# zzmuxi/simian-spacemonkey

Hardware: AMD Instinct MI355X
Metric: Msamples/s + fps, 512^3 VGH vol @1024^2 x 512 steps (higher is better)
Workload: dtype f32

## Files before the change

simian-spacemonkey_amd/csrc/smk_api.hip:

```cpp
#include <math.h>
#include <stdio.h>
#include <string.h>

#include <algorithm>

#include "smk_device.h"

static std::string g_create_err;

#include <condition_variable>
#include <mutex>
#include <thread>
namespace {
struct HostPool {
  std::vector<std::thread> workers;
  std::mutex m, use;
  std::condition_variable cv, done_cv;
  const std::function<void(int)> *job = nullptr;
  int njobs = 0, next = 0, pending = 0;
  unsigned long long gen = 0;
  bool quit = false;
  explicit HostPool(int n) {
    for (int i = 0; i < n; ++i)
      workers.emplace_back([this] {
        unsigned long long seen = 0;
        for (;;) {
          std::unique_lock<std::mutex> lk(m);
          cv.wait(lk, [&] { return quit || (gen != seen && next < njobs); });
          if (quit) return;
          while (next < njobs) {
            const int k = next++;
            lk.unlock();
            (*job)(k);
            lk.lock();
            if (--pending == 0) done_cv.notify_all();
          }
          seen = gen;
        }
      });
  }
  ~HostPool() {
    {
      std::lock_guard<std::mutex> lk(m);
      quit = true;
    }
    cv.notify_all();
    for (std::thread &t : workers) t.join();
  }
};
HostPool *host_pool() {
  static HostPool *pool = [] {
    const char *e = getenv("SMK_HOST_THREADS");
    int n = e ? atoi(e) : (int)std::min(16u, std::max(1u, std::thread::hardware_concurrency() / 2));
    n = std::max(1, std::min(n, 32));
    return new HostPool(n - 1);
  }();
  return pool;
}
}

int smk_host_pool_size() { return (int)host_pool()->workers.size() + 1; }

void smk_host_pool_run(int n, const std::function<void(int)> &f) {
  HostPool *p = host_pool();
  if (n <= 1 || p->workers.empty()) {
    for (int k = 0; k < n; ++k) f(k);
    return;
  }
  std::lock_guard<std::mutex> one(p->use);
  {
    std::lock_guard<std::mutex> lk(p->m);
    p->job = &f;
    p->njobs = n;
    p->next = 1;
    p->pending = n - 1;
    ++p->gen;
  }
  p->cv.notify_all();
  f(0);
  std::unique_lock<std::mutex> lk(p->m);
  while (p->next < p->njobs) {
    const int k = p->next++;
    lk.unlock();
    f(k);
    lk.lock();
    --p->pending;
  }
  p->done_cv.wait(lk, [&] { return p->pending == 0; });
  p->job = nullptr;
  p->njobs = 0;
}


extern "C" smk_ctx *smk_create(int device_ordinal, int *err) {
  int n = 0;
  hipError_t e = hipGetDeviceCount(&n);
  if (e != hipSuccess || n <= 0) {
    g_create_err = "smk_create: no HIP device available (this library has no CPU fallback)";
    if (err) *err = 1;
    return nullptr;
  }
  if (device_ordinal < 0 || device_ordinal >= n) {
    g_create_err = "smk_create: device ordinal out of range";
    if (err) *err = 2;
    return nullptr;
  }
  if (hipSetDevice(device_ordinal) != hipSuccess) {
    g_create_err = "smk_create: hipSetDevice failed";
    if (err) *err = 3;
    return nullptr;
  }
  smk_ctx *c = new smk_ctx();
  c->device = device_ordinal;
  if (hipStreamCreateWithFlags(&c->stream, hipStreamNonBlocking) != hipSuccess) {
    g_create_err = "smk_create: stream/event creation failed";
    delete c;
    if (err) *err = 4;
    return nullptr;
  }
  if (err) *err = 0;
  return c;
}

static void free_brick_set(BrickSet &B) {
  if (B.flags) (void)hipFree(B.flags);
  if (B.dil) (void)hipFree(B.dil);
  if (B.sat) (void)hipFree(B.sat);
  if (B.d_count) (void)hipFree(B.d_count);
  if (B.h_count) (void)hipHostFree(B.h_count);
  if (B.counted) (void)hipEventDestroy(B.counted);
  B = BrickSet();
}

static void free_volume(smk_ctx *c) {
  smk_free_steps(c);
  smk_cols_drop_layouts(&c->cols);
  c->d_brick_mm = nullptr;
  c->d_vox_x = nullptr;
  c->d_vox = nullptr;
  c->d_nrm = nullptr;
  c->have_volume = false;
}

extern "C" void smk_destroy(smk_ctx *c) {
  if (!c) return;
  (void)hipSetDevice(c->device);
  (void)hipDeviceSynchronize();
  free_volume(c);
  for (smk_ctx::TfVersion &T : c->tfv) {
    if (T.d) (void)hipFree(T.d);
    if (T.h) (void)hipHostFree(T.h);
    free_brick_set(T.br);
    if (T.copied) (void)hipEventDestroy(T.copied);
    if (T.used) (void)hipEventDestroy(T.used);
  }
  if (c->tf_raw_ev) (void)hipEventDestroy(c->tf_raw_ev);
  if (c->tf_ready) (void)hipEventDestroy(c->tf_ready);
  if (c->tf_stream) { (void)hipStreamSynchronize(c->tf_stream); (void)hipStreamDestroy(c->tf_stream); }
  free_brick_set(c->br3);
  smk_cols_free(&c->cols);
  void *ptrs[] = {c->d_light_hist, c->d_shadow_entries, c->d_shadow_exports, c->d_shadow_barrier, c->d_tf_raw, c->d_tlut, c->d_tf_h, c->d_tf3d, c->d_tf3d_occ, c->d_noise, c->d_out, c->d_depth, c->d_zscene, c->d_light[0], c->d_light[1]};
  for (void *p : ptrs)
    if (p) (void)hipFree(p);
  smk_slab_free(&c->slab);
  for (hipEvent_t e : c->tev0) (void)hipEventDestroy(e);
  for (hipEvent_t e : c->tev1) (void)hipEventDestroy(e);
  if (c->stream) (void)hipStreamDestroy(c->stream);
  delete c;
}

extern "C" const char *smk_last_error(smk_ctx *c) { return c ? c->err.c_str() : g_create_err.c_str(); }


template <int DT>
__global__ void smk_k_pack(const void *src, const unsigned char *grad, int bx, int by, int cz, int nelts,
                           int gx0, int gy0, int gz0,
                           int Ox, int Oy, int Oz, int Dx, int Dy, int Dz, void *dst, uint32_t *nrm, int n_in_w) {
  size_t t = (size_t)blockIdx.x * blockDim.x + threadIdx.x;
  size_t total = (size_t)bx * by * cz;
  if (t >= total) return;
  int x = (int)(t % bx);
  int y = (int)((t / bx) % by);
  int z = (int)(t / ((size_t)bx * by));
  int X = gx0 + x - Ox, Y = gy0 + y - Oy, Z = gz0 + z - Oz;
  if (X < 0 || X >= Dx || Y < 0 || Y >= Dy || Z < 0 || Z >= Dz) return;
  size_t o = ((size_t)Z * Dy + Y) * Dx + X;
  uint32_t nb = 0x00808080u;
  if (grad) nb = (uint32_t)grad[t * 3] | ((uint32_t)grad[t * 3 + 1] << 8) | ((uint32_t)grad[t * 3 + 2] << 16);
  if (DT == 0) {
    const unsigned char *s = (const unsigned char *)src + t * nelts;
    uint32_t d = 0;
    for (int e = 0; e < nelts; ++e) d |= (uint32_t)s[e] << (8 * e);
    ((uint2 *)dst)[o] = make_uint2(d, nb);
  } else {
    const float *s = (const float *)src + t * nelts;
    float4 v = make_float4(0.f, 0.f, 0.f, 0.f);
    v.x = s[0];
    if (nelts > 1) v.y = s[1];
    if (nelts > 2) v.z = s[2];
    if (n_in_w) v.w = __uint_as_float(nb);
    else {
      v.w = s[3];
      if (nrm) nrm[o] = nb;
    }
    ((float4 *)dst)[o] = v;
  }
}

static void shard_box(const int N[3], int rank, int nranks, int g0[3], int g1[3]) {
  for (int a = 0; a < 3; ++a) {
    g0[a] = 0;
    g1[a] = N[a];
  }
  int bit = 0;
  for (int n = nranks; n > 1; n >>= 1, ++bit) {
    int a = bit % 3, half = N[a] / 2;
    if ((rank >> bit) & 1) g0[a] = std::max(g0[a], half);
    else g1[a] = std::min(g1[a], half);
  }
}

void smk_shard_region(const smk_ctx *c, int rank, int g0[3], int g1[3]) { shard_box(c->N, rank, c->nranks, g0, g1); }

int smk_volume_geometry(smk_ctx *c, const char *who, const smk_volume_desc *b, int nb, int nelts, smk_dtype dtype,
                        smk_datamode dmode, SmkVolGeom &g) {
  if (!b || nb <= 0) FAIL(c, "%s: no bricks", who);
  if (nelts < 1 || nelts > 4) FAIL(c, "%s: nelts %d not in 1..4", who, nelts);
  if (dtype != SMK_U8 && dtype != SMK_F32) FAIL(c, "%s: bad dtype", who);
  g = SmkVolGeom();
  g.dtype = dtype;
  g.nelts = nelts;
  g.dmode = dmode;
  int *N = g.N;
  float *fs = g.fs;
  bool any_grad = false, all_grad = true;
  for (int i = 0; i < nb; ++i) {
    if (!b[i].data) FAIL(c, "%s: brick %d has no data", who, i);
    if (b[i].xiSize <= 0 || b[i].yiSize <= 0 || b[i].ziSize <= 0) FAIL(c, "%s: brick %d empty", who, i);
    if (b[i].xiPos < 0 || b[i].yiPos < 0 || b[i].ziPos < 0) FAIL(c, "%s: brick %d negative origin", who, i);
    N[0] = std::max(N[0], b[i].xiPos + b[i].xiSize);
    N[1] = std::max(N[1], b[i].yiPos + b[i].yiSize);
    N[2] = std::max(N[2], b[i].ziPos + b[i].ziSize);
    fs[0] = std::max(fs[0], b[i].xfPos + b[i].xfSize);
    fs[1] = std::max(fs[1], b[i].yfPos + b[i].yfSize);
    fs[2] = std::max(fs[2], b[i].zfPos + b[i].zfSize);
    any_grad |= b[i].grad != nullptr;
    all_grad &= b[i].grad != nullptr;
  }
  if (any_grad && !all_grad) FAIL(c, "%s: some bricks have normals and some do not", who);
  size_t vox = 0;
  for (int i = 0; i < nb; ++i) vox += (size_t)b[i].xiSize * b[i].yiSize * b[i].ziSize;
  if (vox != (size_t)N[0] * N[1] * N[2]) FAIL(c, "%s: bricks do not tile the %dx%dx%d volume", who, N[0], N[1], N[2]);
  if (!(fs[0] > 0 && fs[1] > 0 && fs[2] > 0)) FAIL(c, "%s: non-positive extent", who);
  if (c->nranks > 1)
    for (int a = 0; a < 3; ++a)
      if (N[a] < 2) FAIL(c, "%s: volume too thin to shard", who);
  g.grad = any_grad;
  shard_box(N, c->rank, c->nranks, g.g0, g.g1);
  for (int a = 0; a < 3; ++a) {
    int lo = std::max(g.g0[a] - c->halo, 0), hi = std::min(g.g1[a] + c->halo, N[a]);
    g.O[a] = lo;
    g.D[a] = hi - lo;
  }
  if (dtype == SMK_U8)
    for (int a = 0; a < 2; ++a)
      if (g.D[a] & 1) {
        if (g.O[a] + g.D[a] < N[a]) ++g.D[a];
        else if (g.O[a] > 0) { --g.O[a]; ++g.D[a]; }
        else { ++g.D[a]; g.padded = true; }
      }
  const size_t nst = (size_t)g.D[0] * g.D[1] * g.D[2];
  g.vox_bytes = nst * (dtype == SMK_U8 ? 8 : 16);
  g.nrm_bytes = dtype == SMK_F32 && nelts == 4 && any_grad ? nst * 4 : 0;
  for (int a = 0; a < 3; ++a) g.nbr[a] = (g.D[a] - 1) / (1 << SMK_BRICK_LOG2) + 1;
  g.mm_bytes = (size_t)g.nbr[0] * g.nbr[1] * g.nbr[2] * sizeof(float4);
  return 0;
}

void smk_set_geometry(smk_ctx *c, const SmkVolGeom &g) {
  c->dtype = g.dtype;
  c->nelts = g.nelts;
  c->dmode = g.dmode;
  for (int a = 0; a < 3; ++a) {
    c->N[a] = g.N[a];
    c->fsize[a] = g.fs[a];
    c->g0[a] = g.g0[a];
    c->g1[a] = g.g1[a];
    c->O[a] = g.O[a];
    c->D[a] = g.D[a];
    c->nbr[a] = g.nbr[a];
  }
  c->vox_bytes = g.vox_bytes;
  c->have_normals = g.grad;
}

int smk_alloc_step(smk_ctx *c, const SmkVolGeom &g, TimeStep &T) {
  if (!T.vox) {
    HIPCHK(c, hipMalloc(&T.vox, g.vox_bytes + 16));
    if (g.padded) HIPCHK(c, hipMemset(T.vox, 0, g.vox_bytes));
  }
  if (g.nrm_bytes && !T.nrm) HIPCHK(c, hipMalloc((void **)&T.nrm, g.nrm_bytes));
  if (!T.mm) HIPCHK(c, hipMalloc((void **)&T.mm, g.mm_bytes));
  return 0;
}

int smk_pack_step(smk_ctx *c, const char *who, const SmkVolGeom &g, const smk_volume_desc *b, int nb, bool on_device, TimeStep &T,
                  hipStream_t s) {
// ... 355 lines not shown
  if (!c || !out) return 1;
  if (!c->have_volume || !c->have_camera) FAIL(c, "smk_get_raycoef: volume and camera must be set");
  double inv[16];
  return compute_raycoef(c, out, inv);
}

static void normalize3(float v[3]) {
  float l = sqrtf(v[0] * v[0] + v[1] * v[1] + v[2] * v[2]);
  if (l > 0) {
    v[0] /= l;
    v[1] /= l;
    v[2] /= l;
  }
}

static void shading_vectors(const smk_ctx *c, RenderParams &P) {
  const float *r = c->xform;
  P.R[0] = r[0]; P.R[1] = r[4]; P.R[2] = r[8];
  P.R[3] = r[1]; P.R[4] = r[5]; P.R[5] = r[9];
  P.R[6] = r[2]; P.R[7] = r[6]; P.R[8] = r[10];
  P.intens = c->intens;
  P.use_spec = (c->shade == SMK_SHADE_R8K_DSPEC || c->shade == SMK_SHADE_NV20_DSPEC) ? 1 : 0;
  if (c->shade == SMK_SHADE_R8K_DIFF || c->shade == SMK_SHADE_R8K_DSPEC) {
    float l[3] = {-c->light_pos[0], -c->light_pos[1], -c->light_pos[2]};
    normalize3(l);
    float vd[3] = {-(c->eye[0] - c->at[0]), -(c->eye[1] - c->at[1]), -(c->eye[2] - c->at[2])};
    normalize3(vd);
    float h[3];
    for (int k = 0; k < 3; ++k) h[k] = l[k] + 0.5f * (vd[k] - l[k]);
    normalize3(h);
    memcpy(P.L, l, 12);
    memcpy(P.Hv, h, 12);
  } else {
    float vd[3] = {c->eye[0] - c->at[0], c->eye[1] - c->at[1], c->eye[2] - c->at[2]};
    normalize3(vd);
    float lt[3] = {c->light_pos[0] - c->at[0], c->light_pos[1] - c->at[1], c->light_pos[2] - c->at[2]};
    normalize3(lt);
    float h[3];
    for (int k = 0; k < 3; ++k) h[k] = lt[k] + 0.5f * (vd[k] - lt[k]);
    float hv[3] = {r[0] * h[0] + r[1] * h[1] + r[2] * h[2], r[4] * h[0] + r[5] * h[1] + r[6] * h[2],
                   r[8] * h[0] + r[9] * h[1] + r[10] * h[2]};
    float lv[3] = {r[0] * lt[0] + r[1] * lt[1] + r[2] * lt[2], r[4] * lt[0] + r[5] * lt[1] + r[6] * lt[2],
                   r[8] * lt[0] + r[9] * lt[1] + r[10] * lt[2]};
    for (int k = 0; k < 3; ++k) {
      hv[k] = -hv[k];
      lv[k] = -lv[k];
    }
    normalize3(hv);
    normalize3(lv);
    memcpy(P.L, lv, 12);
    memcpy(P.Hv, hv, 12);
  }
}

static int make_brick_set(smk_ctx *c, BrickSet &B, const uint32_t *occ, int roww, int sv, int sg, hipStream_t s) {
  const size_t nbricks = (size_t)c->nbr[0] * c->nbr[1] * c->nbr[2], sat_words = (size_t)(sv + 1) * (sg + 1);
  if (B.flags_cap < nbricks) {
    if (B.flags) (void)hipFree(B.flags);
    B.flags = nullptr;
    B.flags_cap = 0;
    HIPCHK(c, hipMalloc((void **)&B.flags, nbricks));
    B.flags_cap = nbricks;
  }
  if (B.sat_cap < sat_words) {
    if (B.sat) (void)hipFree(B.sat);
    B.sat = nullptr;
    B.sat_cap = 0;
    HIPCHK(c, hipMalloc((void **)&B.sat, sat_words * 4));
    B.sat_cap = sat_words;
  }
  if (!B.d_count) HIPCHK(c, hipMalloc((void **)&B.d_count, 4));
  if (!B.h_count) HIPCHK(c, hipHostMalloc((void **)&B.h_count, 4, hipHostMallocDefault));
  if (!B.counted) HIPCHK(c, hipEventCreateWithFlags(&B.counted, hipEventDisableTiming));
  else HIPCHK(c, hipEventSynchronize(B.counted));
  if (smk_step_wait_ready(c, s)) return 1;
  HIPCHK(c, smk_bricks_flags(c->d_brick_mm, c->nbr, occ, roww, sv, sg, B.sat, B.flags, B.d_count, s));
  HIPCHK(c, hipMemcpyAsync(B.h_count, B.d_count, 4, hipMemcpyDeviceToHost, s));
  HIPCHK(c, hipEventRecord(B.counted, s));
  B.valid = true;
  B.fill = -1.f;
  B.dil_r[0] = -1;
  return 0;
}

static const unsigned char *brick_flags_to_use(smk_ctx *c, BrickSet &B) {
  if (!B.valid) return nullptr;
  if (B.fill < 0.f && hipEventQuery(B.counted) == hipSuccess)
    B.fill = (float)((double)*B.h_count / ((double)c->nbr[0] * c->nbr[1] * c->nbr[2]));
  (void)hipGetLastError();
  return B.fill > 0.9f ? nullptr : B.flags;
}

__global__ __launch_bounds__(256) void smk_k_tf_effective(const uint32_t *raw, const unsigned char *map, int sv, int sg, int roww,
                                                           uint32_t *eff, uint32_t *occ) {
  const int wave = (int)((blockIdx.x * 256u + threadIdx.x) >> 6), lane = threadIdx.x & 63;
  const int wpr = (sv + 63) / 64;
  const int t = wave / wpr, s = (wave - t * wpr) * 64 + lane;
  if (t >= sg) return;
  bool any = false;
  if (s < sv) {
    const int s1 = min(s + 1, sv - 1), t1 = min(t + 1, sg - 1);
    const uint32_t a = raw[(size_t)t * sv + s];
    const unsigned ma = map[a >> 24];
    eff[(size_t)t * sv + s] = (a & 0x00ffffffu) | (ma << 24);
    any = (ma | map[raw[(size_t)t * sv + s1] >> 24] | map[raw[(size_t)t1 * sv + s] >> 24] | map[raw[(size_t)t1 * sv + s1] >> 24]) != 0;
  }
  const unsigned long long m = __ballot(any);
  const int w0 = (s - lane) >> 5;
  if (lane == 0 && w0 < roww) occ[(size_t)t * roww + w0] = (uint32_t)m;
  if (lane == 32 && w0 + 1 < roww) occ[(size_t)t * roww + w0 + 1] = (uint32_t)(m >> 32);
}

static float tf2d_rate(const smk_ctx *c, const smk_raycoef &rc) {
  if (c->scale_alphas) {
    float rate = c->steps > 0 ? (float)(c->fsize[0] / ((double)c->N[0] * (double)rc.dis)) : c->sample_rate;
    return rate * 1 / c->gamma;
  }
  return 1 / c->gamma;
}

static void tf2d_alpha_map(const smk_ctx *c, float sr, unsigned char map[256]) {
  if (c->opt_tf_raw) {
    for (int a = 0; a < 256; ++a) map[a] = (unsigned char)a;
    return;
  }
  const float alphaScale = (float)(1.0 / sr);
  for (int a = 0; a < 256; ++a) map[a] = (unsigned char)(int)((1.0 - pow((1.0 - (a / 255.0)), alphaScale)) * 255);
}

static int refresh_tf2d(smk_ctx *c, const smk_raycoef &rc, hipStream_t frame_stream) {
  if (c->tf_mode != 1) return 0;
  const float sr = tf2d_rate(c, rc);
  if (!c->tf_dirty && sr == c->tf_rate_applied && c->d_tf_vg) {
    if (c->tf_ready_pending) HIPCHK(c, hipStreamWaitEvent(frame_stream, c->tf_ready, 0));
    return 0;
  }
  unsigned char newmap[256];
  tf2d_alpha_map(c, sr, newmap);
  if (!c->tf_dirty && c->d_tf_vg && c->tf_map_valid && !memcmp(newmap, c->tf_map_applied, 256)) {
    c->tf_rate_applied = sr;
    if (c->tf_ready_pending) HIPCHK(c, hipStreamWaitEvent(frame_stream, c->tf_ready, 0));
    return 0;
  }
  if (!c->tf_stream) HIPCHK(c, hipStreamCreateWithFlags(&c->tf_stream, hipStreamNonBlocking));
  if (!c->tf_ready) HIPCHK(c, hipEventCreateWithFlags(&c->tf_ready, hipEventDisableTiming));
  const hipStream_t s = c->tf_stream;
  const size_t n = (size_t)c->sv * c->sg;
  const int sv = c->sv, sg = c->sg, roww = (sv + 31) / 32;
  const size_t occ_words = (size_t)roww * sg, bytes = n * 4 + occ_words * 4 + 256;
  const int v = (c->tf_cur + 1) & 3;
  smk_ctx::TfVersion &T = c->tfv[v];
  if (T.cap < bytes) {
    if (T.copied) (void)hipEventSynchronize(T.copied);
    if (T.used_valid) (void)hipEventSynchronize(T.used);
    if (T.d) (void)hipFree(T.d);
    if (T.h) (void)hipHostFree(T.h);
    T.d = nullptr;
    T.h = nullptr;
    T.cap = 0;
    HIPCHK(c, hipMalloc((void **)&T.d, bytes));
    HIPCHK(c, hipHostMalloc((void **)&T.h, bytes, hipHostMallocDefault));
    T.cap = bytes;
    if (!T.copied) HIPCHK(c, hipEventCreateWithFlags(&T.copied, hipEventDisableTiming));
    if (!T.used) HIPCHK(c, hipEventCreateWithFlags(&T.used, hipEventDisableTiming));
    T.used_valid = false;
  } else if (T.copied) {
    HIPCHK(c, hipEventSynchronize(T.copied));
  }
  if (c->tf_raw_cap < n * 4) {
    HIPCHK(c, hipDeviceSynchronize());
    if (c->d_tf_raw) (void)hipFree(c->d_tf_raw);
    c->d_tf_raw = nullptr;
    c->tf_raw_cap = 0;
    HIPCHK(c, hipMalloc((void **)&c->d_tf_raw, n * 4));
    c->tf_raw_cap = n * 4;
    c->tf_raw_stale = true;
  }
  if (!c->tf_raw_ev) HIPCHK(c, hipEventCreateWithFlags(&c->tf_raw_ev, hipEventDisableTiming));
  if (c->tf_raw_stale) {
    memcpy(T.h, c->h_tf_vg.data(), n * 4);
    if (c->tf_raw_ev_valid) HIPCHK(c, hipStreamWaitEvent(s, c->tf_raw_ev, 0));
    HIPCHK(c, hipMemcpyAsync(c->d_tf_raw, T.h, n * 4, hipMemcpyHostToDevice, s));
    c->tf_raw_stale = false;
  }
  unsigned char *map = T.h + n * 4 + occ_words * 4;
  memcpy(map, newmap, 256);
  memcpy(c->tf_map_applied, newmap, 256);
  c->tf_map_valid = true;
  if (T.used_valid) HIPCHK(c, hipStreamWaitEvent(s, T.used, 0));
  HIPCHK(c, hipMemcpyAsync(T.d + n * 4 + occ_words * 4, map, 256, hipMemcpyHostToDevice, s));
  HIPCHK(c, hipEventRecord(T.copied, s));
  {
    const int wpr = (sv + 63) / 64;
    const unsigned blocks = (unsigned)(((size_t)wpr * sg + 3) / 4);
    hipLaunchKernelGGL(smk_k_tf_effective, dim3(blocks), dim3(256), 0, s, (const uint32_t *)c->d_tf_raw, T.d + n * 4 + occ_words * 4, sv,
                       sg, roww, (uint32_t *)T.d, (uint32_t *)(T.d + n * 4));
    HIPCHK(c, hipGetLastError());
    HIPCHK(c, hipEventRecord(c->tf_raw_ev, s));
    c->tf_raw_ev_valid = true;
  }
  c->tf_cur = v;
  c->d_tf_vg = reinterpret_cast<uint32_t *>(T.d);
  c->d_tf_occ = reinterpret_cast<uint32_t *>(T.d + n * 4);
  T.br.valid = false;
  if (c->opt_bricks && c->d_brick_mm && make_brick_set(c, T.br, c->d_tf_occ, roww, sv, sg, s)) return 1;
  c->tf_occ_roww = roww;
  c->tf_rate_applied = sr;
  c->tf_dirty = false;
  HIPCHK(c, hipEventRecord(c->tf_ready, s));
  HIPCHK(c, hipStreamWaitEvent(frame_stream, c->tf_ready, 0));
  c->tf_ready_pending = true;
  return 0;
}

extern "C" int smk_get_tf2d_effective(smk_ctx *c, unsigned char *out, float *rate) {
  if (!c) return 1;
  if (c->tf_mode != 1 || !c->have_volume || !c->have_camera) FAIL(c, "smk_get_tf2d_effective: 2-D TF, volume and camera required");
  smk_raycoef rc;
  double inv[16];
  compute_raycoef(c, &rc, inv);
  if (refresh_tf2d(c, rc, c->stream)) return 1;
  if (out) {
    unsigned char map[256];
    tf2d_alpha_map(c, c->tf_rate_applied, map);
    memcpy(out, c->h_tf_vg.data(), c->h_tf_vg.size());
    for (size_t i = 0; i < (size_t)c->sv * c->sg; ++i) out[i * 4 + 3] = map[c->h_tf_vg[i * 4 + 3]];
  }
  if (rate) *rate = c->tf_rate_applied;
  return 0;
}

void smk_bsp_order(const smk_ctx *c, const double pos[3], int *order) {
  int nearbit[3];
  for (int a = 0; a < 3; ++a) nearbit[a] = pos[a] >= (double)(c->N[a] / 2) - 0.5 ? 1 : 0;
  int nbits = 0;
  for (int n = c->nranks; n > 1; n >>= 1) ++nbits;
  std::vector<std::pair<int, int>> keyed;
  for (int r = 0; r < c->nranks; ++r) {
    int key = 0;
    for (int bit = 0; bit < nbits; ++bit)
      if (((r >> bit) & 1) != nearbit[bit % 3]) key |= 1 << bit;
    keyed.push_back({key, r});
  }
  std::sort(keyed.begin(), keyed.end());
  for (int r = 0; r < c->nranks; ++r) order[r] = keyed[r].second;
}

extern "C" int smk_shard_order(smk_ctx *c, int *order) {
  if (!c || !order) return 1;
  if (!c->have_volume || !c->have_camera) FAIL(c, "smk_shard_order: volume and camera must be set");
  double inv[16];
  smk_inverse_affine(inv, c->mv);
  double e[3];
  for (int a = 0; a < 3; ++a) e[a] = inv[12 + a] * c->N[a] / c->fsize[a] - 0.5;
  smk_bsp_order(c, e, order);
  return 0;
}


extern "C" int smk_set_option(smk_ctx *c, const char *key, int value) {
  if (!c || !key) return 1;
  if (!strcmp(key, "kernel")) c->opt_kernel = value;
  else if (!strcmp(key, "slab_T")) c->slab.opt_T = value & 0xff;
  else if (!strcmp(key, "inject_slab_status")) c->opt_inject_status = value;
  else if (!strcmp(key, "slab_fly")) c->slab.opt_fly = value < 0 ? 0 : (value > 63 ? 63 : value);
  else if (!strcmp(key, "slab_ns")) c->slab.opt_ns = value < 0 ? 0 : (value > 63 ? 63 : value);
  else if (!strcmp(key, "tile")) c->slab.opt_tile = value;
  else if (!strcmp(key, "shadow_march")) c->opt_shadow_march = value ? 1 : 0;
  else if (!strcmp(key, "shadow_fused")) c->opt_lockstep = value ? (c->opt_lockstep | 256) : (c->opt_lockstep & ~256);
  else if (!strcmp(key, "slab_split")) c->slab.opt_split = value < 0 ? 0 : (value > 8 ? 8 : value);
  else if (!strcmp(key, "cols_shape")) c->cols.opt_shape = value & 0xff;
  else if (!strcmp(key, "cols_ns")) c->cols.opt_ns = value & 0xff;
  else if (!strcmp(key, "cols_chunk")) c->cols.opt_chunk = value & 0xfff;
  else if (!strcmp(key, "cols_wstep")) c->cols.opt_wstep = value & 7;
  else if (!strcmp(key, "cols_counts")) c->cols.want_counts = value ? 1 : 0;
  else if (!strcmp(key, "cols_fill")) { c->cols.opt_fill = value; smk_cols_drop_layouts(&c->cols); }
  else if (!strcmp(key, "cols_take_min")) c->cols.opt_take_min = value;
  else if (!strcmp(key, "cols_take_wait")) c->cols.opt_take_wait = value;
  else if (!strcmp(key, "cols_fly")) c->cols.opt_fly = value;
  else if (!strcmp(key, "bricks")) {
    c->opt_bricks = value ? 1 : 0;
    c->tf_dirty = true;
    c->bricks3_dirty = true;
  }
  else if (!strcmp(key, "wave_w")) {
    if (!(value == 1 || value == 2 || value == 4 || value == 8 || value == 16 || value == 32 || value == 64)) FAIL(c, "smk_set_option: wave_w must be a power of two <= 64");
    c->opt_wave_w = value;
  } else if (!strcmp(key, "blk_w")) {
    if (!(value == 1 || value == 2 || value == 4)) FAIL(c, "smk_set_option: blk_w must be 1, 2 or 4");
    c->opt_blk_w = value;
  } else if (!strcmp(key, "lockstep")) c->opt_lockstep = value;
  else if (!strcmp(key, "tf_raw")) {
    c->opt_tf_raw = value;
    c->tf_dirty = true;
  }
  else if (!strcmp(key, "halo")) {
    if (c->have_volume) FAIL(c, "smk_set_option: halo must be set before smk_upload_volume");
    if (value < 1) FAIL(c, "smk_set_option: halo must be >= 1");
    c->halo = value;
  } else
    FAIL(c, "smk_set_option: unknown key '%s'", key);
  return 0;
}

extern "C" int smk_get_brick_flags(smk_ctx *c, unsigned char *flags_out, int *nb_out, int *in_use_out) {
  if (!c || !nb_out) return 1;
  HIPCHK(c, hipSetDevice(c->device));
  RenderParams P;
  if (smk_build_params(c, P, c->stream)) return 1;
  HIPCHK(c, hipDeviceSynchronize());
  for (int a = 0; a < 3; ++a) nb_out[a] = c->nbr[a];
  const BrickSet *B = c->tf_mode == 1 && c->tf_cur >= 0 ? &c->tfv[c->tf_cur].br : c->tf_mode == 2 ? &c->br3 : nullptr;
  if (in_use_out) *in_use_out = P.bricks != nullptr ? 1 : 0;
  if (flags_out) {
    if (!B || !B->valid || !B->flags) FAIL(c, "smk_get_brick_flags: no flags for this table (1-D colour table, or option 'bricks' 0)");
    HIPCHK(c, hipMemcpy(flags_out, B->flags, (size_t)c->nbr[0] * c->nbr[1] * c->nbr[2], hipMemcpyDeviceToHost));
  }
  return 0;
}

template <class Launch>
static int count_on_device(smk_ctx *c, Launch launch, double *out) {
  unsigned long long *d = nullptr, h = 0;
  HIPCHK(c, hipMalloc((void **)&d, 8));
  hipError_t e = hipMemsetAsync(d, 0, 8, c->stream);
  if (e == hipSuccess) e = launch(d);
  if (e == hipSuccess) e = hipMemcpyAsync(&h, d, 8, hipMemcpyDeviceToHost, c->stream);
  if (e == hipSuccess) e = hipStreamSynchronize(c->stream);
  (void)hipFree(d);
  HIPCHK(c, e);
  *out = (double)h;
  return 0;
}

extern "C" int smk_get_stat(smk_ctx *c, const char *name, double *value) {
  if (!c || !name || !value) return 1;
  HIPCHK(c, hipSetDevice(c->device));
  static const char *diag_names[16] = {"slab_iters", "slab_active_lanes", "slab_inside_lanes", "slab_hit_lanes",
                                      "slab_loader_issue_kcyc", "slab_loader_wait_kcyc", "slab_loader_blocked_kcyc", "slab_loader_total_kcyc",
                                      "slab_iters_with_hit", "slab_lead_sum", "slab_waits", "slab_wstep_sum", "slab_dead_tail_sum", "slab_waves",
                                      "slab_iters_sampling", "slab_iters_own_brick"};
  for (int k = 0; k < 16; ++k)
    if (!strcmp(name, diag_names[k])) {
      float v = 0.f;
      if (c->slab.d_diag && read_back(c, &v, c->slab.d_diag + k, 1)) return 1;
      *value = v;
      return 0;
    }
  if (!strcmp(name, "light_samples")) {
    RenderParams P;
    smk_shadowcoef sc;
    float olo[3], ohi[3];
    if (smk_shadow_light_owned(c, P, sc, olo, ohi)) return 1;
    return count_on_device(c, [&](unsigned long long *d) { return smk_launch_shadow_count_light(P, sc, olo, ohi, d, c->stream); }, value);
  }
  if (!strcmp(name, "slab_status")) {
    HIPCHK(c, hipDeviceSynchronize());
    *value = c->slab.h_status ? (((volatile int *)c->slab.h_status)[c->slab.status_slot] & 0xff) : 0;
    return 0;
  }
  if (!strcmp(name, "slab_failures")) {
    long long n = c->slab_failures;
    if (c->slab.h_status)
      for (int k = 0; k < SMK_STATUS_RING; ++k) n += ((volatile int *)c->slab.h_status)[k] != 0;
    *value = (double)n;
    return 0;
  }
  if (!strcmp(name, "slab_streamed_fraction")) {
    *value = 1.0;
    const int nt = c->slab.ticks_n_last;
    if (c->last_kernel == 2 && c->slab.d_ticks && nt > 0) {
      std::vector<unsigned> h((size_t)2 * nt);
      if (read_back(c, h.data(), c->slab.d_ticks + nt, h.size())) return 1;
      double st = 0, pl = 0;
      for (int t = 0; t < nt; ++t) {
        st += h[t];
        pl += h[(size_t)nt + t];
      }
      if (pl > 0) *value = st / pl;
    }
    return 0;
  }
  if (!strcmp(name, "slab_tile_ms_max") || !strcmp(name, "slab_tile_ms_sum")) {
    *value = 0.0;
    const int nt = c->slab.ticks_n_last;
    if (c->last_kernel == 2 && c->slab.d_ticks && nt > 0) {
      std::vector<unsigned> h((size_t)nt);
      if (read_back(c, h.data(), c->slab.d_ticks, h.size())) return 1;
      double mx = 0, sum = 0;
      for (int t = 0; t < nt; ++t) {
        const double k = t < (int)c->slab.ksplit_last.size() ? std::max<int>(c->slab.ksplit_last[t], 1) : 1;
        mx = std::max(mx, (double)h[t] / k);
        sum += h[t];
      }
      *value = (name[13] == 'm' ? mx : sum) * 1e-5;
    }
    return 0;
  }
  if (!strncmp(name, "cols_", 5)) return smk_cols_stat(c, name, value);
  if (!strcmp(name, "slab_split_tiles")) { *value = c->slab.nsplit_last; return 0; }
  if (!strcmp(name, "slab_workgroups")) { *value = c->slab.nblocks_last; return 0; }
  if (!strcmp(name, "slab_retries")) { *value = (double)c->slab_retries; return 0; }
  if (!strcmp(name, "clip_slice_pass")) { *value = c->clip_slice_pass; return 0; }
  FAIL(c, "smk_get_stat: unknown name '%s'", name);
}

extern "C" int smk_get_trace(smk_ctx *c, unsigned *out, int cap_records, int *nrecords) {
  if (!c || !nrecords) return 1;
  HIPCHK(c, hipSetDevice(c->device));
  if (!(c->opt_lockstep & 32)) {
    const int nt = c->last_kernel == 2 && c->slab.d_ticks ? c->slab.ticks_n_last : 0;
    *nrecords = nt;
    if (out && nt > 0) {
      std::vector<unsigned> h((size_t)nt * 5);
      if (read_back(c, h.data(), c->slab.d_ticks, h.size())) return 1;
      for (int t = 0; t < std::min(cap_records, nt); ++t) {
        unsigned *r = out + (size_t)t * 8;
        r[0] = h[(size_t)3 * nt + t];
        r[1] = h[(size_t)3 * nt + t] ? r[0] + h[t] : 0u;
        r[2] = h[(size_t)4 * nt + t] & 0xff00u;
        r[3] = (h[(size_t)4 * nt + t] & 0xfu) | ((unsigned)t << 8) | (h[(size_t)2 * nt + t] << 20);
        r[4] = r[5] = r[6] = r[7] = 0;
      }
    }
    return 0;
  }
  *nrecords = c->slab.d_trace ? c->slab.trace_n : 0;
  if (out && *nrecords > 0 && read_back(c, out, c->slab.d_trace, (size_t)std::min(cap_records, *nrecords) * 8)) return 1;
  return 0;
}

extern "C" int smk_count_samples(smk_ctx *c, double *in_volume) {
  if (!c || !in_volume) return 1;
  HIPCHK(c, hipSetDevice(c->device));
  RenderParams P;
  if (smk_build_params(c, P, c->stream)) return 1;
  smk_shadowcoef sc;
  if (c->shadow_on && c->tf_mode != 0 && !P.pert_on && !c->region_on && smk_shadow_setup(c, P, sc, nullptr, nullptr)) return 1;
  return count_on_device(c, [&](unsigned long long *d) { return smk_launch_count_inside(P, d, c->stream); }, in_volume);
}

void smk_region_box(const smk_ctx *c, const int g0[3], const int g1[3], float lo[3], float hi[3], int top[3]) {
  for (int a = 0; a < 3; ++a) {
    lo[a] = (float)g0[a] - 0.5f;
    hi[a] = (float)g1[a] - 0.5f;
    top[a] = g1[a] == c->N[a];
  }
  if (c->clip_axis >= 1 && c->clip_axis <= 6) {
    const int a = (c->clip_axis - 1) / 2;
    const float fs = c->fsize[a];
    const float cp = c->clip_vpos[a] > 0.0f ? (c->clip_vpos[a] < fs ? c->clip_vpos[a] : fs) : 0.0f;
    const float face = (float)((double)cp / (double)fs * (double)c->N[a] - 0.5);
    if ((c->clip_axis - 1) % 2 == 0) {
      if (face < hi[a] || (face == hi[a] && !top[a])) { hi[a] = face; top[a] = 1; }
    } else if (face > lo[a]) {
      lo[a] = face;
    }
  }
  if (c->region_on)
    for (int a = 0; a < 3; ++a) {
      const double fs = c->fsize[a];
      const double l = c->region_lo[a] > 0 ? (c->region_lo[a] < fs ? c->region_lo[a] : fs) : 0.0;
      const double h = c->region_hi[a] > 0 ? (c->region_hi[a] < fs ? c->region_hi[a] : fs) : 0.0;
      const float flo = (float)(l / fs * (double)c->N[a] - 0.5), fhi = (float)(h / fs * (double)c->N[a] - 0.5);
      if (flo > lo[a]) lo[a] = flo;
      if (fhi < hi[a]) { hi[a] = fhi; top[a] = 0; }
    }
}

int smk_build_params(smk_ctx *c, RenderParams &P, hipStream_t s) {
  if (!c->have_volume) FAIL(c, "smk_render: no volume uploaded");
  if (!c->have_camera) FAIL(c, "smk_render: no camera set");
  if (c->tf_mode < 0) FAIL(c, "smk_render: no transfer function set");
  memset(&P, 0, sizeof P);
  double inv[16];
  compute_raycoef(c, &P.rc, inv);
  if (refresh_tf2d(c, P.rc, s)) return 1;
  if (smk_step_wait_ready(c, s)) return 1;
  P.vox = c->d_vox;
  P.nrm = c->d_nrm;
  for (int a = 0; a < 3; ++a) {
    P.N[a] = c->N[a];
    P.O[a] = c->O[a];
    P.D[a] = c->D[a];
    P.invN[a] = 1.0f / (float)c->N[a];
  }
  smk_region_box(c, c->g0, c->g1, P.lo, P.hi, P.top);
  for (int a = 0; a < 3; ++a) P.hin[a] = P.top[a] ? P.hi[a] : nextafterf(P.hi[a], -INFINITY);
  P.cplane_on = c->cplane_on;
  for (int k = 0; k < 4; ++k) P.cplane[k] = 0.0f;
  if (c->cplane_on) {
    double pm[4];
    for (int k = 0; k < 4; ++k)
      pm[k] = c->cplane_eye[0] * c->mv[4 * k + 0] + c->cplane_eye[1] * c->mv[4 * k + 1] + c->cplane_eye[2] * c->mv[4 * k + 2] +
              c->cplane_eye[3] * c->mv[4 * k + 3];
    double w = pm[3];
    for (int a = 0; a < 3; ++a) {
      const double sc = (double)c->fsize[a] / (double)c->N[a];
      P.cplane[a] = (float)(pm[a] * sc);
      w += pm[a] * sc * 0.5;
    }
    P.cplane[3] = (float)w;
  }
  P.nelts = c->nelts;
  P.n_in_w = (c->dtype == SMK_F32 && c->nelts <= 3) ? 1 : 0;
  P.tlut = c->d_tlut;
  P.tlut_size = c->tlut_size;
  P.tf_vg = c->d_tf_vg;
  P.tf_h = c->d_tf_h;
  P.tf_occ = c->tf_mode == 1 ? c->d_tf_occ : c->tf_mode == 2 ? c->d_tf3d_occ : nullptr;
  P.occ_roww = c->tf_mode == 2 ? c->tf3d_occ_roww : c->tf_occ_roww;
  P.sv = c->sv;
  P.sg = c->sg;
  bool third = c->dmode == SMK_GDM_VGH || c->dmode == SMK_GDM_V1GH || c->dmode == SMK_GDM_V2G ||
               c->dmode == SMK_GDM_V2GH || c->dmode == SMK_GDM_V3 || c->dmode == SMK_GDM_V3G || c->dmode == SMK_GDM_V4;
  P.third_axis = (third && c->d_tf_h && c->nelts >= 3) ? 1 : 0;
  P.tf3d = c->d_tf3d;
  P.s3v = c->s3v;
  P.s3g = c->s3g;
  P.s3h = c->s3h;
  P.bricks = nullptr;
  for (int a = 0; a < 3; ++a) P.nbr[a] = c->nbr[a];
  BrickSet *bset = nullptr;
  P.bricks_dil = nullptr;
  if (c->opt_bricks && c->d_brick_mm) {
    if (c->tf_mode == 1 && c->tf_cur >= 0) {
      P.bricks = brick_flags_to_use(c, c->tfv[c->tf_cur].br);
      bset = &c->tfv[c->tf_cur].br;
    }
    if (c->tf_mode == 2 && c->d_tf3d_occ) {
      if (c->bricks3_dirty || !c->br3.valid) {
        HIPCHK(c, hipDeviceSynchronize());
        if (make_brick_set(c, c->br3, c->d_tf3d_occ, c->tf3d_occ_roww, c->s3v, c->s3g, s)) return 1;
        c->bricks3_dirty = false;
      }
      P.bricks = brick_flags_to_use(c, c->br3);
      bset = &c->br3;
    }
  }
  P.W = c->W;
  P.H = c->H;
  P.znear = c->clip[0];
  shading_vectors(c, P);
  P.blend = c->blend;
  P.noise = c->d_noise;
  P.nn = c->nn;
  P.nn_log2 = -1;
  for (int l = 0; l < 12; ++l)
    if (c->nn == (1 << l)) P.nn_log2 = l;
  P.pw[0] = c->pw[0];
  P.pw[1] = c->pw[1];
  P.ps[0] = c->ps[0];
  P.ps[1] = c->ps[1];
  P.pert_on = (c->d_noise && (c->pw[0] != 0 || c->pw[1] != 0)) ? 1 : 0;
// ... 255 lines not shown
```

simian-spacemonkey_amd/csrc/smk_cols_plan.hip:

```cpp
#include <math.h>
#include <stdio.h>
#include <string.h>

#include <algorithm>
#include <vector>

#include "smk_cols.h"

struct ColPlan {
  int as, au, av;
  int perm;
  double dens;
  int shape;
  int vb;
  size_t fixed;
  int njobs;
};

static const char *cols_refusal(const RenderParams &P, int dtype, int tf_mode) {
  if (P.zscene) return "scene depth";
  if (tf_mode < 0 || tf_mode > 2) return "no classification mode";
  if (tf_mode == 0 && (!P.tlut || P.tlut_size < 1)) return "no colour table";
  if (tf_mode == 1 && (!P.tf_vg || P.sv < 2 || P.sg < 2)) return "transfer function smaller than 2x2";
  if (tf_mode == 2 && (!P.tf3d || P.s3v < 1 || P.s3g < 1 || P.s3h < 1)) return "no 3-D table";
// ... 98 lines not shown
    if (!project(u, v, sc, x0, y0) || !project(u + 1, v, sc, x1, y1) || !project(u, v + 1, sc, x2, y2) || !project(u, v, sc + 1, x3, y3))
      return "volume reaches behind the eye";
    dens = std::max(dens, fabs((x1 - x0) * (y2 - y0) - (x2 - x0) * (y1 - y0)));
  }
  if (!(dens > 1e-9)) return "degenerate projection";
  L.dens = dens;
  return nullptr;
}

static const char *cols_lds_budget(const RenderParams &P, int dtype, int tf_mode, const ColsAux *aux, ColParams &Q, ColPlan &L) {
  L.shape = aux->opt_shape ? aux->opt_shape - 1 : 0;
  if (L.shape < 0 || L.shape >= COL_NSHAPES) return "no such workgroup shape";
  L.vb = dtype == 0 ? 8 : 16;
  const bool three = P.third_axis && P.tf_h;
  Q.use_ah = (tf_mode == 1 && three && P.nelts <= 3 && P.sv >= 2 && P.sv <= 1024) ? 1 : 0;
  Q.fast_tf = (tf_mode == 1 && (!three || Q.use_ah)) ? 1 : 0;
  const size_t occ_bytes = tf_mode == 1 ? (size_t)P.occ_roww * P.sg * 4 : tf_mode == 2 ? (size_t)P.occ_roww * P.s3g * 4 : 0;
  Q.use_occ = (P.tf_occ && occ_bytes > 0 && occ_bytes <= 16384 && (Q.fast_tf || tf_mode == 2)) ? 1 : 0;
  L.fixed = (size_t)COL_MAX_RAYS * 9 + (size_t)3 * (COL_MAX_CL + 4) * 4 + 32 * 4 + (Q.use_ah ? (size_t)P.sv * 4 : 0) + (Q.use_occ ? occ_bytes : 0) + 64;
  return nullptr;
}

static size_t cols_slice_bytes(int cw, int ch, int vb) { return (((size_t)(cw + 1) * (ch + 1) * vb) + 15) & ~(size_t)15; }

static bool cols_fits(const ColPlan &L, double fill, int cw, int ch, int slots) {
  if ((double)cw * ch * L.dens > fill * (kColShapes[L.shape].nw * 64)) return false;
  const size_t sb = cols_slice_bytes(cw, ch, L.vb);
  if (sb * slots + L.fixed > COL_LDS_CAP) return false;
  if ((sb + 1023) / 1024 * 2 > 63) return false;
  return true;
}

static void cols_free_layout(ColLayout &L) {
  if (L.d) (void)hipFree(L.d);
  L = ColLayout();
}

static bool cols_column_size(const ColPlan &L, double fill, int cells_u, int cells_v, int slots, int *bw, int *bh) {
  *bw = *bh = 0;
  double best = 1e300;
  for (int ncu = 1; ncu <= cells_u; ++ncu) {
    const int cw = (cells_u + ncu - 1) / ncu;
    if (cw > 255) continue;
    if (ncu > 1 && (cells_u + ncu - 2) / (ncu - 1) == cw) continue;
    for (int ncv = 1; ncv <= cells_v; ++ncv) {
      const int ch = (cells_v + ncv - 1) / ncv;
      if (ch > 255) continue;
      if (ncv > 1 && (cells_v + ncv - 2) / (ncv - 1) == ch) continue;
      if (!cols_fits(L, fill, cw, ch, slots)) continue;
      const double over = (double)ncu * (cw + 1) * (double)ncv * (ch + 1) / ((double)cells_u * cells_v);
      if (over < best) { best = over; *bw = cw; *bh = ch; }
    }
  }
  return *bw != 0;
}

static hipError_t cols_layout(const RenderParams &P, ColParams &Q, const ColPlan &L, int dtype, const void *vox_native, ColsAux *aux,
                              const char **why, hipStream_t s) {
  ColLayout &LY = aux->lay[L.perm];
  const int lanes = kColShapes[L.shape].nw * 64;
  const int cells_u = Q.Du - 1, cells_v = Q.Dv - 1;
  const double fill = (aux->opt_fill > 0 ? aux->opt_fill : 92) * 0.01;
  bool reuse = LY.d && LY.Du == Q.Du && LY.Dv == Q.Dv && LY.Ds == Q.Ds && LY.src == vox_native && LY.vb == L.vb;
  if (reuse) {
    reuse = cols_fits(L, fill, LY.CW, LY.CH, 3) && ((double)LY.CW * LY.CH * L.dens > 0.45 * lanes || (LY.CW >= cells_u && LY.CH >= cells_v));
  }
  if (!reuse) {
    int bw, bh;
    if (!cols_column_size(L, fill, cells_u, cells_v, aux->opt_ns ? aux->opt_ns : 6, &bw, &bh)) {
      *why = "no column size fits the lanes (view too close)";
      return hipErrorNotSupported;
    }
    const int ncu = (cells_u + bw - 1) / bw, ncv = (cells_v + bh - 1) / bh;
    const size_t sb = cols_slice_bytes(bw, bh, L.vb);
    const size_t bytes = (size_t)ncu * ncv * Q.Ds * sb;
    size_t free_b = 0, total_b = 0;
    (void)hipMemGetInfo(&free_b, &total_b);
    if (LY.d) cols_free_layout(LY);
    if (bytes + ((size_t)2 << 30) > free_b + 0) {
      for (int k = 0; k < 3; ++k)
        if (k != L.perm) cols_free_layout(aux->lay[k]);
      (void)hipMemGetInfo(&free_b, &total_b);
      if (bytes + ((size_t)1 << 30) > free_b) { *why = "no memory for the column layout"; return hipErrorNotSupported; }
    }
    void *d = nullptr;
    if (hipMalloc(&d, bytes + 4096) != hipSuccess) { (void)hipGetLastError(); *why = "no memory for the column layout"; return hipErrorNotSupported; }
    LY.d = d; LY.bytes = bytes; LY.CW = bw; LY.CH = bh; LY.ncu = ncu; LY.ncv = ncv; LY.Du = Q.Du; LY.Dv = Q.Dv; LY.Ds = Q.Ds;
    LY.slice_bytes = (int)sb; LY.src = vox_native; LY.vb = L.vb;
    const size_t total = (size_t)ncu * ncv * Q.Ds * (size_t)(bw + 1) * (bh + 1);
    const unsigned blocks = (unsigned)((total + 255) / 256);
    if (total / 256 > 0x7fffffffull) { *why = "volume too large for the layout builder"; return hipErrorNotSupported; }
    hipError_t e = smk_cols_build(vox_native, dtype, L.perm, P.D, bw, bh, ncu, ncv, (int)sb, d, blocks, s);
    if (e != hipSuccess) return e;
    ++aux->builds;
  }
  Q.lay = (const char *)LY.d;
  Q.CW = LY.CW; Q.CH = LY.CH; Q.ncu = LY.ncu; Q.ncv = LY.ncv;
  Q.slice_bytes = LY.slice_bytes;
  return hipSuccess;
}

static const char *cols_ring(const ColsAux *aux, const ColPlan &L, ColParams &Q) {
  Q.n_ch = (Q.slice_bytes + 1023) / 1024;
  const int last_units = Q.slice_bytes / 16 - 64 * (Q.n_ch - 1);
  Q.last_mask = last_units >= 64 ? ~0ull : ((1ull << last_units) - 1ull);
  int nslots = (int)((COL_LDS_CAP - L.fixed) / (size_t)Q.slice_bytes);
  if (aux->opt_ns) nslots = std::min(nslots, aux->opt_ns);
  nslots = std::min(nslots, 12);
  if (nslots < 3) return "column slice does not fit LDS three times";
  Q.nslots = nslots;
  Q.maxfly = std::max(1, std::min(aux->opt_fly > 0 ? aux->opt_fly : 2, (nslots - 2) / kColShapes[L.shape].nl));
  while (Q.maxfly > 1 && Q.n_ch * Q.maxfly > 63) --Q.maxfly;
  if (Q.n_ch > 63) return "column slice needs more than 63 DMA instructions";
  Q.wstep = aux->opt_wstep ? aux->opt_wstep - 1 : (nslots >= 7 ? 2 : nslots >= 5 ? 1 : 0);
  Q.take_min = aux->opt_take_min > 0 ? aux->opt_take_min : 16;
  Q.take_wait = aux->opt_take_wait > 0 ? aux->opt_take_wait - 1 : 3;
  return nullptr;
}

static const char *cols_chunks(const ColsAux *aux, ColParams &Q, ColPlan &L) {
  const int npos_total = Q.Ds - 1;
  int clmax = aux->opt_chunk ? std::min(aux->opt_chunk, COL_MAX_CL) : 128;
  clmax = std::max(clmax, 4);
  Q.nck = (npos_total + clmax - 1) / clmax;
  Q.CL = (npos_total + Q.nck - 1) / Q.nck;
  Q.nck = (npos_total + Q.CL - 1) / Q.CL;
  Q.nkeys = Q.ncu + Q.ncv + Q.nck - 2;
  Q.mask_words = (Q.nkeys + 63) / 64;
  if (Q.mask_words > 8) return "more than 512 segment keys";
  L.njobs = Q.ncu * Q.ncv * Q.nck;
  return nullptr;
}

static hipError_t cols_side_buffers(const RenderParams &P, ColParams &Q, const ColPlan &L, ColsAux *aux, int *status_word, const char **why,
                                    hipStream_t s) {
  const size_t npix = (size_t)P.W * P.H;
  const size_t lay_bytes = (size_t)Q.nkeys * npix * 16;
  if (lay_bytes > aux->layers_cap) {
    if (aux->d_layers) (void)hipFree(aux->d_layers);
    aux->d_layers = nullptr; aux->layers_cap = 0;
    if (hipMalloc(&aux->d_layers, lay_bytes) != hipSuccess) { (void)hipGetLastError(); *why = "no memory for the segment layers"; return hipErrorNotSupported; }
    aux->layers_cap = lay_bytes;
  }
  const size_t mask_bytes = npix * Q.mask_words * 8;
  if (mask_bytes > aux->masks_cap || aux->masks_dirty) {
    if (mask_bytes > aux->masks_cap) {
      if (aux->d_masks) (void)hipFree(aux->d_masks);
      aux->d_masks = nullptr; aux->masks_cap = 0;
      if (hipMalloc(&aux->d_masks, mask_bytes) != hipSuccess) { (void)hipGetLastError(); *why = "no memory for the segment masks"; return hipErrorNotSupported; }
      aux->masks_cap = mask_bytes;
    }
    hipError_t e = hipMemsetAsync(aux->d_masks, 0, aux->masks_cap, s);
    if (e != hipSuccess) return e;
    aux->masks_dirty = false;
  }
  aux->mask_words_last = Q.mask_words;
  if (L.njobs > aux->ticks_cap) {
    if (aux->d_ticks) (void)hipFree(aux->d_ticks);
    aux->d_ticks = nullptr; aux->ticks_cap = 0;
    if (hipMalloc((void **)&aux->d_ticks, (size_t)L.njobs * 12) != hipSuccess) { (void)hipGetLastError(); *why = "no memory"; return hipErrorNotSupported; }
    aux->ticks_cap = L.njobs;
  }
  if (!aux->d_counts) {
    if (hipMalloc((void **)&aux->d_counts, 8 * 8) != hipSuccess) { (void)hipGetLastError(); *why = "no memory"; return hipErrorNotSupported; }
  }
  Q.layers = (float4 *)aux->d_layers;
  Q.masks = (unsigned long long *)aux->d_masks;
  Q.status = status_word;
  Q.status_tag = aux->status_tag;
  Q.job_ticks = aux->d_ticks;
  Q.counts = aux->want_counts ? aux->d_counts : nullptr;
  if (Q.counts) return hipMemsetAsync(aux->d_counts, 0, 64, s);
  return hipSuccess;
}

static hipError_t cols_run(const RenderParams &P, ColParams &Q, const ColPlan &L, ColsAux *aux, int dtype, int tf_mode, int shade_kind,
                           const char **why, hipStream_t s) {
  aux->njobs_last = L.njobs;
  aux->cw_last = Q.CW; aux->ch_last = Q.CH; aux->nslots_last = Q.nslots; aux->shape_last = L.shape;
  aux->last_stream_bytes = (double)L.njobs / Q.nck * ((double)(Q.Ds - 1) + Q.nck) * Q.slice_bytes;
  Q.ring_bytes = (int)std::max((size_t)Q.nslots * Q.slice_bytes, (size_t)COL_MAX_RAYS * 16);
  const size_t lds = (size_t)Q.ring_bytes + L.fixed;
  if (lds > COL_LDS_CAP) { *why = "column job does not fit LDS"; return hipErrorNotSupported; }
  if (aux->frame_ev0) {
    hipError_t e = hipEventRecord(aux->frame_ev0, s);
    if (e != hipSuccess) return e;
  }
  hipError_t e = smk_cols_march(P, Q, dtype, tf_mode, shade_kind, L.perm, L.shape, lds, L.njobs, s);
  if (e == hipErrorInvalidValue) { *why = "no column-stream instance for this mode"; return hipErrorNotSupported; }
  if (e != hipSuccess) return e;
  aux->masks_dirty = true;
  e = smk_cols_resolve((const float4 *)aux->d_layers, (unsigned long long *)aux->d_masks, Q.mask_words, (size_t)P.W * P.H, P.out,
                       P.blend == SMK_BLEND_MAX ? 1 : 0, s);
  if (e == hipSuccess) aux->masks_dirty = false;
  return e;
}

hipError_t smk_launch_cols(RenderParams P, int dtype, int tf_mode, int shade_kind, const void *vox_native, ColsAux *aux, int *status_word,
                           const char **why, hipStream_t s) {
  ColParams Q;
  memset(&Q, 0, sizeof Q);
  ColPlan L = {};
  if ((*why = cols_refusal(P, dtype, tf_mode))) return hipErrorNotSupported;
  if (tf_mode == 0) shade_kind = 0;
  if ((*why = cols_axes(P, Q, L)) || (*why = cols_projection(P, Q)) || (*why = cols_density(P, Q, L)) ||
      (*why = cols_lds_budget(P, dtype, tf_mode, aux, Q, L)))
    return hipErrorNotSupported;
  hipError_t e = cols_layout(P, Q, L, dtype, vox_native, aux, why, s);
  if (e != hipSuccess) return e;
  if ((*why = cols_ring(aux, L, Q)) || (*why = cols_chunks(aux, Q, L))) return hipErrorNotSupported;
  if ((e = cols_side_buffers(P, Q, L, aux, status_word, why, s)) != hipSuccess) return e;
  return cols_run(P, Q, L, aux, dtype, tf_mode, shade_kind, why, s);
}

void smk_cols_free(ColsAux *aux) {
  for (int k = 0; k < 3; ++k) cols_free_layout(aux->lay[k]);
  if (aux->d_layers) (void)hipFree(aux->d_layers);
  if (aux->d_masks) (void)hipFree(aux->d_masks);
  if (aux->d_ticks) (void)hipFree(aux->d_ticks);
  if (aux->d_counts) (void)hipFree(aux->d_counts);
  *aux = ColsAux();
}

void smk_cols_drop_layouts(ColsAux *aux) {
  for (int k = 0; k < 3; ++k) cols_free_layout(aux->lay[k]);
}

int smk_cols_stat(smk_ctx *c, const char *name, double *value) {
  const ColsAux &A = c->cols;
  *value = 0.0;
  if (!strcmp(name, "cols_builds")) { *value = A.builds; return 0; }
  if (!strcmp(name, "cols_config")) { *value = A.cw_last | (A.ch_last << 8) | (A.nslots_last << 16) | (A.shape_last << 24); return 0; }
  if (!strcmp(name, "cols_jobs")) { *value = A.njobs_last; return 0; }
  if (!strcmp(name, "cols_stream_bytes")) { *value = A.last_stream_bytes; return 0; }
  if (!strcmp(name, "cols_job_ms_max") || !strcmp(name, "cols_job_ms_sum") || !strcmp(name, "cols_setup_ms_sum") || !strcmp(name, "cols_rays")) {
    const int nj = A.njobs_last, part = name[5] == 'j' ? 0 : name[5] == 's' ? 1 : 2;
    if (c->last_kernel == 4 && A.d_ticks && nj > 0) {
      std::vector<unsigned> h((size_t)nj);
      if (read_back(c, h.data(), A.d_ticks + (size_t)nj * part, h.size())) return 1;
      double mx = 0, sum = 0;
      for (unsigned v : h) {
        mx = std::max(mx, (double)v);
        sum += v;
      }
      *value = part == 2 ? sum : (name[12] == 'm' ? mx : sum) * 1e-5;
    }
    return 0;
  }
  static const char *cn[8] = {"cols_samples", "cols_visible", "cols_slices", "cols_segments", "cols_iters", "cols_active_lanes", "cols_switch_iters", "cols_switch_lanes"};
  for (int k = 0; k < 8; ++k)
    if (!strcmp(name, cn[k])) {
      unsigned long long v = 0;
      if (A.d_counts && A.want_counts && read_back(c, &v, A.d_counts + k, 1)) return 1;
      *value = (double)v;
      return 0;
    }
  FAIL(c, "smk_get_stat: unknown name '%s'", name);
}
```

simian-spacemonkey_amd/csrc/smk_frame.hip:

```cpp
#include <math.h>
#include <stdio.h>
#include <stdlib.h>
#include <string.h>

#include <algorithm>

#include "smk_internal.h"

extern "C" int smk_timing_reset(smk_ctx *c) {
  if (!c) return 1;
  c->tcount = 0;
  return 0;
}

extern "C" int smk_timing_read(smk_ctx *c, float *avg_ms, int *nframes) {
  if (!c) return 1;
  HIPCHK(c, hipSetDevice(c->device));
  HIPCHK(c, hipDeviceSynchronize());
  int n = (int)std::min<long long>(c->tcount, SMK_TIMING_RING);
  double sum = 0;
  for (int i = 0; i < n; ++i) {
    float ms = 0;
    HIPCHK(c, hipEventElapsedTime(&ms, c->tev0[i], c->tev1[i]));
    sum += ms;
  }
  if (avg_ms) *avg_ms = n ? (float)(sum / n) : 0.f;
  if (nframes) *nframes = n;
  return 0;
}

extern "C" int smk_last_frame_info(smk_ctx *c, int *kernel, float *ms, double *alg_bytes) {
  if (!c) return 1;
  if (kernel) *kernel = c->last_kernel;
  if (ms) *ms = c->last_ms;
  if (alg_bytes) *alg_bytes = c->last_alg_bytes;
  return 0;
}

static int take_status(smk_ctx *c, long long id) {
  if (!c->slab.h_status || id <= 0) return 0;
  volatile int *w = (volatile int *)c->slab.h_status + (int)(id % SMK_STATUS_RING);
  const int st = *w;
  if (!st) return 0;
  const long long tag = (st >> 8) & 0x7fffff;
  if (tag != (id & 0x7fffff)) {
    if (((id - tag) & 0x7fffff) % SMK_STATUS_RING == 0 && tag != 0) {
      *w = 0;
      ++c->slab_failures;
      ++c->slab_lost;
    }
    return 0;
  }
  *w = 0;
  ++c->slab_failures;
  if (c->opt_kernel == 0 && c->last_slab_sig) c->tune_choice[c->last_slab_sig] = {1, c->frame_id + 256};
  return st & 0xff;
}

static const char *status_text(int st) {
  return st == 1 ? "a streaming kernel reported a producer/consumer time-out" : st == 2 ? "the slice-ring kernel reported a window outside its host bound"
         : st == 3 ? "the column-stream kernel reported a job whose rays do not fit its lanes or its list" : "the column-stream kernel reported a ray it cannot list";
}

static int check_frame_status(smk_ctx *c, long long id) {
  const int st = take_status(c, id);
  if (st) FAIL(c, "%s (status %d, frame %lld); frame invalid", status_text(st), st, id);
  return 0;
}

extern "C" long long smk_last_frame_id(smk_ctx *c) { return c ? c->frame_id : 0; }

extern "C" int smk_frame_failed(smk_ctx *c, long long frame_id) {
  if (!c) return 1;
  if (frame_id <= 0 || frame_id > c->frame_id || frame_id + SMK_STATUS_RING <= c->frame_id) return -1;
  return take_status(c, frame_id) ? 1 : 0;
}

static int status_ring_ready(smk_ctx *c) {
  if (c->slab.h_status) return 0;
  HIPCHK(c, hipHostMalloc((void **)&c->slab.h_status, SMK_STATUS_RING * sizeof(int), hipHostMallocMapped));
  for (int k = 0; k < SMK_STATUS_RING; ++k) c->slab.h_status[k] = 0;
  HIPCHK(c, hipMalloc((void **)&c->slab.d_diag, 16 * sizeof(float)));
  return 0;
}

static void inject_status(smk_ctx *c) {
  if (c->opt_inject_status && c->slab.h_status) {
    ((volatile int *)c->slab.h_status)[c->slab.status_slot] = c->slab.status_tag | c->opt_inject_status;
    c->opt_inject_status = 0;
  }
}


static int frame_open(smk_ctx *c, RenderParams &P, void *d_rgba, void *d_depth) {
  P.out = (float4 *)d_rgba;
  P.depth = (float *)d_depth;
  size_t nst = (size_t)c->D[0] * c->D[1] * c->D[2];
  double bv = c->dtype == SMK_U8 ? (double)c->nelts : 4.0 * c->nelts;
  if (smk_shade_kind(c)) bv += 3.0;
  double tfb = c->tf_mode == 0 ? 16.0 * c->tlut_size
               : c->tf_mode == 1 ? 4.0 * c->sv * c->sg * (P.third_axis ? 2 : 1)
                                 : 4.0 * c->s3v * c->s3g * c->s3h;
  c->last_alg_bytes = (double)nst * bv + tfb + 16.0 * c->W * c->H;
  if (P.zscene) c->last_alg_bytes += 4.0 * c->W * c->H;
  if (c->tev0.empty()) {
    c->tev0.resize(SMK_TIMING_RING);
    c->tev1.resize(SMK_TIMING_RING);
    for (int i = 0; i < SMK_TIMING_RING; ++i) {
      HIPCHK(c, hipEventCreate(&c->tev0[i]));
      HIPCHK(c, hipEventCreate(&c->tev1[i]));
    }
  }
  int slot = (int)(c->tcount % SMK_TIMING_RING);
  c->ev0 = c->tev0[slot];
  c->ev1 = c->tev1[slot];
  c->last_kernel = 1;
  c->slab_why.clear();
  if (check_frame_status(c, c->frame_id + 1 - SMK_STATUS_RING)) return 1;
  ++c->frame_id;
  c->slab.status_slot = (int)(c->frame_id % SMK_STATUS_RING);
  c->slab.status_tag = c->cols.status_tag = (int)((c->frame_id & 0x7fffff) << 8);
  if (c->slab.h_status) ((volatile int *)c->slab.h_status)[c->slab.status_slot] = 0;
  return 0;
}

struct KernelChoice {
  bool try_slab;
  unsigned long long sig;
  int trial;
};

static KernelChoice choose_kernel(smk_ctx *c, const RenderParams &P, bool with_depth, hipStream_t s) {
  KernelChoice k = {c->opt_kernel != 1 && c->opt_kernel != 3, 0, -1};
  if (c->opt_kernel != 0) return k;
  int as = 0;
  for (int a = 1; a < 3; ++a)
    if (fabsf(P.rc.Bc[a]) > fabsf(P.rc.Bc[as])) as = a;
  const unsigned long long f[] = {(unsigned long long)c->dtype, (unsigned long long)c->nelts, (unsigned long long)c->D[0],
                                  (unsigned long long)c->D[1], (unsigned long long)c->D[2], (unsigned long long)c->W,
                                  (unsigned long long)c->H, (unsigned long long)P.rc.nplanes, (unsigned long long)smk_shade_kind(c),
                                  (unsigned long long)P.third_axis, (unsigned long long)(as * 2 + (P.rc.Bc[as] > 0)),
                                  (unsigned long long)c->sv, (unsigned long long)c->sg, (unsigned long long)with_depth,
                                  (unsigned long long)P.pert_on, (unsigned long long)c->tf_mode, (unsigned long long)c->s3v,
                                  (unsigned long long)c->s3g, (unsigned long long)c->s3h, (unsigned long long)c->blend,
                                  (unsigned long long)P.sh.on, (unsigned long long)(P.zscene != nullptr)};
  k.sig = 1469598103934665603ull;
  for (unsigned long long v : f) k.sig = (k.sig ^ v) * 1099511628211ull;
  auto it = c->tune_choice.find(k.sig);
  if (it != c->tune_choice.end() && it->second.expires <= c->frame_id) {
    c->tune_choice.erase(it);
    it = c->tune_choice.end();
    c->tune_sig = 0;
  }
  if (it != c->tune_choice.end()) {
    k.try_slab = it->second.kernel == 2;
    return k;
  }
  if (c->tune_sig != k.sig) {
    c->tune_sig = k.sig;
    c->tune_state = 0;
  }
  if (c->tune_state == SMK_TUNE_SETTLE + 3) {
    float ms_s = 0, ms_g = 0;
    if (c->tcount - c->tune_tcount >= SMK_TIMING_RING - 8) (void)hipEventSynchronize(c->tev1[c->tune_slot[1]]);
    if (hipEventQuery(c->tev1[c->tune_slot[0]]) == hipSuccess && hipEventQuery(c->tev1[c->tune_slot[1]]) == hipSuccess &&
        hipEventElapsedTime(&ms_s, c->tev0[c->tune_slot[0]], c->tev1[c->tune_slot[0]]) == hipSuccess &&
        hipEventElapsedTime(&ms_g, c->tev0[c->tune_slot[1]], c->tev1[c->tune_slot[1]]) == hipSuccess) {
      c->tune_choice[k.sig] = {ms_s <= ms_g ? 2 : 1, c->frame_id + 1024};
      k.try_slab = ms_s <= ms_g;
      if (getenv("SMK_DEBUG")) fprintf(stderr, "[smk] auto mode: slice-ring %.3f ms, gather %.3f ms (frame %lld)\n", ms_s, ms_g, c->frame_id);
    }
    (void)hipGetLastError();
  } else {
    k.trial = c->tune_state;
    k.try_slab = k.trial != SMK_TUNE_SETTLE && k.trial != SMK_TUNE_SETTLE + 2;
    if (k.try_slab && k.trial > 0) (void)hipStreamSynchronize(s);
  }
  return k;
}

static int launch_cols(smk_ctx *c, const RenderParams &P, hipStream_t s) {
  if (status_ring_ready(c)) return 1;
  const char *why = nullptr;
  c->cols.frame_ev0 = c->ev0;
  hipError_t e = smk_launch_cols(P, c->dtype, c->tf_mode, smk_shade_kind(c), c->d_vox, &c->cols,
                                 c->slab.h_status + c->slab.status_slot, &why, s);
  if (e == hipErrorNotSupported) {
    c->slab_why = why ? why : "?";
    FAIL(c, "smk_render: column-stream kernel forced but not applicable: %s", c->slab_why.c_str());
  }
  HIPCHK(c, e);
  c->last_kernel = 4;
  inject_status(c);
  return 0;
}

static int launch_slab(smk_ctx *c, const RenderParams &P, KernelChoice &k, bool ev0_recorded, hipStream_t s) {
  if (status_ring_ready(c)) return 1;
  if (c->opt_lockstep & 16) HIPCHK(c, hipMemsetAsync(c->slab.d_diag, 0, 16 * sizeof(float), s));
  const char *why = nullptr;
  c->slab.frame_ev0 = ev0_recorded ? nullptr : c->ev0;
  hipError_t e = smk_launch_slab(P, c->dtype, c->tf_mode, smk_shade_kind(c), c->d_vox, c->d_vox_x, &c->slab, &why, s);
  if (e == hipErrorNotSupported && why && !strcmp(why, "x-major copy unavailable")) {
    if (smk_make_xmajor_copy(c)) return 1;
    e = smk_launch_slab(P, c->dtype, c->tf_mode, smk_shade_kind(c), c->d_vox, c->d_vox_x, &c->slab, &why, s);
  }
  if (e == hipSuccess) {
    c->last_kernel = 2;
    c->last_slab_sig = k.sig;
    inject_status(c);
  } else if (e == hipErrorNotSupported) {
    c->slab_why = why ? why : "?";
    if (c->opt_kernel == 2) FAIL(c, "smk_render: slab kernel forced but not applicable: %s", c->slab_why.c_str());
    if (c->opt_kernel == 0) k.trial = -1;
  } else
    HIPCHK(c, e);
  return 0;
}

static int launch_gather(smk_ctx *c, const RenderParams &P, bool ev0_recorded, hipStream_t s) {
  if (!ev0_recorded) HIPCHK(c, hipEventRecord(c->ev0, s));
  HIPCHK(c, smk_launch_gather(P, c->dtype, c->tf_mode, smk_shade_kind(c), s));
  return 0;
}

static int frame_close(smk_ctx *c, hipStream_t s, int trial) {
  HIPCHK(c, hipEventRecord(c->ev1, s));
  if (trial >= 0) {
    if (trial >= SMK_TUNE_SETTLE + 1) {
      c->tune_slot[trial - (SMK_TUNE_SETTLE + 1)] = (int)(c->tcount % SMK_TIMING_RING);
      c->tune_tcount = c->tcount;
    }
    c->tune_state = trial + 1;
  }
  if (c->tf_mode == 1 && c->tf_cur >= 0) {
    HIPCHK(c, hipEventRecord(c->tfv[c->tf_cur].used, s));
    c->tfv[c->tf_cur].used_valid = true;
  }
  if (smk_step_mark_used(c, s)) return 1;
  c->tcount++;
  return 0;
}

static int scene_depth_kind_check(smk_ctx *c, const char *who, int kind) {
  if (kind != SMK_SCENE_VIEW_DEPTH && kind != SMK_SCENE_WINDOW_DEPTH)
    FAIL(c, "%s: bad scene depth kind %d (SMK_SCENE_VIEW_DEPTH = 0 or SMK_SCENE_WINDOW_DEPTH = 1)", who, kind);
  return 0;
}

static int render_frame(smk_ctx *c, const char *who, void *d_rgba, void *d_depth, const float *d_zscene, int zkind, void *stream) {
  if (!c) return 1;
  HIPCHK(c, hipSetDevice(c->device));
  if (!d_rgba) FAIL(c, "%s: null output", who);
  RenderParams P;
  hipStream_t s = stream ? (hipStream_t)stream : c->stream;
  if (smk_build_params(c, P, s)) return 1;
  if (d_zscene) {
    P.zscene = d_zscene;
    P.zscene_kind = zkind;
    const double n = c->clip[0], f = c->clip[1];
    if (zkind == SMK_SCENE_WINDOW_DEPTH && !(f > n))
      FAIL(c, "%s: window depths need a far plane beyond the near plane (clip = %g, %g)", who, n, f);
    P.zs_fn = f * n;
    P.zs_f = f;
    P.zs_fmn = f - n;
  }
  if (frame_open(c, P, d_rgba, d_depth)) return 1;
  bool marched = false;
  if (c->shadow_on) {
    if (smk_shadow_frame(c, P, d_rgba, d_depth, s, &marched)) return 1;
    if (!marched) return smk_clip_slice_stage(c, P, s) ? 1 : frame_close(c, s, -1);
  }
  KernelChoice k = choose_kernel(c, P, d_depth != nullptr, s);
  if (c->opt_kernel == 3 && launch_cols(c, P, s)) return 1;
  if (k.try_slab) {
    if (launch_slab(c, P, k, marched, s)) return 1;
  } else if (c->opt_kernel == 2)
    FAIL(c, "smk_render: slab kernel forced but classification mode %d is gather-only", c->tf_mode);
  if (c->last_kernel == 1 && launch_gather(c, P, marched, s)) return 1;
  if (smk_clip_slice_stage(c, P, s)) return 1;
  return frame_close(c, s, k.trial);
}

extern "C" int smk_render_device(smk_ctx *c, void *d_rgba, void *d_depth, void *stream) {
  return render_frame(c, "smk_render_device", d_rgba, d_depth, nullptr, 0, stream);
}

extern "C" int smk_render_occluded_device(smk_ctx *c, const void *d_scene_depth, int kind, void *d_rgba, void *d_depth, void *stream) {
  if (!c) return 1;
  if (scene_depth_kind_check(c, "smk_render_occluded_device", kind)) return 1;
  return render_frame(c, "smk_render_occluded_device", d_rgba, d_depth, (const float *)d_scene_depth, kind, stream);
}

int smk_frame_buffers(smk_ctx *c) {
  const size_t npix = (size_t)c->W * c->H;
  if (npix > c->out_cap) {
    if (c->d_out) (void)hipFree(c->d_out);
    if (c->d_depth) (void)hipFree(c->d_depth);
    c->d_out = nullptr;
    c->d_depth = nullptr;
    HIPCHK(c, hipMalloc((void **)&c->d_out, npix * 16));
    HIPCHK(c, hipMalloc((void **)&c->d_depth, npix * 4));
    c->out_cap = npix;
  }
  return 0;
}

static int render_host(smk_ctx *c, const char *who, float *rgba, float *depth, const float *scene_depth, int zkind) {
  if (!c) return 1;
  HIPCHK(c, hipSetDevice(c->device));
  if (!rgba) FAIL(c, "%s: null output", who);
  if (!c->have_camera) FAIL(c, "%s: no camera set", who);
  size_t npix = (size_t)c->W * c->H;
  if (smk_frame_buffers(c)) return 1;
  const float *d_zscene = nullptr;
  if (scene_depth) {
    if (npix > c->zscene_cap) {
      if (c->d_zscene) (void)hipFree(c->d_zscene);
      c->d_zscene = nullptr;
      c->zscene_cap = 0;
      HIPCHK(c, hipMalloc((void **)&c->d_zscene, npix * 4));
      c->zscene_cap = npix;
    }
    HIPCHK(c, hipMemcpy(c->d_zscene, scene_depth, npix * 4, hipMemcpyHostToDevice));
    d_zscene = c->d_zscene;
  }
  if (render_frame(c, who, c->d_out, depth ? c->d_depth : nullptr, d_zscene, zkind, c->stream)) return 1;
  HIPCHK(c, hipStreamSynchronize(c->stream));
  HIPCHK(c, hipEventElapsedTime(&c->last_ms, c->ev0, c->ev1));
  if (check_frame_status(c, c->frame_id)) {
    if (c->opt_kernel != 0) return 1;
    const std::string first = c->err;
    ++c->slab_retries;
    if (render_frame(c, who, c->d_out, depth ? c->d_depth : nullptr, d_zscene, zkind, c->stream)) return 1;
    HIPCHK(c, hipStreamSynchronize(c->stream));
    if (c->last_kernel != 1 || check_frame_status(c, c->frame_id)) {
      c->err = first;
      return 1;
    }
    fprintf(stderr, "[smk] %s -- frame rendered again by the gather kernel\n", first.c_str());
  }
  HIPCHK(c, hipMemcpy(rgba, c->d_out, npix * 16, hipMemcpyDeviceToHost));
  if (depth) HIPCHK(c, hipMemcpy(depth, c->d_depth, npix * 4, hipMemcpyDeviceToHost));
  return 0;
}

extern "C" int smk_render(smk_ctx *c, float *rgba, float *depth) { return render_host(c, "smk_render", rgba, depth, nullptr, 0); }

extern "C" int smk_render_occluded(smk_ctx *c, const float *scene_depth, int kind, float *rgba, float *depth) {
  if (!c) return 1;
  if (scene_depth_kind_check(c, "smk_render_occluded", kind)) return 1;
  return render_host(c, "smk_render_occluded", rgba, depth, scene_depth, kind);
}
```

simian-spacemonkey_amd/csrc/smk_internal.h:

```cpp
#pragma once
#include <hip/hip_runtime.h>
#include <stdint.h>

#include <map>
#include <string>
#include <vector>

#include "../../include/smk.h"

#define SMK_MAX_RANKS 8
#define SMK_TIMING_RING 64
#define SMK_BRICK_LOG2 3
#define SMK_SHADOW_BOX_EPS 0.0009765625f
#define SMK_TUNE_SETTLE 6
#define SMK_STATUS_RING 8

#define HIPCHK(ctx, call)                                                              \
  do {                                                                                 \
    hipError_t e_ = (call);                                                            \
    if (e_ != hipSuccess) {                                                            \
      char b_[512];                                                                    \
      snprintf(b_, sizeof b_, "%s failed: %s (%s:%d)", #call, hipGetErrorString(e_), __FILE__, __LINE__); \
      (ctx)->err = b_;                                                                 \
      return 1;                                                                        \
    }                                                                                  \
  } while (0)

#define FAIL(ctx, ...)                     \
  do {                                     \
    char b_[512];                          \
    snprintf(b_, sizeof b_, __VA_ARGS__);  \
    (ctx)->err = b_;                       \
    return 1;                              \
  } while (0)

struct SmkShadowRays {
  int on;
  float Ec[3], Dc[3], Dx[3], Dy[3], nDc, nDx, nDy;
  float numA, dB;
  float llo[3], lhi[3];
  int k0, dk, LB;
  float Xm[4], Ym[4], Wm[4], lscale, lbias;
  const float4 *hist;
  long long hstride;
};

struct SmkShadowShard {
  int nranks, rank;
  float olo[3], ohi[3];
  float glo[SMK_MAX_RANKS][3], ghi[SMK_MAX_RANKS][3];
  float xlo[3], xhi[3];
  int order[SMK_MAX_RANKS];
  const float4 *entries;
  float4 *exports;
};

struct RenderParams {
  const void *vox;
  const uint32_t *nrm;
  int N[3];
  int O[3];
  int D[3];
  float lo[3], hi[3];
  int top[3];
  int cplane_on;
  float cplane[4];
  float hin[3];
  float invN[3];
  int nelts;
  int n_in_w;
  const float4 *tlut;
  int tlut_size;
  const uint32_t *tf_vg;
  const uint32_t *tf_h;
  const uint32_t *tf_occ;
  int occ_roww;
  int sv, sg, third_axis;
  const uint32_t *tf3d;
  int s3v, s3g, s3h;
  const unsigned char *bricks;
  int nbr[3];
  const unsigned char *bricks_dil;
  smk_raycoef rc;
  SmkShadowRays sh;
  int W, H;
  float znear;
  int use_spec;
  float L[3], Hv[3];
  float R[9];
  float intens;
  int blend;
  const uint32_t *noise;
  int nn, pert_on;
  int nn_log2;
  float pw[2], ps[2];
  float4 *out;
  float *depth;
  int ntx, nty, tiles_per_xcd;
  int wave_w, blk_w, lockstep;
  const float *zscene;
  int zscene_kind;
  double zs_fn, zs_f, zs_fmn;
};

struct SlabAux {
  int *h_status = nullptr;
  int status_slot = 0;
  int status_tag = 0;
  hipEvent_t frame_ev0 = nullptr;
  float *d_diag = nullptr;
  int2 *d_order = nullptr;
  int2 *h_order[4] = {nullptr, nullptr, nullptr, nullptr};
  hipEvent_t order_ev[4] = {nullptr, nullptr, nullptr, nullptr};
  int order_next = 0;
  int order_cap = 0;
  std::vector<int2> order_host;
  struct Scan {
    std::vector<unsigned char> key;
    double v[4] = {0, 0, 0, 0};
    std::vector<int> work;
  } scan[4];
  unsigned scan_next = 0;
  std::vector<unsigned char> shape_key;
  int shape_choice = -1, shape_age = 0, shape_chunks = 0;
  std::vector<int> plan_work;
  std::vector<unsigned char> plan_cuts;
  std::vector<int2> plan_order;
  int plan_slots = 0;
  unsigned *d_ticks = nullptr, *h_ticks = nullptr;
  int ticks_cap = 0, ticks_pending_n = 0, ticks_age = 0, ticks_adopted = 0;
  int ticks_n_last = 0;
  bool ticks_pending = false;
  long long ticks_pending_sig = 0, ticks_good_sig = -1;
  hipEvent_t ticks_ev = nullptr;
  std::vector<unsigned> ticks_good;
  void *d_seg = nullptr;
  size_t seg_cap = 0;
  int opt_split = 0;
  int opt_tile = 0, opt_T = 0, opt_fly = 0, opt_ns = 0;
  bool ticks_stale = false;
  int nsplit_last = 0, nblocks_last = 0;
  std::vector<unsigned char> ksplit_last;
  unsigned *d_pticks = nullptr, *h_pticks = nullptr;
  std::vector<unsigned> pticks_good;
  std::vector<unsigned char> cuts, cuts_pending, cuts_good;
  int cuts_split = -1;
  long long cuts_sig = -1;
  bool recut = true, cuts_engaged = false, merge_warm = false;
  unsigned *d_trace = nullptr;
  int trace_cap = 0, trace_n = 0;
};

struct ColLayout {
  void *d = nullptr;
  size_t bytes = 0;
  int CW = 0, CH = 0, ncu = 0, ncv = 0, Du = 0, Dv = 0, Ds = 0, slice_bytes = 0, vb = 0;
  const void *src = nullptr;
};
struct ColsAux {
  ColLayout lay[3];
  void *d_layers = nullptr;
  size_t layers_cap = 0;
  void *d_masks = nullptr;
  size_t masks_cap = 0;
  bool masks_dirty = true;
  int mask_words_last = 0;
  unsigned *d_ticks = nullptr;
  int ticks_cap = 0, njobs_last = 0;
  unsigned long long *d_counts = nullptr;
  int want_counts = 0;
  int opt_shape = 0, opt_ns = 0, opt_chunk = 0, opt_wstep = 0;
  int opt_fill = 0, opt_take_min = 0, opt_take_wait = 0, opt_fly = 0;
  int builds = 0;
  int cw_last = 0, ch_last = 0, nslots_last = 0, shape_last = 0;
  double last_stream_bytes = 0;
  hipEvent_t frame_ev0 = nullptr;
  int status_tag = 0;
};
void smk_cols_free(ColsAux *aux);
void smk_cols_drop_layouts(ColsAux *aux);

hipError_t smk_bricks_dilate(const unsigned char *flags, const int nb[3], const int r[3], unsigned char *out, hipStream_t s);
struct BrickSet {
  unsigned char *flags = nullptr;
  uint32_t *sat = nullptr;
  unsigned *d_count = nullptr, *h_count = nullptr;
  hipEvent_t counted = nullptr;
  size_t flags_cap = 0, sat_cap = 0;
  unsigned char *dil = nullptr;
  size_t dil_cap = 0;
  int dil_r[3] = {-1, -1, -1};
  bool valid = false;
  float fill = -1.f;
};

struct TimeStep {
  int id = -1;
  long long written = 0;
  void *vox = nullptr;
  uint32_t *nrm = nullptr;
  float4 *mm = nullptr;
  void *vox_x = nullptr;
  bool vox_x_valid = false;
  hipEvent_t ready = nullptr;
  bool ready_pending = false;
  hipEvent_t used = nullptr;
  bool used_valid = false;
};

struct smk_ctx {
  int device = 0;
  std::string err;
  hipStream_t stream = nullptr;
  hipEvent_t ev0 = nullptr, ev1 = nullptr;
  std::vector<hipEvent_t> tev0, tev1;
  long long tcount = 0;

  bool have_volume = false;
  int dtype = 0, nelts = 0, dmode = 0;
  int N[3] = {0, 0, 0};
  float fsize[3] = {1, 1, 1};
  int g0[3] = {0, 0, 0}, g1[3] = {0, 0, 0};
  int O[3] = {0, 0, 0}, D[3] = {0, 0, 0};
  int halo = 1;
  int region_on = 0;
  float region_lo[3] = {0, 0, 0}, region_hi[3] = {0, 0, 0};
  int clip_axis = 0;
  float clip_vpos[3] = {0, 0, 0};
  int cplane_on = 0;
  double cplane_eye[4] = {0, 0, 0, 0};
  int clip_slice_on = 0, clip_slice_look = 0;
  float clip_slice_corners[4][3] = {{0, 0, 0}, {0, 0, 0}, {0, 0, 0}, {0, 0, 0}};
  float clip_slice_alpha = 0, clip_slice_dv = 0;
  int clip_slice_pass = 0;
  void *d_vox = nullptr;
  void *d_vox_x = nullptr;
  float4 *d_brick_mm = nullptr;
  int nbr[3] = {0, 0, 0};
  BrickSet br3;
  bool bricks3_dirty = true;
  std::string slab_why;
  uint32_t *d_nrm = nullptr;
  bool have_normals = false;
  size_t vox_bytes = 0;
  std::vector<TimeStep> ts;
  int ts_cap = 1, ts_cur = -1, ts_cur_id = 0;
  long long ts_written = 0;
  bool ts_series = false;

  int rank = 0, nranks = 1;

  int tf_mode = -1;
  float4 *d_tlut = nullptr;
  int tlut_size = 0;
  std::vector<unsigned char> h_tf_vg, h_tf_h;
  unsigned char *d_tf_raw = nullptr;
  size_t tf_raw_cap = 0;
  bool tf_raw_stale = true, tf_raw_ev_valid = false;
  hipEvent_t tf_raw_ev = nullptr;
  hipStream_t tf_stream = nullptr;
  hipEvent_t tf_ready = nullptr;
  bool tf_ready_pending = false;
  uint32_t *d_tf_vg = nullptr, *d_tf_h = nullptr, *d_tf3d = nullptr;
  uint32_t *d_tf3d_occ = nullptr;
  int tf3d_occ_roww = 0;
  uint32_t *d_tf_occ = nullptr;
  int tf_occ_roww = 0;
  struct TfVersion {
    unsigned char *d = nullptr, *h = nullptr;
    BrickSet br;
    size_t cap = 0;
    hipEvent_t copied = nullptr, used = nullptr;
    bool used_valid = false;
  } tfv[4];
  int tf_cur = -1;
  int sv = 0, sg = 0, s3v = 0, s3g = 0, s3h = 0;
  bool tf_dirty = true;
  float tf_rate_applied = -1.f;
  unsigned char tf_map_applied[256] = {0};
  bool tf_map_valid = false;

  bool have_camera = false;
  double mv[16];
  float frustum[4], clip[2];
  int W = 0, H = 0;

  float sample_rate = 2.5f, gamma = 1.f;
  int steps = 0, scale_alphas = 1;

  int blend = 0;
  int shade = 0;
  float light_pos[3] = {0, 0, -5}, eye[3] = {0, 0, -7}, at[3] = {0, 0, 0};
  float xform[16] = {1, 0, 0, 0, 0, 1, 0, 0, 0, 0, 1, 0, 0, 0, 0, 1};
  float intens = .75f, amb = .05f;

  int shadow_on = 0, shadow_px = 1024;
  float shadow_q = .5f;
  float4 *d_light[2] = {nullptr, nullptr};
  size_t light_cap = 0;
  int light_lb = 0;
  float4 *d_light_hist = nullptr;
  size_t light_hist_cap = 0;
  const float4 *d_light_last = nullptr;
  int opt_shadow_march = 1;
  unsigned *d_shadow_barrier = nullptr;
  int light_hist_n = 0;
  long long light_hist_stride = 0;
  float4 *d_shadow_entries = nullptr;
  size_t shadow_entries_cap = 0;
  bool shadow_entries_fresh = false;
  smk_shadowcoef shadow_entries_sc;
  float4 *d_shadow_exports = nullptr;
  size_t shadow_exports_cap = 0;

  uint32_t *d_noise = nullptr;
  std::vector<unsigned char> h_noise;
  int nn = 0;
  float pw[4] = {0, 0, 0, 0}, ps[4] = {0, 0, 0, 0};

  float4 *d_out = nullptr;
  float *d_depth = nullptr;
  size_t out_cap = 0;
  float *d_zscene = nullptr;
  size_t zscene_cap = 0;

  int opt_kernel = 0, opt_tf_raw = 0;
  int opt_bricks = 1;
  int opt_inject_status = 0;
  int opt_wave_w = 8, opt_blk_w = 2, opt_lockstep = 1;
  SlabAux slab;
  ColsAux cols;
  long long frame_id = 0;
  long long slab_failures = 0, slab_retries = 0;
  long long slab_lost = 0;
  struct TuneEntry { int kernel; long long expires; };
  std::map<unsigned long long, TuneEntry> tune_choice;
  unsigned long long last_slab_sig = 0;
  unsigned long long tune_sig = 0;
  int tune_state = 0, tune_slot[2] = {0, 0};
  long long tune_tcount = 0;
  int last_kernel = 0;
  float last_ms = 0;
  double last_alg_bytes = 0;
};

hipError_t smk_bricks_minmax(const void *vox, int dtype, const int D[3], const int nb[3], float4 *mm, hipStream_t s);
hipError_t smk_bricks_flags(const float4 *mm, const int nb[3], const uint32_t *occ, int roww, int sv, int sg, uint32_t *sat,
                            unsigned char *flags, unsigned *count, hipStream_t s);

hipError_t smk_launch_gather(const RenderParams &P, int dtype, int tf_mode, int shade_kind,
                             hipStream_t s);
hipError_t smk_launch_count_inside(const RenderParams &P, unsigned long long *d_count, hipStream_t s);
hipError_t smk_launch_shadow(const RenderParams &P, const smk_shadowcoef &sc, int dtype, int tf_mode, int shade_kind,
                             float4 *L0, float4 *L1, unsigned *barrier , hipStream_t s);
hipError_t smk_launch_shadow_march(const RenderParams &P, const smk_shadowcoef &sc, int dtype, int tf_mode, float4 *hist, long long hstride,
                                   hipStream_t s);
hipError_t smk_launch_shadow_exports(const RenderParams &P, const smk_shadowcoef &sc, int dtype, int tf_mode, const SmkShadowShard &S,
                                     hipStream_t s);
hipError_t smk_launch_shadow_march_shard(const RenderParams &P, const smk_shadowcoef &sc, int dtype, int tf_mode, float4 *hist,
                                         long long hstride, const SmkShadowShard &S, hipStream_t s);
hipError_t smk_launch_shadow_count_light(const RenderParams &P, const smk_shadowcoef &sc, const float olo[3], const float ohi[3],
                                         unsigned long long *d_count, hipStream_t s);
int smk_shadow_shard_setup(smk_ctx *c, RenderParams &P, smk_shadowcoef &sc, SmkShadowShard &S, hipStream_t s);
float4 *smk_shadow_entries_reserve(smk_ctx *c, int LB);
void smk_shadow_entries_commit(smk_ctx *c, const smk_shadowcoef &sc);
hipError_t smk_launch_slab(RenderParams P, int dtype, int tf_mode, int shade_kind, const void *vox_native, const void *vox_xmajor, SlabAux *aux,
                           const char **why, hipStream_t s);
void smk_slab_forget_measurements(SlabAux *aux);
hipError_t smk_launch_cols(RenderParams P, int dtype, int tf_mode, int shade_kind, const void *vox_native, ColsAux *aux, int *status_word,
                           const char **why, hipStream_t s);

#include <functional>
int smk_host_pool_size();
void smk_host_pool_run(int n, const std::function<void(int)> &f);

struct SmkVolGeom {
  int dtype = 0, nelts = 0, dmode = 0;
  int N[3] = {0, 0, 0};
  float fs[3] = {0, 0, 0};
  int g0[3] = {0, 0, 0}, g1[3] = {0, 0, 0}, O[3] = {0, 0, 0}, D[3] = {0, 0, 0}, nbr[3] = {0, 0, 0};
  bool grad = false, padded = false;
  size_t vox_bytes = 0, nrm_bytes = 0, mm_bytes = 0;
};
int smk_volume_geometry(smk_ctx *c, const char *who, const smk_volume_desc *b, int nb, int nelts, smk_dtype dtype,
                        smk_datamode dmode, SmkVolGeom &g);
void smk_set_geometry(smk_ctx *c, const SmkVolGeom &g);
int smk_alloc_step(smk_ctx *c, const SmkVolGeom &g, TimeStep &T);
int smk_pack_step(smk_ctx *c, const char *who, const SmkVolGeom &g, const smk_volume_desc *b, int nb, bool on_device, TimeStep &T,
                  hipStream_t s);
void smk_use_step(smk_ctx *c, int k);

template <class T>
static int read_back(smk_ctx *c, T *h, const T *d, size_t n) {
  HIPCHK(c, hipDeviceSynchronize());
  HIPCHK(c, hipMemcpy(h, d, n * sizeof(T), hipMemcpyDeviceToHost));
  return 0;
}

#pragma GCC visibility push(hidden)
int smk_build_params(smk_ctx *c, RenderParams &P, hipStream_t s);
int smk_shade_kind(const smk_ctx *c);
void smk_region_box(const smk_ctx *c, const int g0[3], const int g1[3], float lo[3], float hi[3], int top[3]);
void smk_shard_region(const smk_ctx *c, int rank, int g0[3], int g1[3]);
void smk_bsp_order(const smk_ctx *c, const double pos[3], int *order);
void smk_inverse_affine(double inv[16], const double m[16]);
int smk_make_xmajor_copy(smk_ctx *c);
int smk_frame_buffers(smk_ctx *c);
void smk_slab_free(SlabAux *aux);
void host_ray_at(const RenderParams &P, double px, double py, double A[3], double B[3]);
int smk_cols_stat(smk_ctx *c, const char *name, double *value);
int smk_shadow_setup(smk_ctx *c, RenderParams &P, smk_shadowcoef &sc, SmkShadowShard *S, int *halo_need);
int smk_shadow_light_owned(smk_ctx *c, RenderParams &P, smk_shadowcoef &sc, float olo[3], float ohi[3]);
int smk_shadow_frame(smk_ctx *c, RenderParams &P, void *d_rgba, void *d_depth, hipStream_t s, bool *marched);
bool smk_shadow_light_along_view(const smk_ctx *c);
int smk_clip_slice_stage(smk_ctx *c, const RenderParams &P, hipStream_t s);
#pragma GCC visibility pop

int smk_step_wait_ready(smk_ctx *c, hipStream_t s);
int smk_step_mark_used(smk_ctx *c, hipStream_t s);
void smk_free_steps(smk_ctx *c);
```

simian-spacemonkey_amd/csrc/smk_shadow_plan.hip:

```cpp
#include <math.h>
#include <stdio.h>
#include <string.h>

#include <algorithm>

#include "smk_internal.h"

static double dot3d(const double a[3], const double b[3]) { return a[0] * b[0] + a[1] * b[1] + a[2] * b[2]; }

static bool view_and_light(const smk_ctx *c, double vd[3], double ld[3], double *light_dist, double *vdl) {
  for (int k = 0; k < 3; ++k) {
    vd[k] = (double)c->at[k] - c->eye[k];
    ld[k] = -(double)c->light_pos[k];
  }
  const double vl = sqrt(dot3d(vd, vd)), d0 = sqrt(dot3d(ld, ld));
  if (!(vl > 0) || !(d0 > 0)) return false;
  for (int k = 0; k < 3; ++k) {
    vd[k] /= vl;
    ld[k] /= d0;
  }
  *light_dist = d0;
  *vdl = dot3d(vd, ld);
  return true;
}
// ... 159 lines not shown
    HIPCHK(c, hipDeviceSynchronize());
    HIPCHK(c, hipMemcpy(rgba_out, c->d_light_last, (size_t)c->light_lb * c->light_lb * 16, hipMemcpyDeviceToHost));
  }
  return 0;
}

extern "C" int smk_shard_light_order(smk_ctx *c, int *order) {
  if (!c || !order) return 1;
  if (!c->have_volume || !c->have_camera) FAIL(c, "smk_shard_light_order: volume and camera must be set");
  smk_shadowcoef sc;
  if (compute_shadowcoef(c, &sc)) return 1;
  const double l[3] = {sc.Lc[0], sc.Lc[1], sc.Lc[2]};
  smk_bsp_order(c, l, order);
  return 0;
}

static int shadow_margin(const smk_shadowcoef &sc, const int g0[3], const int g1[3]) {
  double worst = 0.0;
  const int n = 8;
  for (int iz = 0; iz <= n; ++iz)
    for (int iy = 0; iy <= n; ++iy)
      for (int ix = 0; ix <= n; ++ix) {
        const int ii[3] = {ix, iy, iz};
        double p[3];
        for (int a = 0; a < 3; ++a) p[a] = (double)g0[a] - 0.5 + (double)(g1[a] - g0[a]) * ii[a] / n;
        const double lw = sc.Wm[0] * p[0] + sc.Wm[1] * p[1] + sc.Wm[2] * p[2] + sc.Wm[3];
        if (!(fabs(lw) > 1e-30)) return 1 << 20;
        const double lx = (sc.Xm[0] * p[0] + sc.Xm[1] * p[1] + sc.Xm[2] * p[2] + sc.Xm[3]) / lw * sc.lscale + sc.lbias;
        const double ly = (sc.Ym[0] * p[0] + sc.Ym[1] * p[1] + sc.Ym[2] * p[2] + sc.Ym[3]) / lw * sc.lscale + sc.lbias;
        const double a = lx * sc.las + sc.lal, b = ly * sc.las + sc.lal;
        double G[3], d[3], gg = 0.0, dg = 0.0;
        for (int q = 0; q < 3; ++q) {
          G[q] = a * sc.Gx[q] + b * sc.Gy[q] + sc.Gc[q];
          d[q] = p[q] - sc.Lc[q];
          gg += G[q] * G[q];
          dg += d[q] * G[q];
        }
        const double nG = a * sc.nGx + b * sc.nGy + sc.nGc;
        if (!(gg > 0.0) || !(fabs(nG) > 1e-30)) return 1 << 20;
        const double w = dg / gg;
        for (int q = 0; q < 3; ++q) {
          const double ja = w * (sc.Gx[q] - G[q] * sc.nGx / nG), jb = w * (sc.Gy[q] - G[q] * sc.nGy / nG);
          worst = std::max(worst, (double)sc.las * (fabs(ja) + fabs(jb)));
        }
      }
  const double m = ceil(1.5 * worst + 0.5);
  return m > (double)(1 << 20) || m != m ? 1 << 20 : std::max(1, (int)m);
}

int smk_shadow_setup(smk_ctx *c, RenderParams &P, smk_shadowcoef &sc, SmkShadowShard *S, int *halo_need) {
  if (compute_shadowcoef(c, &sc)) return 1;
  SmkShadowRays &h = P.sh;
  memset(&h, 0, sizeof h);
  h.on = 1;
  for (int a = 0; a < 3; ++a) { h.Ec[a] = sc.Ec[a]; h.Dc[a] = sc.Dc[a]; h.Dx[a] = sc.Dx[a]; h.Dy[a] = sc.Dy[a]; }
  h.nDc = sc.nDc; h.nDx = sc.nDx; h.nDy = sc.nDy;
  if (sc.front_to_back) { h.numA = fmaf(1.0f, sc.dnum, sc.num0); h.dB = sc.dnum; h.k0 = 1; h.dk = 1; }
  else { h.numA = fmaf((float)sc.nslices, sc.dnum, sc.num0); h.dB = -sc.dnum; h.k0 = sc.nslices; h.dk = -1; }
  h.LB = sc.LB;
  for (int q = 0; q < 4; ++q) { h.Xm[q] = sc.Xm[q]; h.Ym[q] = sc.Ym[q]; h.Wm[q] = sc.Wm[q]; }
  h.lscale = sc.lscale; h.lbias = sc.lbias;
  {
    smk_raycoef &rc = P.rc;
    memset(&rc, 0, sizeof rc);
    rc.pxs = sc.pxs; rc.pxl = sc.pxl; rc.pys = sc.pys; rc.pyl = sc.pyl;
    rc.nplanes = sc.nslices;
    const double nDc = (double)sc.nDc != 0.0 ? (double)sc.nDc : 1.0;
    for (int a = 0; a < 3; ++a) rc.Bc[a] = (float)((double)h.dB / nDc * (double)sc.Dc[a]);
  }
  float wlo[3], whi[3];
  int wtop[3];
  const int z0[3] = {0, 0, 0};
  smk_region_box(c, z0, c->N, wlo, whi, wtop);
  float olo[3], ohi[3];
  for (int a = 0; a < 3; ++a) {
    const bool inner_lo = c->g0[a] > 0 && P.lo[a] == (float)c->g0[a] - 0.5f, inner_hi = !P.top[a];
    h.llo[a] = wlo[a] - SMK_SHADOW_BOX_EPS;
    h.lhi[a] = whi[a] + SMK_SHADOW_BOX_EPS;
    olo[a] = inner_lo ? P.lo[a] : P.lo[a] - SMK_SHADOW_BOX_EPS;
    ohi[a] = inner_hi ? nextafterf(P.hi[a], -INFINITY) : P.hi[a] + SMK_SHADOW_BOX_EPS;
    if (!inner_lo) P.lo[a] -= SMK_SHADOW_BOX_EPS;
    if (inner_hi) P.hin[a] = nextafterf(P.hi[a], -INFINITY);
    else {
      P.hi[a] += SMK_SHADOW_BOX_EPS;
      P.hin[a] = P.hi[a];
      P.top[a] = 1;
    }
  }
  if (!S) return 0;
  memset(S, 0, sizeof *S);
  S->nranks = c->nranks;
  S->rank = c->rank;
  for (int a = 0; a < 3; ++a) { S->olo[a] = olo[a]; S->ohi[a] = ohi[a]; }
  int m_own = 0;
  for (int j = 0; j < c->nranks; ++j) {
    int g0[3], g1[3];
    smk_shard_region(c, j, g0, g1);
    const int m = shadow_margin(sc, g0, g1);
    if (j == c->rank) m_own = m;
    for (int a = 0; a < 3; ++a) {
      S->glo[j][a] = (float)((double)g0[a] - 0.5 - m);
      S->ghi[j][a] = (float)((double)g1[a] - 0.5 + m);
    }
  }
  for (int a = 0; a < 3; ++a) {
    S->xlo[a] = S->glo[c->rank][a] - 0.25f;
    S->xhi[a] = S->ghi[c->rank][a] + 0.25f;
  }
  const double l[3] = {sc.Lc[0], sc.Lc[1], sc.Lc[2]};
  smk_bsp_order(c, l, S->order);
  if (halo_need) *halo_need = m_own + 1;
  return 0;
}

static int shadow_refusals(smk_ctx *c, const RenderParams &P) {
  const int sk = smk_shade_kind(c);
  if (c->tf_mode == 0) FAIL(c, "smk_render: shadows need a 2-D or 3-D transfer function (the 1-D table renderer has no shadow mode)");
  if (sk == 2) FAIL(c, "smk_render: shadows are implemented for R8k shading or none (NV20 combiners: no shadow mode in NV20VolRen3D)");
  if (c->nranks > 1 && (!c->opt_shadow_march || (c->opt_lockstep & 256)))
    FAIL(c, "smk_render: shadows need the whole volume on one GPU with option shadow_march 0 or shadow_fused (the light buffer couples every "
            "slice of every brick); a shard renders shadows with the two marches only");
  if (P.pert_on || c->region_on) FAIL(c, "smk_render: shadows cannot be combined with perturbation or a sub-box");
  if (c->opt_kernel == 3) FAIL(c, "smk_render: the column-stream kernel has no shadow mode");
  return 0;
}

static int shadow_halo_check(smk_ctx *c, int need) {
  for (int a = 0; a < 3; ++a)
    if (c->halo < need && c->D[a] < c->N[a])
      FAIL(c, "smk_render: shadows on a shard need halo >= %d voxels (have %d; margin %d, smk_get_shadow_margin); set option 'halo' before upload",
           need, c->halo, need - 1);
  return 0;
}

static bool light_history_fits(smk_ctx *c, size_t nhist) {
  if (nhist <= c->light_hist_cap) return true;
  size_t fr = 0, tot = 0;
  if (c->d_light_hist) (void)hipFree(c->d_light_hist);
  c->d_light_hist = nullptr;
  c->light_hist_cap = 0;
  c->d_light_last = nullptr;
  if (hipMemGetInfo(&fr, &tot) != hipSuccess || nhist * 16 > fr / 4 || nhist * 16 > ((size_t)32 << 30) ||
      hipMalloc((void **)&c->d_light_hist, nhist * 16) != hipSuccess) {
    (void)hipGetLastError();
    c->d_light_hist = nullptr;
    return false;
  }
  c->light_hist_cap = nhist;
  return true;
}

static int light_march(smk_ctx *c, RenderParams &P, const smk_shadowcoef &sc, const SmkShadowShard &S, size_t hstride, hipStream_t s) {
  HIPCHK(c, hipEventRecord(c->ev0, s));
  hipError_t e = c->nranks > 1 ? smk_launch_shadow_march_shard(P, sc, c->dtype, c->tf_mode, c->d_light_hist, (long long)hstride, S, s)
                               : smk_launch_shadow_march(P, sc, c->dtype, c->tf_mode, c->d_light_hist, (long long)hstride, s);
  if (e == hipErrorNotSupported) FAIL(c, "smk_render: no shadow kernel instance for this configuration");
  HIPCHK(c, e);
  P.sh.hist = c->d_light_hist;
  P.sh.hstride = (long long)hstride;
  c->light_hist_n = sc.nslices + 1;
  c->light_hist_stride = (long long)hstride;
  c->d_light_last = c->d_light_hist + (size_t)sc.nslices * hstride;
  c->last_alg_bytes += (double)sc.nslices * (16.0 * (double)((size_t)sc.LB * sc.LB));
  return 0;
}

static int launch_per_slice(smk_ctx *c, const RenderParams &P, const smk_shadowcoef &sc, void *d_rgba, void *d_depth, hipStream_t s) {
  const size_t nl = (size_t)sc.LB * sc.LB;
  if (nl > c->light_cap) {
    for (int k = 0; k < 2; ++k) {
      if (c->d_light[k]) (void)hipFree(c->d_light[k]);
      c->d_light[k] = nullptr;
      HIPCHK(c, hipMalloc((void **)&c->d_light[k], nl * 16));
    }
    c->light_cap = nl;
    c->d_light_last = nullptr;
  }
  HIPCHK(c, hipEventRecord(c->ev0, s));
  HIPCHK(c, hipMemsetAsync(c->d_light[0], 0, nl * 16, s));
  HIPCHK(c, hipMemsetAsync(d_rgba, 0, (size_t)c->W * c->H * 16, s));
  if (d_depth) HIPCHK(c, hipMemsetD32Async((hipDeviceptr_t)d_depth, 0x7f800000, (size_t)c->W * c->H, s));
  if (!c->d_shadow_barrier) HIPCHK(c, hipMalloc((void **)&c->d_shadow_barrier, 16 * 9 * 4));
  hipError_t e = smk_launch_shadow(P, sc, c->dtype, c->tf_mode, smk_shade_kind(c), c->d_light[0], c->d_light[1], c->d_shadow_barrier, s);
  if (e == hipErrorNotSupported) FAIL(c, "smk_render: no shadow kernel instance for this configuration");
  HIPCHK(c, e);
  c->d_light_last = c->d_light[sc.nslices & 1];
  c->last_alg_bytes += (double)sc.nslices * (32.0 * (double)nl);
  c->last_kernel = 3;
  return 0;
}

int smk_shadow_frame(smk_ctx *c, RenderParams &P, void *d_rgba, void *d_depth, hipStream_t s, bool *marched) {
  const int sk = smk_shade_kind(c);
  if (c->nranks > 1 && !c->shadow_entries_fresh && c->tf_mode != 0 && sk != 2)
    FAIL(c, "smk_render: shadows need the whole volume on one GPU (the light buffer couples every slice of every brick) -- "
            "or, on a shard, this frame's light entries: smk_shadow_exports_device on every rank, then smk_shadow_entries_device "
            "(smk_shadow_exchange_local in one process)");
  const bool entries = c->shadow_entries_fresh;
  c->shadow_entries_fresh = false;
  if (shadow_refusals(c, P)) return 1;
  smk_shadowcoef sc;
  SmkShadowShard S;
  int halo_need = 0;
  if (smk_shadow_setup(c, P, sc, c->nranks > 1 ? &S : nullptr, &halo_need)) return 1;
  if (c->nranks > 1) {
    if (shadow_halo_check(c, halo_need)) return 1;
    if (!entries || memcmp(&sc, &c->shadow_entries_sc, sizeof sc))
      FAIL(c, "smk_render: shadows on a shard: the light entries were made for another slice set (camera, light or buffer changed since)");
    S.entries = c->d_shadow_entries;
  }
  P.blend = SMK_BLEND_FRONT_TO_BACK;
  const size_t hstride = (size_t)sc.LB * sc.LB + 272;
  const size_t nhist = hstride * ((size_t)sc.nslices + 1);
  *marched = c->opt_shadow_march && !(c->opt_lockstep & 256) && sc.nslices > 0 && light_history_fits(c, nhist);
  c->light_lb = sc.LB;
  c->light_hist_n = 0;
  if (c->nranks > 1 && !*marched)
    FAIL(c, "smk_render: shadows on a shard: the light history (%.1f GB) does not fit a quarter of the free device memory",
         (double)nhist * 16.0 / 1e9);
  return *marched ? light_march(c, P, sc, S, hstride, s) : launch_per_slice(c, P, sc, d_rgba, d_depth, s);
}

float4 *smk_shadow_entries_reserve(smk_ctx *c, int LB) {
  const size_t n = (size_t)c->nranks * LB * LB;
  if (n > c->shadow_entries_cap) {
    if (c->d_shadow_entries) (void)hipFree(c->d_shadow_entries);
    c->d_shadow_entries = nullptr;
    c->shadow_entries_cap = 0;
    if (hipMalloc((void **)&c->d_shadow_entries, n * 16) != hipSuccess) {
      (void)hipGetLastError();
      c->d_shadow_entries = nullptr;
      return nullptr;
    }
    c->shadow_entries_cap = n;
  }
  c->shadow_entries_fresh = false;
  return c->d_shadow_entries;
}

void smk_shadow_entries_commit(smk_ctx *c, const smk_shadowcoef &sc) {
  c->shadow_entries_sc = sc;
  c->shadow_entries_fresh = true;
}

int smk_shadow_shard_setup(smk_ctx *c, RenderParams &P, smk_shadowcoef &sc, SmkShadowShard &S, hipStream_t s) {
  if (!c->shadow_on) FAIL(c, "smk_shadow_exports_device: shadows are off (smk_set_shadow)");
  if (smk_build_params(c, P, s)) return 1;
  if (shadow_refusals(c, P)) return 1;
  int need = 0;
  if (smk_shadow_setup(c, P, sc, &S, &need)) return 1;
  if (shadow_halo_check(c, need)) return 1;
  return 0;
}

extern "C" int smk_shadow_exports_device(smk_ctx *c, void *d_exports, void *stream) {
  if (!c) return 1;
  HIPCHK(c, hipSetDevice(c->device));
  if (!d_exports) FAIL(c, "smk_shadow_exports_device: null output");
  hipStream_t s = stream ? (hipStream_t)stream : c->stream;
  RenderParams P;
  smk_shadowcoef sc;
  SmkShadowShard S;
  if (smk_shadow_shard_setup(c, P, sc, S, s)) return 1;
  S.exports = (float4 *)d_exports;
  hipError_t e = smk_launch_shadow_exports(P, sc, c->dtype, c->tf_mode, S, s);
  if (e == hipErrorNotSupported) FAIL(c, "smk_shadow_exports_device: no shadow kernel instance for this configuration");
  HIPCHK(c, e);
  return smk_step_mark_used(c, s);
}

extern "C" int smk_shadow_entries_device(smk_ctx *c, const void *d_entries, void *stream) {
  if (!c) return 1;
  HIPCHK(c, hipSetDevice(c->device));
  if (!d_entries) FAIL(c, "smk_shadow_entries_device: null input");
  if (!c->have_volume || !c->have_camera) FAIL(c, "smk_shadow_entries_device: volume and camera must be set");
  hipStream_t s = stream ? (hipStream_t)stream : c->stream;
  smk_shadowcoef sc;
  if (compute_shadowcoef(c, &sc)) return 1;
  float4 *d = smk_shadow_entries_reserve(c, sc.LB);
  if (!d) FAIL(c, "smk_shadow_entries_device: device allocation failed");
  HIPCHK(c, hipMemcpyAsync(d, d_entries, (size_t)c->nranks * sc.LB * sc.LB * 16, hipMemcpyDeviceToDevice, s));
  smk_shadow_entries_commit(c, sc);
  return 0;
}

extern "C" int smk_get_shadow_margin(smk_ctx *c, int *m, int *halo_needed) {
  if (!c) return 1;
  if (!c->have_volume || !c->have_camera) FAIL(c, "smk_get_shadow_margin: volume and camera must be set");
  smk_shadowcoef sc;
  if (compute_shadowcoef(c, &sc)) return 1;
  const int mm = shadow_margin(sc, c->g0, c->g1);
  if (m) *m = mm;
  if (halo_needed) *halo_needed = mm + 1;
  return 0;
}

int smk_shadow_light_owned(smk_ctx *c, RenderParams &P, smk_shadowcoef &sc, float olo[3], float ohi[3]) {
  if (!c->shadow_on) FAIL(c, "smk_get_stat: light_samples needs shadows on (smk_set_shadow)");
  if (smk_build_params(c, P, c->stream)) return 1;
  SmkShadowShard S;
  if (smk_shadow_setup(c, P, sc, &S, nullptr)) return 1;
  for (int a = 0; a < 3; ++a) { olo[a] = S.olo[a]; ohi[a] = S.ohi[a]; }
  return 0;
}

extern "C" int smk_shadow_exchange_local(smk_ctx *const *all, int nranks) {
  if (!all || nranks < 1 || nranks > SMK_MAX_RANKS) return 1;
  for (int r = 0; r < nranks; ++r) {
    if (!all[r]) return 1;
    if (all[r]->nranks != nranks || all[r]->rank != r) FAIL(all[r], "smk_shadow_exchange_local: context %d is not shard %d of %d", r, r, nranks);
  }
  std::vector<smk_shadowcoef> scs(nranks);
  for (int r = 0; r < nranks; ++r) {
    smk_ctx *c = all[r];
    HIPCHK(c, hipSetDevice(c->device));
    HIPCHK(c, hipStreamSynchronize(c->stream));
    RenderParams P;
    SmkShadowShard S;
    if (smk_shadow_shard_setup(c, P, scs[r], S, c->stream)) return 1;
    if (r > 0 && memcmp(&scs[r], &scs[0], sizeof scs[0])) FAIL(c, "smk_shadow_exchange_local: the ranks' slice sets differ (camera, light, buffer or volume)");
    const size_t n = (size_t)nranks * scs[r].LB * scs[r].LB;
    if (n > c->shadow_exports_cap) {
      if (c->d_shadow_exports) (void)hipFree(c->d_shadow_exports);
      c->d_shadow_exports = nullptr;
      c->shadow_exports_cap = 0;
      HIPCHK(c, hipMalloc((void **)&c->d_shadow_exports, n * 16));
      c->shadow_exports_cap = n;
    }
    S.exports = c->d_shadow_exports;
    hipError_t e = smk_launch_shadow_exports(P, scs[r], c->dtype, c->tf_mode, S, c->stream);
    if (e == hipErrorNotSupported) FAIL(c, "smk_shadow_exchange_local: no shadow kernel instance for this configuration");
    HIPCHK(c, e);
  }
  const size_t nl = (size_t)scs[0].LB * scs[0].LB;
// ... 35 lines not shown
```

simian-spacemonkey_amd/csrc/smk_slab.h:

```cpp
#pragma once

#include "smk_internal.h"

struct SlabParams {
  int perm;
  int au, av, as;
  long long strideV, strideS;
  int Ou, Ov, Os;
  int Du, Dv, Ds;
  int wu;
  int wv;
  int wp;
  int per, rpg;
  int groups;
  int mask_need;
  int chunks;
  int slot_bytes;
  int nslots;
  int maxfly;
  int wstep;
  int pmask;
  int dir;
  int tw, th;
  const void *vox;
  int use_ah;
  int use_occ;
  int fast_tf;
  const unsigned char *bricks;
  int bsu, bsv, bss;
  const int2 *order;
  unsigned *tile_ticks;
  int ntiles;
  int *status;
  int status_tag;
  float *diag;
  unsigned *trace;
  float4 *seg_out;
  unsigned *piece_ticks;
};

struct SlabEnt {
  int base;
  unsigned pack;
};

#define SLAB_EPS 0.02f

constexpr int SLAB_BIG_WAVES = 12;
constexpr bool slab_big(int nw, int nl) { return nw + nl > SLAB_BIG_WAVES; }
constexpr int SLAB_BIG_NLG = 2;
constexpr int slab_loader_groups(int nw, int nl) { return slab_big(nw, nl) ? ((nl % SLAB_BIG_NLG) == 0 ? SLAB_BIG_NLG : 1) : nl; }

hipError_t smk_slab_dispatch_u8(const RenderParams &P, const SlabParams &Q, int tf_mode, int shade_kind, int nw, int nl, bool diag, size_t lds,
                                int nblocks, const char **why, hipStream_t s);
hipError_t smk_slab_dispatch_f32(const RenderParams &P, const SlabParams &Q, int tf_mode, int shade_kind, int nw, int nl, bool diag, size_t lds,
                                 int nblocks, const char **why, hipStream_t s);
hipError_t smk_slab_dispatch_shadow(const RenderParams &P, const SlabParams &Q, int dtype, int tf_mode, int shade_kind, int nw, int nl, size_t lds,
                                    int nblocks, const char **why, hipStream_t s);
hipError_t smk_slab_dispatch_occluded(const RenderParams &P, const SlabParams &Q, int dtype, int tf_mode, int shade_kind, int nw, int nl, size_t lds,
                                      int nblocks, const char **why, hipStream_t s);
hipError_t smk_slab_dispatch_occluded_shadow(const RenderParams &P, const SlabParams &Q, int dtype, int tf_mode, int shade_kind, int nw, int nl,
                                             size_t lds, int nblocks, const char **why, hipStream_t s);
hipError_t smk_slab_merge(const int2 *list, int n, int tw, int th, int ntx, int W, int H, const float4 *seg_out, float4 *out, int use_max,
                          hipStream_t s);
```

simian-spacemonkey_amd/csrc/smk_slab.hip:

```cpp
#include <math.h>
#include <stdio.h>
#include <stdlib.h>
#include <string.h>

#include <algorithm>
#include <functional>
#include <type_traits>

#include "smk_device.h"
#include "smk_slab.h"

#define SLAB_DONE 0x3fffffff
constexpr int SLAB_POLL_SLEEP = 2;

template <int DT>
struct VoxT;
template <>
struct VoxT<0> {
  typedef uint2 type;
};
template <>
struct VoxT<1> {
  typedef float4 type;
};
// ... 965 lines not shown
            }
            hit = col.w != 0.0f;
          } else if (TF == 2 && Q.use_occ) {
            int s0, s1, t0, t1;
            float fs, ft;
            smk_lin_clamp(__fmaf_rn(ch0, (float)P.s3v, -0.5f), P.s3v, s0, s1, fs);
            smk_lin_clamp(__fmaf_rn(ch1, (float)P.s3g, -0.5f), P.s3g, t0, t1, ft);
            col.w = 0.0f;
            hit = false;
            if ((occ[__mul24(t0, P.occ_roww) + (s0 >> 5)] >> (s0 & 31)) & 1u) {
              ch2 = tri_h_early();
              hit = smk_classify<DT, TF>(P, ch0, ch1, ch2, ch3, col);
            }
          } else {
            hit = smk_classify<DT, TF>(P, ch0, ch1, ch2, ch3, col);
          }
          d_hit = hit;
          if (hit) {
            if (TF == 1 && Q.fast_tf) {
              col.x = slab_tex_chan(tx4, 0);
              col.y = slab_tex_chan(tx4, 1);
              col.z = slab_tex_chan(tx4, 2);
            }
            float4 src;
            float shadow[3];
            const float *shp = nullptr;
            if (TF != 0 && SHD) {
              const float mf = (float)m;
              smk_shadow_term(P, m, __fmaf_rn(mf, B[0], A[0]), __fmaf_rn(mf, B[1], A[1]), __fmaf_rn(mf, B[2], A[2]), shadow);
              shp = shadow;
            }
            if (TF == 0) {
              src = col;
            } else if (SH == 0) {
              src = smk_shade_sample<0>(P, col, 0.f, 0.f, 0.f, 0.f, shp);
            } else {
              uint32_t nb[8];
              if constexpr (EARLY) {
#pragma unroll
                for (int k = 0; k < 8; ++k) {
                  if constexpr (DT == 1) nb[k] = __float_as_uint(rq[k].w);
                  else nb[k] = rq[k].y;
                }
              } else if (DT == 1) slab_read8_nb16(a0, a0 + pitch_b, b0, b0 + pitch_b, nb);
              else slab_read8_nb8(a0, a0 + pitch_b, b0, b0 + pitch_b, nb);
#define NB(dx, dy, dz) nb[QI(dx, dy, dz)]
              float n0 = smk_nrm(NB(0, 0, 0), NB(1, 0, 0), NB(0, 1, 0), NB(1, 1, 0), NB(0, 0, 1), NB(1, 0, 1), NB(0, 1, 1), NB(1, 1, 1), 0, fx, fy, fz);
              float n1 = smk_nrm(NB(0, 0, 0), NB(1, 0, 0), NB(0, 1, 0), NB(1, 1, 0), NB(0, 0, 1), NB(1, 0, 1), NB(0, 1, 1), NB(1, 1, 1), 1, fx, fy, fz);
              float n2 = smk_nrm(NB(0, 0, 0), NB(1, 0, 0), NB(0, 1, 0), NB(1, 1, 0), NB(0, 0, 1), NB(1, 0, 1), NB(0, 1, 1), NB(1, 1, 1), 2, fx, fy, fz);
#undef NB
              src = smk_shade_sample<SH>(P, col, n0, n1, n2, ch1, shp);
            }
            if (P.depth != nullptr && C3 == 0.0f) P.depth[(size_t)j * P.W + i] = smk_plane_depth_px<SHD>(P, m, px, py);
            if (P.blend == SMK_BLEND_MAX) {
              C0 = fmaxf(C0, src.x);
              C1 = fmaxf(C1, src.y);
              C2 = fmaxf(C2, src.z);
              C3 = fmaxf(C3, src.w);
            } else {
              float w = 1.0f - C3;
              C0 = __fmaf_rn(w, src.x, C0);
              C1 = __fmaf_rn(w, src.y, C1);
              C2 = __fmaf_rn(w, src.z, C2);
              C3 = __fmaf_rn(w, src.w, C3);
              if (C3 == 1.0f) m1 = m;
            }
          }
#undef QI
        }
        if (act) {
          m = m_next;
          if constexpr (EARLY) {
            if (m <= m1) {
              car_sc = early_nsc;
              car_i = early_ni;
              pb = __mul24(psgn, car_i) + poff;
            } else pb = SLAB_DONE;
          } else if (m <= m1) {
            car_i = base_slice_c(m, car_sc);
            pb = __mul24(psgn, car_i) + poff;
          } else pb = SLAB_DONE;
        }
        if (count) {
          n_it += 1.f;
          n_act += (float)__popcll(__ballot(act));
          n_in += (float)__popcll(__ballot(work));
          n_hit += (float)__popcll(__ballot(d_hit));
          n_anyhit += __any(d_hit) ? 1.f : 0.f;
          n_work += __any(work) ? 1.f : 0.f;
          n_own += __any(work && d_own) ? 1.f : 0.f;
        }
        }
      }
      if (lane == 0) lds_st(&ctl[8 + wave], SLAB_DONE);
      if (tracing && lane == 0) atomicAdd(Q.trace + 8 * (size_t)blockIdx.x + 7, (unsigned)n_it);
      if (count && lane == 0) {
        atomicAdd(&Q.diag[0], n_it);
        atomicAdd(&Q.diag[1], n_act);
        atomicAdd(&Q.diag[2], n_in);
        atomicAdd(&Q.diag[3], n_hit);
        atomicAdd(&Q.diag[8], n_anyhit);
        atomicAdd(&Q.diag[14], n_work);
        atomicAdd(&Q.diag[15], n_own);
        atomicAdd(&Q.diag[9], n_lead);
        atomicAdd(&Q.diag[10], n_waits);
        atomicAdd(&Q.diag[11], n_wstep);
        atomicAdd(&Q.diag[12], (float)max(npos - min(pos, npos), 0) / (float)max(npos, 1));
        atomicAdd(&Q.diag[13], 1.0f);
      }
    }
  }
  if (live) {
    size_t o = (size_t)j * P.W + i;
    float4 *outp = seg == 0 ? P.out : Q.seg_out + (size_t)(seg - 1) * ((size_t)P.W * P.H);
    outp[o] = make_float4(C0, C1, C2, C3);
    if (P.depth != nullptr && C3 == 0.0f) P.depth[o] = __int_as_float(0x7f800000);
  }
  if (npos > 0) {
    __syncthreads();
    if (tid == 0 && ctl[3]) *(volatile int *)Q.status = Q.status_tag | ctl[3];
  }
  if (tid == 0 && Q.tile_ticks && nseg > 1) {
    const unsigned dur = max((unsigned)__builtin_amdgcn_s_memrealtime() - trace_t0, 1u);
    if (Q.piece_ticks) Q.piece_ticks[(size_t)tile * 8 + seg] = dur;
    atomicAdd(&Q.tile_ticks[tile], dur);
    atomicAdd(&Q.tile_ticks[Q.ntiles + tile], npos > 0 ? (unsigned)max(min(max(min(min(ctl[4], ctl[5]), min(ctl[6], ctl[7])), 0), npos + 1) - ctl[2], 0) : 0u);
    atomicAdd(&Q.tile_ticks[2 * Q.ntiles + tile], npos > 0 ? (unsigned)(npos + 1) : 0u);
  } else if (tid == 0 && Q.tile_ticks) {
    Q.tile_ticks[tile] = max((unsigned)__builtin_amdgcn_s_memrealtime() - trace_t0, 1u);
    Q.tile_ticks[Q.ntiles + tile] = npos > 0 ? (unsigned)max(min(max(min(min(ctl[4], ctl[5]), min(ctl[6], ctl[7])), 0), npos + 1) - ctl[2], 0) : 0u;
    Q.tile_ticks[2 * Q.ntiles + tile] = npos > 0 ? (unsigned)(npos + 1) : 0u;
    Q.tile_ticks[3 * Q.ntiles + tile] = trace_t0;
    Q.tile_ticks[4 * Q.ntiles + tile] = (__builtin_amdgcn_s_getreg((31 << 11) | 4) & 0xff00u) | (__builtin_amdgcn_s_getreg((31 << 11) | 20) & 0xfu);
  }
  if (tracing && tid == 0) {
    unsigned *t = Q.trace + 8 * (size_t)blockIdx.x;
    if (phases) {
      t[4] = ph1;
      t[5] = ph2;
      t[6] = ph3;
    }
    t[0] = trace_t0;
    t[1] = (unsigned)__builtin_amdgcn_s_memrealtime();
    t[2] = __builtin_amdgcn_s_getreg((31 << 11) | 4);
    t[3] = (__builtin_amdgcn_s_getreg((31 << 11) | 20) & 0xf) | ((unsigned)tile << 8) | ((unsigned)max(npos, 0) << 20);
  }
}


#ifndef SLAB_PART
#define SLAB_PART 0
#endif
#if SLAB_PART == 0
__global__ __launch_bounds__(256) void smk_k_slab_merge(const int2 *list, int tw, int th, int ntx, int W, int H, const float4 *seg_out, float4 *out, int use_max) {
  const int code = list[blockIdx.x].x;
  const int tile = code & 0xfffff, nseg = code >> 20;
  const int ty = tile / ntx, tx = tile - ty * ntx;
  const size_t npix = (size_t)W * H;
  for (int p = threadIdx.x; p < tw * th; p += blockDim.x) {
    const int i = tx * tw + p % tw, j = ty * th + p / tw;
    if (i >= W || j >= H) continue;
    const size_t o = (size_t)j * W + i;
    float4 C = out[o];
    for (int k = 1; k < nseg; ++k) {
      const float4 sgm = seg_out[(size_t)(k - 1) * npix + o];
      if (use_max) {
        C = make_float4(fmaxf(C.x, sgm.x), fmaxf(C.y, sgm.y), fmaxf(C.z, sgm.z), fmaxf(C.w, sgm.w));
      } else {
        const float w = 1.0f - C.w;
        C.x = __fmaf_rn(w, sgm.x, C.x);
        C.y = __fmaf_rn(w, sgm.y, C.y);
        C.z = __fmaf_rn(w, sgm.z, C.z);
        C.w = __fmaf_rn(w, sgm.w, C.w);
      }
    }
    out[o] = C;
  }
}
hipError_t smk_slab_merge(const int2 *list, int n, int tw, int th, int ntx, int W, int H, const float4 *seg_out, float4 *out, int use_max,
                          hipStream_t s) {
  hipLaunchKernelGGL(smk_k_slab_merge, dim3(n), dim3(256), 0, s, list, tw, th, ntx, W, H, seg_out, out, use_max);
  return hipGetLastError();
}
#endif

template <int DT, int SH, int PERM, int NW, int NL, bool DIAG, int TF = 1, bool BR = true, bool SHD = false, bool OCC = false>
static hipError_t launch_slab(const RenderParams &P, const SlabParams &Q, size_t lds, int nblocks, hipStream_t s) {
  auto k = smk_k_slab<DT, SH, PERM, NW, NL, DIAG, TF, BR, SHD, OCC>;
  static bool attr_set[64] = {};
  int dev = 0;
  (void)hipGetDevice(&dev);
  if (dev < 0 || dev >= 64 || !attr_set[dev]) {
    hipError_t e = hipFuncSetAttribute((const void *)k, hipFuncAttributeMaxDynamicSharedMemorySize, 160 * 1024);
    if (e != hipSuccess) return e;
    if (dev >= 0 && dev < 64) attr_set[dev] = true;
  }
  hipLaunchKernelGGL(k, dim3(nblocks), dim3((NW + NL) * 64), lds, s, P, Q);
  return hipGetLastError();
}

#if SLAB_PART == 3 || SLAB_PART == 4
#if SLAB_PART == 3
hipError_t smk_slab_dispatch_occluded(const RenderParams &P, const SlabParams &Q, int dtype, int tf_mode, int shade_kind, int nw, int nl, size_t lds,
                                      int nblocks, const char **why, hipStream_t s) {
#define GO(D, S, R, N, L)                                                                              \
  if (dtype == D && shade_kind == S && Q.perm == R && nw == N && nl == L) {                          \
    if (tf_mode == 2) return (launch_slab<D, S, R, N, L, false, 2, true, false, true>(P, Q, lds, nblocks, s)); \
    if (tf_mode == 1) return (launch_slab<D, S, R, N, L, false, 1, true, false, true>(P, Q, lds, nblocks, s)); \
    if constexpr (S == 0) return (launch_slab<D, S, R, N, L, false, 0, false, false, true>(P, Q, lds, nblocks, s)); \
    *why = "no colour-table instance with this shading";                                               \
    return hipErrorNotSupported;                                                                     \
  }
#define GO_R(D, S) GO_NW(D, S, 0) GO_NW(D, S, 1) GO_NW(D, S, 2)
#define GO_NW(D, S, R) GO(D, S, R, 8, 2) GO(D, S, R, 10, 2) GO(D, S, R, 12, 4)
  GO_R(0, 0) GO_R(0, 1) GO_R(0, 2) GO_R(1, 0) GO_R(1, 1) GO_R(1, 2)
#else
hipError_t smk_slab_dispatch_occluded_shadow(const RenderParams &P, const SlabParams &Q, int dtype, int tf_mode, int shade_kind, int nw, int nl,
                                             size_t lds, int nblocks, const char **why, hipStream_t s) {
#define GO(D, S, R, N, L)                                                                              \
  if (dtype == D && shade_kind == S && Q.perm == R && nw == N && nl == L) {                          \
    if (tf_mode == 2) return (launch_slab<D, S, R, N, L, false, 2, true, true, true>(P, Q, lds, nblocks, s)); \
    if (tf_mode == 1) return (launch_slab<D, S, R, N, L, false, 1, true, true, true>(P, Q, lds, nblocks, s)); \
    *why = "shadows need a 2-D or 3-D table";                                                        \
    return hipErrorNotSupported;                                                                     \
  }
#define GO_R(D, S) GO_NW(D, S, 0) GO_NW(D, S, 1) GO_NW(D, S, 2)
#define GO_NW(D, S, R) GO(D, S, R, 8, 2) GO(D, S, R, 10, 2) GO(D, S, R, 12, 4)
  GO_R(0, 0) GO_R(0, 1) GO_R(1, 0) GO_R(1, 1)
#endif
#undef GO_R
#undef GO_NW
#undef GO
  *why = "no scene-depth instance for this configuration";
  return hipErrorNotSupported;
}
#elif SLAB_PART == 2
hipError_t smk_slab_dispatch_shadow(const RenderParams &P, const SlabParams &Q, int dtype, int tf_mode, int shade_kind, int nw, int nl, size_t lds,
                                    int nblocks, const char **why, hipStream_t s) {
#define GO(D, S, R, N, L)                                                                                  \
  if (dtype == D && shade_kind == S && Q.perm == R && nw == N && nl == L) {                              \
    if (tf_mode == 2) {                                                                                  \
      if (Q.bricks) return (launch_slab<D, S, R, N, L, false, 2, true, true>(P, Q, lds, nblocks, s));    \
      return (launch_slab<D, S, R, N, L, false, 2, false, true>(P, Q, lds, nblocks, s));                 \
    }                                                                                                    \
    if (tf_mode == 1) {                                                                                  \
      if (Q.bricks) return (launch_slab<D, S, R, N, L, false, 1, true, true>(P, Q, lds, nblocks, s));    \
      return (launch_slab<D, S, R, N, L, false, 1, false, true>(P, Q, lds, nblocks, s));                 \
    }                                                                                                    \
    *why = "shadows need a 2-D or 3-D table";                                                            \
    return hipErrorNotSupported;                                                                         \
  }
#define GO_NW(D, S, R) GO(D, S, R, 8, 2) GO(D, S, R, 10, 2) GO(D, S, R, 12, 4)
#define GO_R(D, S) GO_NW(D, S, 0) GO_NW(D, S, 1) GO_NW(D, S, 2)
  GO_R(0, 0) GO_R(0, 1) GO_R(1, 0) GO_R(1, 1)
#undef GO_R
#undef GO_NW
#undef GO
  *why = "no shadow instance for this configuration";
  return hipErrorNotSupported;
}
#else
#if SLAB_PART == 0
hipError_t smk_slab_dispatch_u8(const RenderParams &P, const SlabParams &Q, int tf_mode, int shade_kind, int nw, int nl, bool diag, size_t lds,
                                int nblocks, const char **why, hipStream_t s) {
  const int dtype = 0;
#else
hipError_t smk_slab_dispatch_f32(const RenderParams &P, const SlabParams &Q, int tf_mode, int shade_kind, int nw, int nl, bool diag, size_t lds,
                                 int nblocks, const char **why, hipStream_t s) {
  const int dtype = 1;
#endif
  (void)diag;
#define GO(D, S, R, N, L)                                                                              \
  if (dtype == D && shade_kind == S && Q.perm == R && nw == N && nl == L) {                          \
    if (tf_mode == 2) {                                                                              \
      if constexpr ((N == 8 && L == 2) || (N == 10 && L == 2) || (N == 12 && L == 4)) {              \
        if (Q.bricks) return (launch_slab<D, S, R, N, L, false, 2, true>(P, Q, lds, nblocks, s));  \
        return (launch_slab<D, S, R, N, L, false, 2, false>(P, Q, lds, nblocks, s));     \
      }                                                                                              \
      *why = "no dense-3-D-table instance for this tile size";                                       \
      return hipErrorNotSupported;                                                                   \
    }                                                                                                \
    if (tf_mode == 0) {                                                                              \
      if constexpr (S == 0 && ((N == 8 && L == 2) || (N == 10 && L == 2) || (N == 12 && L == 4)))    \
        return (launch_slab<D, S, R, N, L, false, 0, false>(P, Q, lds, nblocks, s));     \
      *why = "no colour-table instance for this tile size";                                          \
      return hipErrorNotSupported;                                                                   \
    }                                                                                                \
    if constexpr (D == 1 && S == 1) {                                                                \
      if (diag) return (launch_slab<D, S, R, N, L, true>(P, Q, lds, nblocks, s));        \
    }                                                                                                \
    if (Q.bricks) return (launch_slab<D, S, R, N, L, false, 1, true>(P, Q, lds, nblocks, s));  \
    return (launch_slab<D, S, R, N, L, false, 1, false>(P, Q, lds, nblocks, s));         \
  }
#define GO_NW(D, S, R) GO(D, S, R, 8, 2) GO(D, S, R, 10, 2) GO(D, S, R, 12, 4)
#define GO_R(D, S) GO_NW(D, S, 0) GO_NW(D, S, 1) GO_NW(D, S, 2)
#if SLAB_PART == 0
  GO_R(0, 0) GO_R(0, 1) GO_R(0, 2)
#else
  GO_R(1, 0) GO_R(1, 1) GO_R(1, 2)
#endif
#undef GO_R
#undef GO_NW
#undef GO
  *why = "no kernel instance for this tile size";
  return hipErrorNotSupported;
}
#endif
```

simian-spacemonkey_amd/csrc/smk_slab_plan.hip:

```cpp
#include <math.h>
#include <stdio.h>
#include <stdlib.h>
#include <string.h>
#include <time.h>

#include <algorithm>
#include <vector>

#include "smk_slab.h"

void host_ray_at(const RenderParams &P, double px, double py, double A[3], double B[3]) {
  const smk_raycoef &rc = P.rc;
  if (!P.sh.on) {
    for (int a = 0; a < 3; ++a) {
      A[a] = px * rc.Ax[a] + py * rc.Ay[a] + rc.Ac[a];
      B[a] = px * rc.Bx[a] + py * rc.By[a] + rc.Bc[a];
    }
    return;
  }
  const SmkShadowRays &sh = P.sh;
  const double nD = px * sh.nDx + py * sh.nDy + sh.nDc, tauA = sh.numA / nD, dtau = sh.dB / nD;
  for (int a = 0; a < 3; ++a) {
    const double D = px * sh.Dx[a] + py * sh.Dy[a] + sh.Dc[a];
    A[a] = sh.Ec[a] + tauA * D;
// ... 336 lines not shown
    int g = 64, r = wp;
    while (r) { int t = g % r; g = r; r = t; }
    per = wp / g;
    rpg = 64 / g;
    groups = (Q.wv + rpg - 1) / rpg;
  };
  int wp8 = (Q.wu + 7) & ~7, per8, rpg8, gr8;
  shape(wp8, per8, rpg8, gr8);
  Q.wp = wp8; Q.per = per8; Q.rpg = rpg8;
  const int wp4 = (Q.wu + 3) & ~3;
  if (wp4 != wp8) {
    int per4, rpg4, gr4;
    shape(wp4, per4, rpg4, gr4);
    if (per4 <= 7 && gr4 * per4 < gr8 * per8) { Q.wp = wp4; Q.per = per4; Q.rpg = rpg4; }
  }
  Q.groups = (Q.wv + Q.rpg - 1) / Q.rpg;
  if (!big && Q.groups * Q.rpg <= Q.Dv) Q.wv = Q.groups * Q.rpg;
  Q.chunks = Q.groups * Q.per;
  return nullptr;
}

static const char *slab_size_shape(RenderParams &P, SlabParams &Q, SlabShape sh, int dtype, bool sparse, bool last, SlabAux *aux,
                                   std::vector<int> &work) {
  Q.tw = sh.tw;
  Q.th = sh.th;
  P.ntx = (P.W + sh.tw - 1) / sh.tw;
  P.nty = (P.H + sh.th - 1) / sh.th;
  P.tiles_per_xcd = (P.ntx * P.nty + 7) / 8;
  double m[4];
  const char *why = slab_scan(P, Q, sparse, aux, m, work);
  return why ? why : slab_window(P, Q, dtype, slab_big(slab_waves(sh), sh.nl), m, last);
}

static const char *slab_probe(RenderParams P, SlabParams Q, int dtype, SlabAux *aux, int *best) {
  double best_score = 1e300;
  int best_wu = 0;
  std::vector<int> work;
  *best = -1;
  for (int ci = 0; ci < 3; ++ci) {
    const SlabShape sh = SLAB_CAND[ci];
    const char *why = slab_size_shape(P, Q, sh, dtype, true, false, aux, work);
    if (why == SLAB_NEXT) continue;
    if (why) return why;
    const int nw = slab_waves(sh);
    const double score = (double)Q.chunks / (nw * 64) * (nw + sh.nl < 12 ? 1.4 : 1.0);
    if (score < best_score || (score == best_score && Q.wu > best_wu)) { best_score = score; *best = ci; best_wu = Q.wu; }
  }
  return nullptr;
}

static const char *slab_ring(const RenderParams &P, SlabParams &Q, SlabShape sh, int tf_mode, double ds, const SlabAux *aux, bool last,
                             size_t *lds) {
  const int nw = slab_waves(sh), nl = sh.nl;
  const bool big = slab_big(nw, nl);
  Q.slot_bytes = Q.chunks * 1024;
  Q.mask_need = Q.chunks >= 4 ? 1 : 0;
  const int nlg = slab_loader_groups(nw, nl), lpg = nl / nlg;
  const int mych = (Q.groups + lpg - 1) / lpg * Q.per;
  if (mych > 63) return last ? "window needs more than 63 DMA chunks per loader" : SLAB_NEXT;
  if (!last && (double)Q.chunks * 1024.0 / (nw * 64) > 16.0 * nl) return SLAB_NEXT_BIG;
  Q.use_ah = (tf_mode == 1 && P.third_axis && P.nelts <= 3 && P.sv >= 2 && P.sv <= 2048) ? 1 : 0;
  if (tf_mode == 1 && (P.sv < 2 || P.sg < 2)) return "transfer function smaller than 2x2";
  const size_t occ_bytes = tf_mode == 1 ? (size_t)P.occ_roww * P.sg * 4 : tf_mode == 2 ? (size_t)P.occ_roww * P.s3g * 4 : 0;
  Q.fast_tf = (tf_mode == 1 && (!P.third_axis || Q.use_ah)) ? 1 : 0;
  Q.use_occ = ((Q.fast_tf || tf_mode == 2) && Q.mask_need && P.tf_occ && occ_bytes > 0 && occ_bytes <= 8192) ? 1 : 0;
  {
    Q.bricks = (tf_mode == 1 || tf_mode == 2) ? P.bricks : nullptr;
    const int bst[3] = {1, P.nbr[0], P.nbr[0] * P.nbr[1]};
    Q.bsu = bst[Q.au];
    Q.bsv = bst[Q.av];
    Q.bss = bst[Q.as];
  }
  const size_t fixed = (size_t)Q.Ds * sizeof(SlabEnt) + (8 + 32) * 4 + 64 + (Q.use_ah ? (size_t)P.sv * 4 : 0) + (Q.use_occ ? occ_bytes : 0);
  const size_t budget = big ? 158 * 1024 : 78 * 1024;
  if (budget <= fixed) return "slice table does not fit LDS";
  int ns = (int)((budget - fixed) / (size_t)Q.slot_bytes);
  if (ns > 24) ns = 24;
  const int band = (int)ceil(ds) + 2;
  if (ns < band + 2 && 158 * 1024 > fixed) {
    if (!last && budget < 158 * 1024) return SLAB_NEXT;
    ns = (int)((158 * 1024 - fixed) / (size_t)Q.slot_bytes);
    if (ns > band + 4) ns = band + 4;
  }
  if (aux->opt_ns >= 3 && ns > aux->opt_ns) ns = aux->opt_ns;
  if (ns < 3) return last ? "window does not fit LDS" : SLAB_NEXT;
  Q.nslots = ns;
  if (Q.bricks && (size_t)ns * Q.slot_bytes < ((size_t)((Q.Ds - 1) >> SMK_BRICK_LOG2) + 1) * 16) Q.bricks = nullptr;
  Q.maxfly = std::max(1, std::min(std::min(ns, 63 / mych + 1), aux->opt_fly > 0 ? aux->opt_fly : (nlg > 1 && !big ? 1 : 2)));
  Q.wstep = std::max(0, std::min((int)ceil(ds), ns - 4));
  if (aux->opt_T > 0) Q.wstep = std::max(0, std::min(aux->opt_T - 1, ns - 3));
  Q.pmask = ns >= 2 * band ? 1 : 0;
  *lds = (size_t)ns * Q.slot_bytes + fixed;
  if (getenv("SMK_DEBUG"))
    fprintf(stderr, "[smk] slice-ring plan: tile %dx%d, %d+%d waves, window %d units x %d rows (pitch %d units), %d chunks/slice, %d slots of %d B, table+ctl %zu B, LDS %zu B, band %d, wstep %d, pmask %d, maxfly %d\n",
            sh.tw, sh.th, nw, nl, Q.wu, Q.wv, Q.wp, Q.chunks, ns, Q.slot_bytes, fixed, *lds, band, Q.wstep, Q.pmask, Q.maxfly);
  return nullptr;
}

static const char *slab_choose_shape(RenderParams &P, SlabParams &Q, int dtype, int tf_mode, double ds, SlabAux *aux, SlabShape &shape,
                                     size_t *lds, std::vector<int> &work) {
  SlabShape list[3] = {{32, 16, 2}, SLAB_BIG_SHAPE, SLAB_BIG_SHAPE};
  int n = 2;
  const bool choose = aux->opt_tile == 0;
  if (!choose) {
    const auto *t = std::find_if(std::begin(SLAB_TILE_OPTION), std::end(SLAB_TILE_OPTION), [&](const auto &o) { return o.id == aux->opt_tile; });
    if (t == std::end(SLAB_TILE_OPTION)) return "no kernel instance for this tile size";
    list[0] = t->sh;
    n = 1;
  }
  struct ShapeKey { int as, dir, W, H, dtype, N[3]; float lo[3], hi[3]; } skey;
  memset(&skey, 0, sizeof skey);
  skey.as = Q.as; skey.dir = Q.dir; skey.W = P.W; skey.H = P.H; skey.dtype = dtype;
  for (int a = 0; a < 3; ++a) { skey.N[a] = P.N[a]; skey.lo[a] = P.lo[a]; skey.hi[a] = P.hi[a]; }
  const bool shape_known = choose && aux->shape_key.size() == sizeof skey && !memcmp(aux->shape_key.data(), &skey, sizeof skey) &&
                           aux->shape_choice >= 0 && ++aux->shape_age < 64;
  int best = shape_known ? aux->shape_choice : -1;
  const char *why = choose && !shape_known ? slab_probe(P, Q, dtype, aux, &best) : nullptr;
  if (why) return why;
  int alt = -1;
  if (best >= 0) {
    alt = best == 0 ? 1 : 0;
    list[0] = SLAB_CAND[best];
    list[1] = SLAB_CAND[alt];
    list[2] = SLAB_BIG_SHAPE;
    n = 3;
    if (!shape_known) {
      aux->shape_key.assign(reinterpret_cast<const unsigned char *>(&skey), reinterpret_cast<const unsigned char *>(&skey) + sizeof skey);
      aux->shape_choice = best;
      aux->shape_age = 0;
    }
  }
  for (int ci = 0; ci < n; ++ci) {
    shape = list[ci];
    const bool last = ci + 1 == n;
    why = slab_size_shape(P, Q, shape, dtype, false, last, aux, work);
    if (!why && choose && best >= 0 && ci == 0) {
      if (shape_known && aux->shape_chunks != Q.chunks) aux->shape_age = 64;
      if (!shape_known) aux->shape_chunks = Q.chunks;
    }
    if (!why) why = slab_ring(P, Q, shape, tf_mode, ds, aux, last, lds);
    if (why == SLAB_NEXT_BIG && alt >= 0 && ci == 0) ci = 1;
    if (why == SLAB_NEXT || why == SLAB_NEXT_BIG) continue;
    if (why) return why;
    if (choose && alt >= 0 && ci == 1) {
      aux->shape_choice = alt;
      aux->shape_chunks = Q.chunks;
      aux->shape_age = 0;
    }
    return nullptr;
  }
  return "no configuration fits";
}

static hipError_t slab_measured_weights(SlabAux *aux, long long tsig, int nt, std::vector<int> &work, SlabParams &Q) {
  ++aux->ticks_age;
  if (aux->ticks_pending && aux->ticks_stale && hipEventQuery(aux->ticks_ev) == hipSuccess) {
    aux->ticks_pending = aux->ticks_stale = false;
  }
  if (aux->ticks_pending && hipEventQuery(aux->ticks_ev) == hipSuccess) {
    const bool fresh = aux->ticks_good_sig != aux->ticks_pending_sig;
    const int due = aux->ticks_adopted < 3 ? (4 << aux->ticks_adopted) : 32;
    if (fresh || aux->ticks_age >= due) {
      if (fresh || (int)aux->ticks_good.size() != aux->ticks_pending_n) {
        aux->ticks_good.assign(aux->h_ticks, aux->h_ticks + aux->ticks_pending_n);
        aux->ticks_adopted = 0;
      } else {
        unsigned longest_new = 0;
        for (int t = 0; t < aux->ticks_pending_n; ++t) longest_new = std::max(longest_new, aux->h_ticks[t]);
        for (int t = 0; t < aux->ticks_pending_n; ++t)
          aux->ticks_good[t] = longest_new < 10000u ? (aux->h_ticks[t] ? std::min(std::max(aux->ticks_good[t], 1u), aux->h_ticks[t]) : aux->ticks_good[t])
                                                    : (aux->ticks_good[t] + aux->h_ticks[t] + 1) / 2;
        ++aux->ticks_adopted;
      }
      aux->ticks_good_sig = aux->ticks_pending_sig;
      aux->ticks_age = 0;
      if (aux->h_pticks && (int)aux->cuts_pending.size() == aux->ticks_pending_n * 10) {
        aux->pticks_good.assign(aux->h_pticks, aux->h_pticks + (size_t)aux->ticks_pending_n * 8);
        aux->cuts_good = aux->cuts_pending;
      }
      aux->recut = true;
    }
    aux->ticks_pending = false;
  }
  (void)hipGetLastError();
  if (aux->ticks_good_sig == tsig && (int)aux->ticks_good.size() == nt) {
    for (int t = 0; t < nt; ++t)
      if (aux->ticks_good[t] > 0) work[t] = (int)std::min<unsigned>(aux->ticks_good[t], 1u << 30);
  }
  if (nt > aux->ticks_cap) {
    if (aux->ticks_pending) (void)hipEventSynchronize(aux->ticks_ev);
    aux->ticks_pending = aux->ticks_stale = false;
    if (aux->d_ticks) (void)hipFree(aux->d_ticks);
    if (aux->h_ticks) (void)hipHostFree(aux->h_ticks);
    if (aux->d_pticks) (void)hipFree(aux->d_pticks);
    if (aux->h_pticks) (void)hipHostFree(aux->h_pticks);
    aux->d_ticks = aux->h_ticks = aux->d_pticks = aux->h_pticks = nullptr;
    aux->ticks_cap = 0;
    hipError_t e = hipMalloc((void **)&aux->d_ticks, (size_t)nt * 20);
    if (e == hipSuccess) e = hipMemset(aux->d_ticks, 0, (size_t)nt * 20);
    if (e == hipSuccess) e = hipHostMalloc((void **)&aux->h_ticks, (size_t)nt * 4, hipHostMallocDefault);
    if (e == hipSuccess) e = hipMalloc((void **)&aux->d_pticks, (size_t)nt * 32);
    if (e == hipSuccess) e = hipMemset(aux->d_pticks, 0, (size_t)nt * 32);
    if (e == hipSuccess) e = hipHostMalloc((void **)&aux->h_pticks, (size_t)nt * 32, hipHostMallocDefault);
    if (e != hipSuccess) return e;
    aux->ticks_cap = nt;
  }
  if (!aux->ticks_ev) {
    hipError_t e = hipEventCreateWithFlags(&aux->ticks_ev, hipEventDisableTiming);
    if (e != hipSuccess) return e;
  }
  Q.tile_ticks = aux->d_ticks;
  Q.piece_ticks = aux->d_pticks;
  Q.ntiles = nt;
  aux->ticks_n_last = nt;
  return hipSuccess;
}

void smk_slab_forget_measurements(SlabAux *aux) {
  aux->ticks_good.clear();
  aux->ticks_good_sig = -1;
  aux->ticks_adopted = 0;
  aux->ticks_stale = aux->ticks_pending;
  aux->pticks_good.clear();
  aux->cuts_good.clear();
  aux->cuts.clear();
  aux->cuts_sig = -1;
  aux->cuts_engaged = false;
  aux->recut = true;
}

void smk_slab_free(SlabAux *aux) {
  for (void *p : {(void *)aux->d_diag, (void *)aux->d_order, (void *)aux->d_pticks, aux->d_seg, (void *)aux->d_trace, (void *)aux->d_ticks})
    if (p) (void)hipFree(p);
  for (void *p : {(void *)aux->h_status, (void *)aux->h_pticks, (void *)aux->h_ticks, (void *)aux->h_order[0], (void *)aux->h_order[1],
                  (void *)aux->h_order[2], (void *)aux->h_order[3]})
    if (p) (void)hipHostFree(p);
  for (hipEvent_t e : {aux->order_ev[0], aux->order_ev[1], aux->order_ev[2], aux->order_ev[3], aux->ticks_ev})
    if (e) (void)hipEventDestroy(e);
}

static void slab_cut_segments(SlabAux *aux, const std::vector<int> &work, int nt, long long tsig, int opt_split, bool big) {
  const bool measured = aux->ticks_good_sig == tsig && (int)aux->ticks_good.size() == nt;
  if ((int)aux->cuts.size() != nt * 10 || aux->cuts_split != opt_split || aux->cuts_sig != tsig) {
    aux->cuts.assign((size_t)nt * 10, 0);
    for (int t = 0; t < nt; ++t) { aux->cuts[(size_t)t * 10] = 1; aux->cuts[(size_t)t * 10 + 2] = 255; }
    aux->cuts_split = opt_split;
    aux->cuts_sig = tsig;
    aux->recut = true;
  }
  if (aux->recut) {
    aux->recut = false;
    auto equal_cuts = [&](int t, int K) {
      unsigned char *c = &aux->cuts[(size_t)t * 10];
      c[0] = (unsigned char)K;
      for (int k = 0; k <= K; ++k) c[1 + k] = (unsigned char)(255 * k / K);
    };
    if (opt_split >= 2) {
      for (int t = 0; t < nt; ++t) equal_cuts(t, std::min(opt_split, 8));
    } else if (opt_split == 0 && measured) {
      long long total = 0;
      for (int t = 0; t < nt; ++t) total += work[t];
      const double wg_slots = 256.0 * (big ? 1 : 2);
      const double mean_load = (double)total / wg_slots;
      double longest_tile = 0;
      for (int t = 0; t < nt; ++t) longest_tile = std::max(longest_tile, (double)work[t]);
      const double piece = std::max(0.75 * mean_load, 6000.0);
      bool big_frame = mean_load >= 5000.0 && longest_tile > 1.5 * mean_load;
      if (aux->cuts_engaged && mean_load >= 5000.0 && longest_tile > 1.2 * mean_load) big_frame = true;
      aux->cuts_engaged = big_frame;
      const bool have_pieces = (int)aux->pticks_good.size() == nt * 8 && (int)aux->cuts_good.size() == nt * 10;
      for (int t = 0; t < nt; ++t) {
        unsigned char *c = &aux->cuts[(size_t)t * 10];
        int Kw = (big_frame && (double)work[t] > 1.25 * piece) ? (int)std::min(8.0, ceil((double)work[t] / piece)) : 1;
        if (big_frame && c[0] >= 2 && Kw >= 1 && abs(Kw - (int)c[0]) <= 1 && (double)work[t] > piece) Kw = c[0];
        if (Kw == 1) { equal_cuts(t, 1); continue; }
        const unsigned char *g = have_pieces ? &aux->cuts_good[(size_t)t * 10] : nullptr;
        const int Kg = g ? g[0] : 1;
        if (!g || Kg < 2) {
          if (c[0] != Kw) equal_cuts(t, Kw);
          continue;
        }
        double d[8], tot = 0, longest = 0;
        for (int k = 0; k < Kg; ++k) {
          d[k] = std::max(1.0, (double)aux->pticks_good[(size_t)t * 8 + k] - 1300.0);
          tot += d[k];
          longest = std::max(longest, d[k]);
        }
        const bool same = !memcmp(g, c, 10);
        if (same && Kg == Kw && longest <= 1.3 * tot / Kg) continue;
        unsigned char nc[10] = {(unsigned char)Kw, 0};
        int k = 0;
        double acc = 0;
        for (int j = 1; j < Kw; ++j) {
          const double want = tot * j / Kw;
          while (k < Kg - 1 && acc + d[k] < want) acc += d[k++];
          const double f = d[k] > 0 ? (want - acc) / d[k] : 0.5;
          int x = (int)lround(g[1 + k] + f * (g[2 + k] - g[1 + k]));
          x = std::max(x, (int)nc[j] + 1);
          x = std::min(x, 255 - (Kw - j));
          nc[1 + j] = (unsigned char)x;
        }
        nc[1 + Kw] = 255;
        memcpy(c, nc, 10);
      }
    } else {
      for (int t = 0; t < nt; ++t) equal_cuts(t, 1);
    }
  }
}

static void slab_schedule(const RenderParams &P, SlabAux *aux, const std::vector<int> &work, int slots, std::vector<int2> &order) {
  const int nt = P.ntx * P.nty;
  if (aux->plan_slots == slots && aux->plan_work == work && aux->plan_cuts == aux->cuts && !aux->plan_order.empty()) {
    order = aux->plan_order;
    return;
  }
  std::vector<unsigned char> ksplit((size_t)nt, 1);
  for (int t = 0; t < nt; ++t) ksplit[t] = aux->cuts[(size_t)t * 10];
  auto piece_weight = [&](int t, int k) -> int {
    const unsigned char *c = &aux->cuts[(size_t)t * 10];
    if ((int)aux->pticks_good.size() == nt * 8 && (int)aux->cuts_good.size() == nt * 10 && !memcmp(&aux->cuts_good[(size_t)t * 10], c, 10) &&
        aux->pticks_good[(size_t)t * 8 + k] > 0)
      return (int)std::min<unsigned>(aux->pticks_good[(size_t)t * 8 + k], 1u << 30);
    return work[t] / std::max<int>(c[0], 1);
  };
  std::vector<std::vector<int>> run(8);
  std::vector<int> ws;
  ws.reserve((size_t)nt);
  for (int t = 0; t < nt; ++t)
    if (work[t] > 0) ws.push_back(work[t]);
  std::sort(ws.begin(), ws.end());
  const bool even = ws.size() >= 16 && (long long)ws[ws.size() * 95 / 100] * 4 <= (long long)ws[ws.size() / 2] * 5;
  const int SLAB_DEAL_W = even ? 4 : 2, SLAB_DEAL_H = even ? 4 : 2;
  const int gbx = (P.ntx + SLAB_DEAL_W - 1) / SLAB_DEAL_W, gby = (P.nty + SLAB_DEAL_H - 1) / SLAB_DEAL_H;
  std::vector<long long> gw((size_t)gbx * gby, 0);
  for (int t = 0; t < nt; ++t) gw[(size_t)((t / P.ntx) / SLAB_DEAL_H) * gbx + (t % P.ntx) / SLAB_DEAL_W] += work[t];
  std::vector<int> idx((size_t)gbx * gby);
  for (int g = 0; g < gbx * gby; ++g) idx[g] = g;
  std::stable_sort(idx.begin(), idx.end(), [&](int a, int b) { return gw[a] > gw[b]; });
  long long load[8] = {0, 0, 0, 0, 0, 0, 0, 0};
  for (int g : idx) {
    int x = 0;
    for (int k = 1; k < 8; ++k)
      if (load[k] < load[x]) x = k;
    const int gy = g / gbx, gx = g - gy * gbx;
    for (int dy = 0; dy < SLAB_DEAL_H; ++dy)
      for (int dx = 0; dx < SLAB_DEAL_W; ++dx) {
        const int ty = gy * SLAB_DEAL_H + dy, tx = gx * SLAB_DEAL_W + dx;
        if (ty < P.nty && tx < P.ntx) run[x].push_back(ty * P.ntx + tx);
      }
    load[x] += gw[g];
  }
  for (int x = 0; x < 8; ++x)
    std::stable_sort(run[x].begin(), run[x].end(), [&](int a, int b) { return work[a] / ksplit[a] > work[b] / ksplit[b]; });
  size_t longest = 0;
  std::vector<std::vector<std::pair<int, int2>>> items(8);
  for (int x = 0; x < 8; ++x) {
    for (int t : run[x]) {
      const unsigned char *c = &aux->cuts[(size_t)t * 10];
      for (int k = 0; k < c[0]; ++k)
        items[x].push_back({piece_weight(t, k), make_int2(t | (k << 20) | ((int)c[0] << 26), (int)c[1 + k] | ((int)c[2 + k] << 8))});
    }
    std::stable_sort(items[x].begin(), items[x].end(), [](const std::pair<int, int2> &a, const std::pair<int, int2> &b) { return a.first > b.first; });
    longest = std::max(longest, items[x].size());
  }
  order.assign(longest * 8, make_int2(-1, 0));
  for (int x = 0; x < 8; ++x)
    for (size_t k = 0; k < items[x].size(); ++k) order[k * 8 + x] = items[x][k].second;
  int nsplit = 0;
  for (int t = 0; t < nt; ++t)
    if (ksplit[t] > 1) { order.push_back(make_int2(t | ((int)ksplit[t] << 20), 0)); ++nsplit; }
  order.push_back(make_int2(nsplit, 0));
  aux->plan_work = work;
  aux->plan_cuts = aux->cuts;
  aux->plan_order = order;
  aux->plan_slots = slots;
}

static hipError_t slab_segments(const RenderParams &P, SlabParams &Q, SlabAux *aux, const std::vector<int2> &order, int *nblocks) {
  const int nt = P.ntx * P.nty;
  const int nsplit = order.back().x;
  *nblocks = (int)order.size() - 1 - nsplit;
  aux->ksplit_last.assign((size_t)nt, 1);
  int maxseg = 1;
  for (int k = 0; k < nsplit; ++k) {
    const int code = order[(size_t)*nblocks + k].x;
    aux->ksplit_last[code & 0xfffff] = (unsigned char)(code >> 20);
    maxseg = std::max(maxseg, code >> 20);
  }
  aux->nsplit_last = nsplit;
  aux->nblocks_last = *nblocks;
  if (maxseg > 1) {
    const size_t need = (size_t)(8 - 1) * P.W * P.H * 16;
    if (need > aux->seg_cap) {
      if (aux->d_seg) (void)hipFree(aux->d_seg);
      aux->d_seg = nullptr;
      aux->seg_cap = 0;
      hipError_t e = hipMalloc(&aux->d_seg, need);
      if (e != hipSuccess) return e;
      aux->seg_cap = need;
    }
  }
  Q.seg_out = (float4 *)aux->d_seg;
  return hipSuccess;
}

static hipError_t slab_upload_order(SlabAux *aux, std::vector<int2> &order, hipStream_t s) {
  if (aux->frame_ev0) {
    hipError_t e = hipEventRecord(aux->frame_ev0, s);
    if (e != hipSuccess) return e;
  }
  auto same_order = [&]() { return aux->order_host.size() == order.size() && (order.empty() || !memcmp(aux->order_host.data(), order.data(), order.size() * sizeof(int2))); };
  if (!same_order()) {
    if ((int)order.size() > aux->order_cap) {
      if (aux->d_order) (void)hipFree(aux->d_order);
      aux->d_order = nullptr;
      for (int k = 0; k < 4; ++k) {
        if (aux->order_ev[k]) (void)hipEventSynchronize(aux->order_ev[k]);
        if (aux->h_order[k]) (void)hipHostFree(aux->h_order[k]);
        aux->h_order[k] = nullptr;
      }
      aux->order_cap = 0;
      const size_t cap = order.size() * 2 + 1024;
      hipError_t e = hipMalloc((void **)&aux->d_order, cap * sizeof(int2));
      for (int k = 0; k < 4 && e == hipSuccess; ++k) e = hipHostMalloc((void **)&aux->h_order[k], cap * sizeof(int2), hipHostMallocDefault);
      if (e != hipSuccess) return e;
      aux->order_cap = (int)cap;
    }
    const int k = aux->order_next;
    aux->order_next = (k + 1) & 3;
    hipError_t e = aux->order_ev[k] ? hipEventSynchronize(aux->order_ev[k]) : hipEventCreateWithFlags(&aux->order_ev[k], hipEventDisableTiming);
    if (e != hipSuccess) return e;
    memcpy(aux->h_order[k], order.data(), order.size() * sizeof(int2));
    e = hipMemcpyAsync(aux->d_order, aux->h_order[k], order.size() * sizeof(int2), hipMemcpyHostToDevice, s);
    if (e != hipSuccess) return e;
    e = hipEventRecord(aux->order_ev[k], s);
    if (e != hipSuccess) return e;
    aux->order_host.swap(order);
  }
  return hipSuccess;
}

static hipError_t slab_trace(const RenderParams &P, SlabParams &Q, SlabAux *aux, int nblocks, hipStream_t s) {
  Q.trace = nullptr;
  if (!(P.lockstep & 32)) return hipSuccess;
  if (nblocks > aux->trace_cap) {
    if (aux->d_trace) (void)hipFree(aux->d_trace);
    aux->d_trace = nullptr;
    aux->trace_cap = 0;
    hipError_t e = hipMalloc((void **)&aux->d_trace, (size_t)nblocks * 32);
    if (e != hipSuccess) return e;
    aux->trace_cap = nblocks;
  }
  hipError_t e = hipMemsetAsync(aux->d_trace, 0, (size_t)nblocks * 32, s);
  if (e != hipSuccess) return e;
  aux->trace_n = nblocks;
  Q.trace = aux->d_trace;
  return hipSuccess;
}

static hipError_t slab_run(const RenderParams &P, const SlabParams &Q, SlabAux *aux, int dtype, int tf_mode, int shade_kind, SlabShape sh,
                           size_t lds, int nblocks, long long tsig, const char **why, hipStream_t s) {
  const int nw = slab_waves(sh), nt = Q.ntiles, nsplit = aux->nsplit_last;
  const bool diag = (P.lockstep & ~1) != 0 && dtype == 1 && shade_kind == 1;
  hipError_t e = nsplit > 0 ? hipMemsetAsync(aux->d_ticks, 0, (size_t)nt * 20, s) : hipSuccess;
  if (e != hipSuccess) return e;
  if (!aux->merge_warm && nblocks >= 1) {
    aux->merge_warm = true;
    static const int2 one = make_int2(0 | (1 << 20), 0);
    int2 *d_one = nullptr;
    if (hipMalloc((void **)&d_one, sizeof one) == hipSuccess) {
      if (hipMemcpyAsync(d_one, &one, sizeof one, hipMemcpyHostToDevice, s) == hipSuccess)
        (void)smk_slab_merge(d_one, 1, sh.tw, sh.th, P.ntx, P.W, P.H, (const float4 *)P.out, P.out, 0, s);
      (void)hipStreamSynchronize(s);
      (void)hipFree(d_one);
    }
    (void)hipGetLastError();
  }
  e = P.zscene   ? (P.sh.on ? smk_slab_dispatch_occluded_shadow(P, Q, dtype, tf_mode, shade_kind, nw, sh.nl, lds, nblocks, why, s)
                             : smk_slab_dispatch_occluded(P, Q, dtype, tf_mode, shade_kind, nw, sh.nl, lds, nblocks, why, s))
      : P.sh.on    ? smk_slab_dispatch_shadow(P, Q, dtype, tf_mode, shade_kind, nw, sh.nl, lds, nblocks, why, s)
      : dtype == 0 ? smk_slab_dispatch_u8(P, Q, tf_mode, shade_kind, nw, sh.nl, diag, lds, nblocks, why, s)
                   : smk_slab_dispatch_f32(P, Q, tf_mode, shade_kind, nw, sh.nl, diag, lds, nblocks, why, s);
  if (e == hipSuccess && nsplit > 0)
    e = smk_slab_merge(aux->d_order + nblocks, nsplit, sh.tw, sh.th, P.ntx, P.W, P.H, (const float4 *)aux->d_seg, P.out,
                       P.blend == SMK_BLEND_MAX ? 1 : 0, s);
  if (e != hipSuccess || aux->ticks_pending) return e;
  e = hipMemcpyAsync(aux->h_ticks, aux->d_ticks, (size_t)nt * 4, hipMemcpyDeviceToHost, s);
  if (e == hipSuccess && nsplit > 0) e = hipMemcpyAsync(aux->h_pticks, aux->d_pticks, (size_t)nt * 32, hipMemcpyDeviceToHost, s);
  if (nsplit > 0) aux->cuts_pending = aux->cuts; else aux->cuts_pending.clear();
  if (e == hipSuccess) e = hipEventRecord(aux->ticks_ev, s);
  if (e != hipSuccess) return e;
  aux->ticks_pending = true;
  aux->ticks_pending_sig = tsig;
  aux->ticks_pending_n = nt;
  return hipSuccess;
}

static hipError_t slab_plan_and_launch(RenderParams &P, int dtype, int tf_mode, int shade_kind, const void *vox_native, const void *vox_xmajor,
                                       SlabAux *aux, const char **why, hipStream_t s) {
  const double t0 = slab_clock.on ? slab_now() : 0;
  slab_clock.frame_scan = 0;
  SlabParams Q;
  memset(&Q, 0, sizeof Q);
  Q.status = aux->h_status + aux->status_slot;
  Q.status_tag = aux->status_tag;
  Q.diag = aux->d_diag;
  const double ds = slab_axes(P, vox_native, vox_xmajor, Q);
  if ((*why = slab_refusal(P, dtype, tf_mode, Q))) return hipErrorNotSupported;
  if (tf_mode == 0) shade_kind = 0;
  SlabShape shape;
  size_t lds = 0;
  std::vector<int> work;
  if ((*why = slab_choose_shape(P, Q, dtype, tf_mode, ds, aux, shape, &lds, work))) return hipErrorNotSupported;

  const int nw = slab_waves(shape), nt = P.ntx * P.nty;
  const long long tsig = (((long long)P.ntx * 4096 + P.nty) * 64 + shape.tw) * 64 + shape.th + ((long long)(Q.perm * 2 + (Q.dir > 0)) << 48) +
                         ((long long)nw << 52) + ((long long)dtype << 56);
  hipError_t e = slab_measured_weights(aux, tsig, nt, work, Q);
  if (e != hipSuccess) return e;
  const int opt_split = P.depth ? 1 : aux->opt_split;
  slab_cut_segments(aux, work, nt, tsig, opt_split, slab_big(nw, shape.nl));
  std::vector<int2> order;
  slab_schedule(P, aux, work, (nw + shape.nl) | (opt_split << 12), order);
  int nblocks = 0;
  if ((e = slab_segments(P, Q, aux, order, &nblocks)) != hipSuccess) return e;
  if (slab_clock.on) {
    slab_clock.scan += slab_clock.frame_scan;
    slab_clock.planned += slab_now() - t0;
    if (++slab_clock.n % 60 == 0) {
      fprintf(stderr, "[smk] planning per frame: scans %.3f ms, all of it up to the launch %.3f ms, whole launcher (previous 60) %.3f ms\n",
              slab_clock.scan / 60, slab_clock.planned / 60, slab_clock.whole / 60);
      slab_clock.scan = slab_clock.planned = slab_clock.whole = 0;
    }
  }
  if ((e = slab_upload_order(aux, order, s)) != hipSuccess) return e;
  Q.order = aux->d_order;
  if ((e = slab_trace(P, Q, aux, nblocks, s)) != hipSuccess) return e;
  return slab_run(P, Q, aux, dtype, tf_mode, shade_kind, shape, lds, nblocks, tsig, why, s);
}

hipError_t smk_launch_slab(RenderParams P, int dtype, int tf_mode, int shade_kind, const void *vox_native, const void *vox_xmajor, SlabAux *aux,
                           const char **why, hipStream_t s) {
  const double t0 = slab_clock.on ? slab_now() : 0;
  const hipError_t e = slab_plan_and_launch(P, dtype, tf_mode, shade_kind, vox_native, vox_xmajor, aux, why, s);
  if (slab_clock.on) slab_clock.whole += slab_now() - t0;
  return e;
}
```

simian-spacemonkey_amd/csrc/smk_timesteps.hip:

```cpp
#include <string.h>

#include <algorithm>

#include "smk_internal.h"

int smk_step_wait_ready(smk_ctx *c, hipStream_t s) {
  if (c->ts_cur < 0) return 0;
  TimeStep &T = c->ts[c->ts_cur];
  if (!T.ready_pending) return 0;
  if (hipEventQuery(T.ready) == hipSuccess) {
    T.ready_pending = false;
    return 0;
  }
  (void)hipGetLastError();
  HIPCHK(c, hipStreamWaitEvent(s, T.ready, 0));
  return 0;
}

int smk_step_mark_used(smk_ctx *c, hipStream_t s) {
  if (!c->ts_series || c->ts_cur < 0) return 0;
  TimeStep &T = c->ts[c->ts_cur];
  if (!T.used) HIPCHK(c, hipEventCreateWithFlags(&T.used, hipEventDisableTiming));
  HIPCHK(c, hipEventRecord(T.used, s));
  T.used_valid = true;
  return 0;
}

static void free_step(TimeStep &T) {
  if (T.used_valid) (void)hipEventSynchronize(T.used);
  if (T.ready_pending) (void)hipEventSynchronize(T.ready);
  if (T.vox) (void)hipFree(T.vox);
  if (T.nrm) (void)hipFree(T.nrm);
  if (T.mm) (void)hipFree(T.mm);
  if (T.vox_x) (void)hipFree(T.vox_x);
  if (T.ready) (void)hipEventDestroy(T.ready);
  if (T.used) (void)hipEventDestroy(T.used);
  T = TimeStep();
}

void smk_free_steps(smk_ctx *c) {
  for (TimeStep &T : c->ts) free_step(T);
  c->ts.clear();
  c->ts_cur = -1;
}

void smk_use_step(smk_ctx *c, int k) {
  TimeStep &T = c->ts[(size_t)k];
  c->ts_cur = k;
  c->ts_cur_id = T.id;
  c->d_vox = T.vox;
  c->d_nrm = T.nrm;
  c->d_brick_mm = T.mm;
  c->d_vox_x = T.vox_x_valid ? T.vox_x : nullptr;
  c->bricks3_dirty = true;
  c->tf_dirty = true;
  c->have_volume = true;
}

static void switch_step(smk_ctx *c, int k) {
  smk_use_step(c, k);
  smk_slab_forget_measurements(&c->slab);
  bool layouts = false;
  for (const ColLayout &L : c->cols.lay) layouts |= L.d != nullptr;
  if (layouts) smk_cols_drop_layouts(&c->cols);
}

static int find_step(const smk_ctx *c, int id) {
  for (size_t k = 0; k < c->ts.size(); ++k)
    if (c->ts[k].id == id) return (int)k;
  return -1;
}

static size_t bytes_per_step(const smk_ctx *c) {
  const size_t nst = (size_t)c->D[0] * c->D[1] * c->D[2];
  const size_t nrm = c->dtype == SMK_F32 && c->nelts == 4 && c->have_normals ? nst * 4 : 0;
  return c->vox_bytes + 16 + nrm + (size_t)c->nbr[0] * c->nbr[1] * c->nbr[2] * sizeof(float4);
}

extern "C" int smk_set_timestep_cache(smk_ctx *c, int nsteps) {
  if (!c) return 1;
  if (nsteps < 1) FAIL(c, "smk_set_timestep_cache: capacity %d: the cache holds at least the current step", nsteps);
  HIPCHK(c, hipSetDevice(c->device));
  c->ts_series = true;
  if (!c->have_volume) {
    c->ts_cap = nsteps;
    return 0;
  }
  int held = 0;
  for (const TimeStep &T : c->ts) held += T.vox != nullptr;
  if (nsteps > held) {
    const size_t per = bytes_per_step(c), need = per * (size_t)(nsteps - held);
    size_t fr = 0, tot = 0;
    HIPCHK(c, hipMemGetInfo(&fr, &tot));
    if (need > fr)
      FAIL(c, "smk_set_timestep_cache: %d steps do not fit: %zu bytes per step, %zu bytes more needed, %zu free", nsteps, per, need, fr);
  }
  std::vector<int> order;
  for (size_t k = 0; k < c->ts.size(); ++k)
    if (c->ts[k].id >= 0) order.push_back((int)k);
  std::sort(order.begin(), order.end(), [&](int a, int b) { return c->ts[(size_t)a].written < c->ts[(size_t)b].written; });
  std::vector<int> keep;
  if (c->ts_cur >= 0) keep.push_back(c->ts_cur);
  for (int i = (int)order.size() - 1; i >= 0 && (int)keep.size() < nsteps; --i)
    if (order[(size_t)i] != c->ts_cur) keep.push_back(order[(size_t)i]);
  std::sort(keep.begin(), keep.end(), [&](int a, int b) { return c->ts[(size_t)a].written < c->ts[(size_t)b].written; });
  std::vector<TimeStep> ring((size_t)nsteps);
  int cur = -1;
  for (size_t i = 0; i < keep.size(); ++i) {
    if (keep[i] == c->ts_cur) cur = (int)i;
    ring[i] = c->ts[(size_t)keep[i]];
    c->ts[(size_t)keep[i]] = TimeStep();
  }
  for (TimeStep &T : c->ts) free_step(T);
  c->ts.swap(ring);
  c->ts_cap = nsteps;
  c->ts_cur = cur;
  return 0;
}

static int next_slot(const smk_ctx *c) {
  for (size_t k = 0; k < c->ts.size(); ++k)
    if (c->ts[k].id < 0) return (int)k;
  int last = 0;
  for (size_t k = 0; k < c->ts.size(); ++k)
    if (c->ts[k].written > c->ts[(size_t)last].written) last = (int)k;
  int k = (last + 1) % (int)c->ts.size();
  if (k == c->ts_cur) k = (k + 1) % (int)c->ts.size();
  return k;
}

static int upload_step(smk_ctx *c, const char *who, int id, const smk_volume_desc *b, int nb, int nelts, smk_dtype dtype,
                       smk_datamode dmode, bool on_device, void *stream) {
  if (!c) return 1;
  HIPCHK(c, hipSetDevice(c->device));
  if (id < 0) FAIL(c, "%s: time step %d: ids are >= 0", who, id);
  SmkVolGeom g;
  if (smk_volume_geometry(c, who, b, nb, nelts, dtype, dmode, g)) return 1;
  c->ts_series = true;
  if (c->have_volume) {
    if (g.N[0] != c->N[0] || g.N[1] != c->N[1] || g.N[2] != c->N[2])
      FAIL(c, "%s: time step %d: sizes %dx%dx%d differ from the series' %dx%dx%d", who, id, g.N[0], g.N[1], g.N[2], c->N[0], c->N[1], c->N[2]);
    if (g.fs[0] != c->fsize[0] || g.fs[1] != c->fsize[1] || g.fs[2] != c->fsize[2])
      FAIL(c, "%s: time step %d: extents %g x %g x %g differ from the series' %g x %g x %g", who, id, g.fs[0], g.fs[1], g.fs[2],
           c->fsize[0], c->fsize[1], c->fsize[2]);
    if (g.nelts != c->nelts) FAIL(c, "%s: time step %d: nelts %d differs from the series' %d", who, id, g.nelts, c->nelts);
    if (g.dtype != c->dtype) FAIL(c, "%s: time step %d: dtype %d differs from the series' %d", who, id, g.dtype, c->dtype);
    if (g.dmode != c->dmode) FAIL(c, "%s: time step %d: datamode %d differs from the series' %d", who, id, g.dmode, c->dmode);
    if (g.grad != c->have_normals)
      FAIL(c, "%s: time step %d: normals %s, the series' %s", who, id, g.grad ? "present" : "absent", c->have_normals ? "present" : "absent");
  }
  int k = c->have_volume ? find_step(c, id) : -1;
  if (k < 0) {
    if (!c->have_volume) {
      smk_set_geometry(c, g);
      c->ts.assign((size_t)c->ts_cap, TimeStep());
      c->ts_cur = -1;
      c->tune_choice.clear();
      c->tune_sig = 0;
    } else if (c->ts.size() == 1)
      FAIL(c, "%s: time step %d: the cache holds one step, the current one (%d); smk_set_timestep_cache sets more", who, id, c->ts_cur_id);
    k = next_slot(c);
  }
  TimeStep &T = c->ts[(size_t)k];
  const hipStream_t s = on_device ? (stream ? (hipStream_t)stream : c->stream) : nullptr;
  if (T.used_valid) {
    if (s) HIPCHK(c, hipStreamWaitEvent(s, T.used, 0));
    else HIPCHK(c, hipEventSynchronize(T.used));
  }
  if (T.ready_pending) {
    if (s) HIPCHK(c, hipStreamWaitEvent(s, T.ready, 0));
    else HIPCHK(c, hipEventSynchronize(T.ready));
    T.ready_pending = false;
  }
  T.id = -1;
  if (smk_alloc_step(c, g, T)) return 1;
  if (smk_pack_step(c, who, g, b, nb, on_device, T, s)) return 1;
  T.id = id;
  T.written = ++c->ts_written;
  if (s) {
    if (!T.ready) HIPCHK(c, hipEventCreateWithFlags(&T.ready, hipEventDisableTiming));
    HIPCHK(c, hipEventRecord(T.ready, s));
    T.ready_pending = true;
  }
  if (c->ts_cur < 0) smk_use_step(c, k);
  else if (k == c->ts_cur) switch_step(c, k);
  return 0;
}

extern "C" int smk_upload_timestep(smk_ctx *c, int timestep, const smk_volume_desc *bricks, int n_bricks, int nelts, smk_dtype dtype,
                                   smk_datamode dmode) {
  return upload_step(c, "smk_upload_timestep", timestep, bricks, n_bricks, nelts, dtype, dmode, false, nullptr);
}

extern "C" int smk_upload_timestep_device(smk_ctx *c, int timestep, const smk_volume_desc *bricks, int n_bricks, int nelts,
                                          smk_dtype dtype, smk_datamode dmode, void *stream) {
  return upload_step(c, "smk_upload_timestep_device", timestep, bricks, n_bricks, nelts, dtype, dmode, true, stream);
}

extern "C" int smk_select_timestep(smk_ctx *c, int timestep) {
  if (!c) return 1;
  HIPCHK(c, hipSetDevice(c->device));
  c->ts_series = true;
  if (!c->have_volume) FAIL(c, "smk_select_timestep: no volume uploaded");
  const int k = find_step(c, timestep);
  if (k < 0) FAIL(c, "smk_select_timestep: time step %d is not cached (upload it with smk_upload_timestep)", timestep);
  if (k != c->ts_cur) switch_step(c, k);
  return 0;
}

extern "C" int smk_get_timesteps(smk_ctx *c, int *current, int *ids_out, int cap, int *n) {
  if (!c) return 1;
  std::vector<const TimeStep *> held;
  for (const TimeStep &T : c->ts)
    if (T.id >= 0) held.push_back(&T);
  std::sort(held.begin(), held.end(), [](const TimeStep *a, const TimeStep *b) { return a->written < b->written; });
  if (current) *current = c->have_volume ? c->ts_cur_id : -1;
  if (n) *n = (int)held.size();
  if (ids_out)
    for (int i = 0; i < cap && i < (int)held.size(); ++i) ids_out[i] = held[(size_t)i]->id;
  return 0;
}
```

Before: 938,300.

## Cut per-frame stream ops: reuse timing events, double-buffer tick zeroing, throttle readbacks

Replaces the per-frame 'used' event records for transfer-function versions and time steps with a frame index that refers to the existing timing-ring end event. Double-buffers the slab tick array so the merge kernel zeroes the idle half, which removes a per-frame memset. Tick readbacks now happen only when the adaptive-weights logic will actually adopt them. Together these reduce per-frame enqueued stream operations and API overhead, and add frame-op counters for inspection. The trade-off is more complex lifetime tracking tied to the timing ring, plus extra zeroing work inside the merge kernel.

```diff
diff --git a/simian-spacemonkey_amd/csrc/smk_api.hip b/simian-spacemonkey_amd/csrc/smk_api.hip
--- a/simian-spacemonkey_amd/csrc/smk_api.hip
+++ b/simian-spacemonkey_amd/csrc/smk_api.hip
@@ -152,7 +152,6 @@
     if (T.h) (void)hipHostFree(T.h);
     free_brick_set(T.br);
     if (T.copied) (void)hipEventDestroy(T.copied);
-    if (T.used) (void)hipEventDestroy(T.used);
   }
   if (c->tf_raw_ev) (void)hipEventDestroy(c->tf_raw_ev);
   if (c->tf_ready) (void)hipEventDestroy(c->tf_ready);
@@ -814,7 +813,7 @@
   smk_ctx::TfVersion &T = c->tfv[v];
   if (T.cap < bytes) {
     if (T.copied) (void)hipEventSynchronize(T.copied);
-    if (T.used_valid) (void)hipEventSynchronize(T.used);
+    if (smk_frame_ref_wait(c, T.used_frame, nullptr)) return 1;
     if (T.d) (void)hipFree(T.d);
     if (T.h) (void)hipHostFree(T.h);
     T.d = nullptr;
@@ -824,8 +823,6 @@
     HIPCHK(c, hipHostMalloc((void **)&T.h, bytes, hipHostMallocDefault));
     T.cap = bytes;
     if (!T.copied) HIPCHK(c, hipEventCreateWithFlags(&T.copied, hipEventDisableTiming));
-    if (!T.used) HIPCHK(c, hipEventCreateWithFlags(&T.used, hipEventDisableTiming));
-    T.used_valid = false;
   } else if (T.copied) {
     HIPCHK(c, hipEventSynchronize(T.copied));
   }
@@ -849,7 +846,7 @@
   memcpy(map, newmap, 256);
   memcpy(c->tf_map_applied, newmap, 256);
   c->tf_map_valid = true;
-  if (T.used_valid) HIPCHK(c, hipStreamWaitEvent(s, T.used, 0));
+  if (smk_frame_ref_wait(c, T.used_frame, s)) return 1;
   HIPCHK(c, hipMemcpyAsync(T.d + n * 4 + occ_words * 4, map, 256, hipMemcpyHostToDevice, s));
   HIPCHK(c, hipEventRecord(T.copied, s));
   {
@@ -1062,6 +1059,9 @@
   if (!strncmp(name, "cols_", 5)) return smk_cols_stat(c, name, value);
   if (!strcmp(name, "slab_split_tiles")) { *value = c->slab.nsplit_last; return 0; }
   if (!strcmp(name, "slab_workgroups")) { *value = c->slab.nblocks_last; return 0; }
+  if (!strcmp(name, "frame_stream_ops")) { *value = c->frame_ops + c->slab.frame_ops + c->cols.frame_ops; return 0; }
+  if (!strcmp(name, "slab_tick_readbacks")) { *value = (double)c->slab.tick_readbacks; return 0; }
+  if (!strcmp(name, "slab_tick_adoptions")) { *value = (double)c->slab.tick_adoptions; return 0; }
   if (!strcmp(name, "slab_retries")) { *value = (double)c->slab_retries; return 0; }
   if (!strcmp(name, "clip_slice_pass")) { *value = c->clip_slice_pass; return 0; }
   FAIL(c, "smk_get_stat: unknown name '%s'", name);
diff --git a/simian-spacemonkey_amd/csrc/smk_cols_plan.hip b/simian-spacemonkey_amd/csrc/smk_cols_plan.hip
--- a/simian-spacemonkey_amd/csrc/smk_cols_plan.hip
+++ b/simian-spacemonkey_amd/csrc/smk_cols_plan.hip
@@ -274,6 +274,7 @@
     }
     hipError_t e = hipMemsetAsync(aux->d_masks, 0, aux->masks_cap, s);
     if (e != hipSuccess) return e;
+    ++aux->frame_ops;
     aux->masks_dirty = false;
   }
   aux->mask_words_last = Q.mask_words;
@@ -292,7 +293,10 @@
   Q.status_tag = aux->status_tag;
   Q.job_ticks = aux->d_ticks;
   Q.counts = aux->want_counts ? aux->d_counts : nullptr;
-  if (Q.counts) return hipMemsetAsync(aux->d_counts, 0, 64, s);
+  if (Q.counts) {
+    ++aux->frame_ops;
+    return hipMemsetAsync(aux->d_counts, 0, 64, s);
+  }
   return hipSuccess;
 }
 
@@ -307,6 +311,7 @@
   if (aux->frame_ev0) {
     hipError_t e = hipEventRecord(aux->frame_ev0, s);
     if (e != hipSuccess) return e;
+    ++aux->frame_ops;
   }
   hipError_t e = smk_cols_march(P, Q, dtype, tf_mode, shade_kind, L.perm, L.shape, lds, L.njobs, s);
   if (e == hipErrorInvalidValue) { *why = "no column-stream instance for this mode"; return hipErrorNotSupported; }
diff --git a/simian-spacemonkey_amd/csrc/smk_frame.hip b/simian-spacemonkey_amd/csrc/smk_frame.hip
--- a/simian-spacemonkey_amd/csrc/smk_frame.hip
+++ b/simian-spacemonkey_amd/csrc/smk_frame.hip
@@ -21,7 +21,8 @@
   double sum = 0;
   for (int i = 0; i < n; ++i) {
     float ms = 0;
-    HIPCHK(c, hipEventElapsedTime(&ms, c->tev0[i], c->tev1[i]));
+    const int slot = (int)((c->tframe - n + i) % SMK_TIMING_RING);
+    HIPCHK(c, hipEventElapsedTime(&ms, c->tev0[slot], c->tev1[slot]));
     sum += ms;
   }
   if (avg_ms) *avg_ms = n ? (float)(sum / n) : 0.f;
@@ -111,7 +112,7 @@
       HIPCHK(c, hipEventCreate(&c->tev1[i]));
     }
   }
-  int slot = (int)(c->tcount % SMK_TIMING_RING);
+  int slot = (int)(c->tframe % SMK_TIMING_RING);
   c->ev0 = c->tev0[slot];
   c->ev1 = c->tev1[slot];
   c->last_kernel = 1;
@@ -162,7 +163,7 @@
   }
   if (c->tune_state == SMK_TUNE_SETTLE + 3) {
     float ms_s = 0, ms_g = 0;
-    if (c->tcount - c->tune_tcount >= SMK_TIMING_RING - 8) (void)hipEventSynchronize(c->tev1[c->tune_slot[1]]);
+    if (c->tframe - c->tune_tframe >= SMK_TIMING_RING - 8) (void)hipEventSynchronize(c->tev1[c->tune_slot[1]]);
     if (hipEventQuery(c->tev1[c->tune_slot[0]]) == hipSuccess && hipEventQuery(c->tev1[c->tune_slot[1]]) == hipSuccess &&
         hipEventElapsedTime(&ms_s, c->tev0[c->tune_slot[0]], c->tev1[c->tune_slot[0]]) == hipSuccess &&
         hipEventElapsedTime(&ms_g, c->tev0[c->tune_slot[1]], c->tev1[c->tune_slot[1]]) == hipSuccess) {
@@ -197,7 +198,10 @@
 
 static int launch_slab(smk_ctx *c, const RenderParams &P, KernelChoice &k, bool ev0_recorded, hipStream_t s) {
   if (status_ring_ready(c)) return 1;
-  if (c->opt_lockstep & 16) HIPCHK(c, hipMemsetAsync(c->slab.d_diag, 0, 16 * sizeof(float), s));
+  if (c->opt_lockstep & 16) {
+    HIPCHK(c, hipMemsetAsync(c->slab.d_diag, 0, 16 * sizeof(float), s));
+    ++c->frame_ops;
+  }
   const char *why = nullptr;
   c->slab.frame_ev0 = ev0_recorded ? nullptr : c->ev0;
   hipError_t e = smk_launch_slab(P, c->dtype, c->tf_mode, smk_shade_kind(c), c->d_vox, c->d_vox_x, &c->slab, &why, s);
@@ -219,26 +223,47 @@
 }
 
 static int launch_gather(smk_ctx *c, const RenderParams &P, bool ev0_recorded, hipStream_t s) {
-  if (!ev0_recorded) HIPCHK(c, hipEventRecord(c->ev0, s));
+  if (!ev0_recorded) {
+    HIPCHK(c, hipEventRecord(c->ev0, s));
+    ++c->frame_ops;
+  }
   HIPCHK(c, smk_launch_gather(P, c->dtype, c->tf_mode, smk_shade_kind(c), s));
   return 0;
 }
 
+int smk_frame_ref_wait(smk_ctx *c, long long &frame, hipStream_t s) {
+  if (frame < 0) return 0;
+  const hipEvent_t done = c->tev1[(size_t)(frame % SMK_TIMING_RING)];
+  if (s) {
+    HIPCHK(c, hipStreamWaitEvent(s, done, 0));
+  } else {
+    HIPCHK(c, hipEventSynchronize(done));
+    frame = -1;
+  }
+  return 0;
+}
+
 static int frame_close(smk_ctx *c, hipStream_t s, int trial) {
+  const long long old = c->tframe - SMK_TIMING_RING;
+  if (old >= 0) {
+    for (int v = 0; v < 4; ++v)
+      if (c->tfv[v].used_frame == old && smk_frame_ref_wait(c, c->tfv[v].used_frame, nullptr)) return 1;
+    for (TimeStep &T : c->ts)
+      if (T.used_frame == old && smk_frame_ref_wait(c, T.used_frame, nullptr)) return 1;
+  }
   HIPCHK(c, hipEventRecord(c->ev1, s));
+  ++c->frame_ops;
   if (trial >= 0) {
     if (trial >= SMK_TUNE_SETTLE + 1) {
-      c->tune_slot[trial - (SMK_TUNE_SETTLE + 1)] = (int)(c->tcount % SMK_TIMING_RING);
-      c->tune_tcount = c->tcount;
+      c->tune_slot[trial - (SMK_TUNE_SETTLE + 1)] = (int)(c->tframe % SMK_TIMING_RING);
+      c->tune_tframe = c->tframe;
     }
     c->tune_state = trial + 1;
   }
-  if (c->tf_mode == 1 && c->tf_cur >= 0) {
-    HIPCHK(c, hipEventRecord(c->tfv[c->tf_cur].used, s));
-    c->tfv[c->tf_cur].used_valid = true;
-  }
-  if (smk_step_mark_used(c, s)) return 1;
+  if (c->tf_mode == 1 && c->tf_cur >= 0) c->tfv[c->tf_cur].used_frame = c->tframe;
+  smk_step_mark_frame(c, c->tframe);
   c->tcount++;
+  c->tframe++;
   return 0;
 }
 
@@ -254,6 +279,7 @@
   if (!d_rgba) FAIL(c, "%s: null output", who);
   RenderParams P;
   hipStream_t s = stream ? (hipStream_t)stream : c->stream;
+  c->frame_ops = c->slab.frame_ops = c->cols.frame_ops = 0;
   if (smk_build_params(c, P, s)) return 1;
   if (d_zscene) {
     P.zscene = d_zscene;
diff --git a/simian-spacemonkey_amd/csrc/smk_internal.h b/simian-spacemonkey_amd/csrc/smk_internal.h
--- a/simian-spacemonkey_amd/csrc/smk_internal.h
+++ b/simian-spacemonkey_amd/csrc/smk_internal.h
@@ -128,6 +128,10 @@
   std::vector<int2> plan_order;
   int plan_slots = 0;
   unsigned *d_ticks = nullptr, *h_ticks = nullptr;
+  unsigned *d_ticks_buf = nullptr;
+  int ticks_half = 0, ticks_clean[2] = {0, 0};
+  long long tick_readbacks = 0, tick_adoptions = 0;
+  int frame_ops = 0;
   int ticks_cap = 0, ticks_pending_n = 0, ticks_age = 0, ticks_adopted = 0;
   int ticks_n_last = 0;
   bool ticks_pending = false;
@@ -176,6 +180,7 @@
   double last_stream_bytes = 0;
   hipEvent_t frame_ev0 = nullptr;
   int status_tag = 0;
+  int frame_ops = 0;
 };
 void smk_cols_free(ColsAux *aux);
 void smk_cols_drop_layouts(ColsAux *aux);
@@ -204,6 +209,7 @@
   bool vox_x_valid = false;
   hipEvent_t ready = nullptr;
   bool ready_pending = false;
+  long long used_frame = -1;
   hipEvent_t used = nullptr;
   bool used_valid = false;
 };
@@ -215,6 +221,8 @@
   hipEvent_t ev0 = nullptr, ev1 = nullptr;
   std::vector<hipEvent_t> tev0, tev1;
   long long tcount = 0;
+  long long tframe = 0;
+  int frame_ops = 0;
 
   bool have_volume = false;
   int dtype = 0, nelts = 0, dmode = 0;
@@ -270,8 +278,8 @@
     unsigned char *d = nullptr, *h = nullptr;
     BrickSet br;
     size_t cap = 0;
-    hipEvent_t copied = nullptr, used = nullptr;
-    bool used_valid = false;
+    hipEvent_t copied = nullptr;
+    long long used_frame = -1;
   } tfv[4];
   int tf_cur = -1;
   int sv = 0, sg = 0, s3v = 0, s3g = 0, s3h = 0;
@@ -338,7 +346,7 @@
   unsigned long long last_slab_sig = 0;
   unsigned long long tune_sig = 0;
   int tune_state = 0, tune_slot[2] = {0, 0};
-  long long tune_tcount = 0;
+  long long tune_tframe = 0;
   int last_kernel = 0;
   float last_ms = 0;
   double last_alg_bytes = 0;
@@ -417,5 +425,7 @@
 #pragma GCC visibility pop
 
 int smk_step_wait_ready(smk_ctx *c, hipStream_t s);
+void smk_step_mark_frame(smk_ctx *c, long long frame);
 int smk_step_mark_used(smk_ctx *c, hipStream_t s);
+int smk_frame_ref_wait(smk_ctx *c, long long &frame, hipStream_t s);
 void smk_free_steps(smk_ctx *c);
diff --git a/simian-spacemonkey_amd/csrc/smk_shadow_plan.hip b/simian-spacemonkey_amd/csrc/smk_shadow_plan.hip
--- a/simian-spacemonkey_amd/csrc/smk_shadow_plan.hip
+++ b/simian-spacemonkey_amd/csrc/smk_shadow_plan.hip
@@ -335,6 +335,7 @@
 
 static int light_march(smk_ctx *c, RenderParams &P, const smk_shadowcoef &sc, const SmkShadowShard &S, size_t hstride, hipStream_t s) {
   HIPCHK(c, hipEventRecord(c->ev0, s));
+  ++c->frame_ops;
   hipError_t e = c->nranks > 1 ? smk_launch_shadow_march_shard(P, sc, c->dtype, c->tf_mode, c->d_light_hist, (long long)hstride, S, s)
                                : smk_launch_shadow_march(P, sc, c->dtype, c->tf_mode, c->d_light_hist, (long long)hstride, s);
   if (e == hipErrorNotSupported) FAIL(c, "smk_render: no shadow kernel instance for this configuration");
@@ -363,6 +364,7 @@
   HIPCHK(c, hipMemsetAsync(c->d_light[0], 0, nl * 16, s));
   HIPCHK(c, hipMemsetAsync(d_rgba, 0, (size_t)c->W * c->H * 16, s));
   if (d_depth) HIPCHK(c, hipMemsetD32Async((hipDeviceptr_t)d_depth, 0x7f800000, (size_t)c->W * c->H, s));
+  c->frame_ops += d_depth ? 4 : 3;
   if (!c->d_shadow_barrier) HIPCHK(c, hipMalloc((void **)&c->d_shadow_barrier, 16 * 9 * 4));
   hipError_t e = smk_launch_shadow(P, sc, c->dtype, c->tf_mode, smk_shade_kind(c), c->d_light[0], c->d_light[1], c->d_shadow_barrier, s);
   if (e == hipErrorNotSupported) FAIL(c, "smk_render: no shadow kernel instance for this configuration");
diff --git a/simian-spacemonkey_amd/csrc/smk_slab.h b/simian-spacemonkey_amd/csrc/smk_slab.h
--- a/simian-spacemonkey_amd/csrc/smk_slab.h
+++ b/simian-spacemonkey_amd/csrc/smk_slab.h
@@ -62,4 +62,4 @@
 hipError_t smk_slab_dispatch_occluded_shadow(const RenderParams &P, const SlabParams &Q, int dtype, int tf_mode, int shade_kind, int nw, int nl,
                                              size_t lds, int nblocks, const char **why, hipStream_t s);
 hipError_t smk_slab_merge(const int2 *list, int n, int tw, int th, int ntx, int W, int H, const float4 *seg_out, float4 *out, int use_max,
-                          hipStream_t s);
+                          unsigned *zero, int nzero, hipStream_t s);
diff --git a/simian-spacemonkey_amd/csrc/smk_slab.hip b/simian-spacemonkey_amd/csrc/smk_slab.hip
--- a/simian-spacemonkey_amd/csrc/smk_slab.hip
+++ b/simian-spacemonkey_amd/csrc/smk_slab.hip
@@ -1141,7 +1141,10 @@
 #define SLAB_PART 0
 #endif
 #if SLAB_PART == 0
-__global__ __launch_bounds__(256) void smk_k_slab_merge(const int2 *list, int tw, int th, int ntx, int W, int H, const float4 *seg_out, float4 *out, int use_max) {
+__global__ __launch_bounds__(256) void smk_k_slab_merge(const int2 *list, int tw, int th, int ntx, int W, int H, const float4 *seg_out, float4 *out, int use_max,
+                                                        unsigned *zero, int nzero) {
+  if (zero)
+    for (int i = blockIdx.x * blockDim.x + threadIdx.x; i < nzero; i += gridDim.x * blockDim.x) zero[i] = 0u;
   const int code = list[blockIdx.x].x;
   const int tile = code & 0xfffff, nseg = code >> 20;
   const int ty = tile / ntx, tx = tile - ty * ntx;
@@ -1167,8 +1170,8 @@
   }
 }
 hipError_t smk_slab_merge(const int2 *list, int n, int tw, int th, int ntx, int W, int H, const float4 *seg_out, float4 *out, int use_max,
-                          hipStream_t s) {
-  hipLaunchKernelGGL(smk_k_slab_merge, dim3(n), dim3(256), 0, s, list, tw, th, ntx, W, H, seg_out, out, use_max);
+                          unsigned *zero, int nzero, hipStream_t s) {
+  hipLaunchKernelGGL(smk_k_slab_merge, dim3(n), dim3(256), 0, s, list, tw, th, ntx, W, H, seg_out, out, use_max, zero, nzero);
   return hipGetLastError();
 }
 #endif
diff --git a/simian-spacemonkey_amd/csrc/smk_slab_plan.hip b/simian-spacemonkey_amd/csrc/smk_slab_plan.hip
--- a/simian-spacemonkey_amd/csrc/smk_slab_plan.hip
+++ b/simian-spacemonkey_amd/csrc/smk_slab_plan.hip
@@ -512,6 +512,13 @@
   return "no configuration fits";
 }
 
+static int slab_ticks_due(const SlabAux *aux) { return aux->ticks_adopted < 3 ? (4 << aux->ticks_adopted) : 32; }
+
+static bool slab_ticks_wanted(const SlabAux *aux, long long tsig) {
+  if (aux->ticks_pending) return false;
+  return aux->ticks_good_sig != tsig || aux->ticks_age + 1 >= slab_ticks_due(aux);
+}
+
 static hipError_t slab_measured_weights(SlabAux *aux, long long tsig, int nt, std::vector<int> &work, SlabParams &Q) {
   ++aux->ticks_age;
   if (aux->ticks_pending && aux->ticks_stale && hipEventQuery(aux->ticks_ev) == hipSuccess) {
@@ -519,8 +526,8 @@
   }
   if (aux->ticks_pending && hipEventQuery(aux->ticks_ev) == hipSuccess) {
     const bool fresh = aux->ticks_good_sig != aux->ticks_pending_sig;
-    const int due = aux->ticks_adopted < 3 ? (4 << aux->ticks_adopted) : 32;
-    if (fresh || aux->ticks_age >= due) {
+    if (fresh || aux->ticks_age >= slab_ticks_due(aux)) {
+      ++aux->tick_adoptions;
       if (fresh || (int)aux->ticks_good.size() != aux->ticks_pending_n) {
         aux->ticks_good.assign(aux->h_ticks, aux->h_ticks + aux->ticks_pending_n);
         aux->ticks_adopted = 0;
@@ -550,14 +557,15 @@
   if (nt > aux->ticks_cap) {
     if (aux->ticks_pending) (void)hipEventSynchronize(aux->ticks_ev);
     aux->ticks_pending = aux->ticks_stale = false;
-    if (aux->d_ticks) (void)hipFree(aux->d_ticks);
+    if (aux->d_ticks_buf) (void)hipFree(aux->d_ticks_buf);
     if (aux->h_ticks) (void)hipHostFree(aux->h_ticks);
     if (aux->d_pticks) (void)hipFree(aux->d_pticks);
     if (aux->h_pticks) (void)hipHostFree(aux->h_pticks);
-    aux->d_ticks = aux->h_ticks = aux->d_pticks = aux->h_pticks = nullptr;
+    aux->d_ticks_buf = aux->d_ticks = aux->h_ticks = aux->d_pticks = aux->h_pticks = nullptr;
     aux->ticks_cap = 0;
-    hipError_t e = hipMalloc((void **)&aux->d_ticks, (size_t)nt * 20);
-    if (e == hipSuccess) e = hipMemset(aux->d_ticks, 0, (size_t)nt * 20);
+    hipError_t e = hipMalloc((void **)&aux->d_ticks_buf, (size_t)nt * 40);
+    if (e == hipSuccess) e = hipMemset(aux->d_ticks_buf, 0, (size_t)nt * 40);
+    aux->ticks_clean[0] = aux->ticks_clean[1] = nt * 5;
     if (e == hipSuccess) e = hipHostMalloc((void **)&aux->h_ticks, (size_t)nt * 4, hipHostMallocDefault);
     if (e == hipSuccess) e = hipMalloc((void **)&aux->d_pticks, (size_t)nt * 32);
     if (e == hipSuccess) e = hipMemset(aux->d_pticks, 0, (size_t)nt * 32);
@@ -569,6 +577,8 @@
     hipError_t e = hipEventCreateWithFlags(&aux->ticks_ev, hipEventDisableTiming);
     if (e != hipSuccess) return e;
   }
+  aux->ticks_half ^= 1;
+  aux->d_ticks = aux->d_ticks_buf + (size_t)aux->ticks_half * aux->ticks_cap * 5;
   Q.tile_ticks = aux->d_ticks;
   Q.piece_ticks = aux->d_pticks;
   Q.ntiles = nt;
@@ -590,7 +600,7 @@
 }
 
 void smk_slab_free(SlabAux *aux) {
-  for (void *p : {(void *)aux->d_diag, (void *)aux->d_order, (void *)aux->d_pticks, aux->d_seg, (void *)aux->d_trace, (void *)aux->d_ticks})
+  for (void *p : {(void *)aux->d_diag, (void *)aux->d_order, (void *)aux->d_pticks, aux->d_seg, (void *)aux->d_trace, (void *)aux->d_ticks_buf})
     if (p) (void)hipFree(p);
   for (void *p : {(void *)aux->h_status, (void *)aux->h_pticks, (void *)aux->h_ticks, (void *)aux->h_order[0], (void *)aux->h_order[1],
                   (void *)aux->h_order[2], (void *)aux->h_order[3]})
@@ -769,6 +779,7 @@
   if (aux->frame_ev0) {
     hipError_t e = hipEventRecord(aux->frame_ev0, s);
     if (e != hipSuccess) return e;
+    ++aux->frame_ops;
   }
   auto same_order = [&]() { return aux->order_host.size() == order.size() && (order.empty() || !memcmp(aux->order_host.data(), order.data(), order.size() * sizeof(int2))); };
   if (!same_order()) {
@@ -796,6 +807,7 @@
     if (e != hipSuccess) return e;
     e = hipEventRecord(aux->order_ev[k], s);
     if (e != hipSuccess) return e;
+    aux->frame_ops += 2;
     aux->order_host.swap(order);
   }
   return hipSuccess;
@@ -814,6 +826,7 @@
   }
   hipError_t e = hipMemsetAsync(aux->d_trace, 0, (size_t)nblocks * 32, s);
   if (e != hipSuccess) return e;
+  ++aux->frame_ops;
   aux->trace_n = nblocks;
   Q.trace = aux->d_trace;
   return hipSuccess;
@@ -823,15 +836,20 @@
                            size_t lds, int nblocks, long long tsig, const char **why, hipStream_t s) {
   const int nw = slab_waves(sh), nt = Q.ntiles, nsplit = aux->nsplit_last;
   const bool diag = (P.lockstep & ~1) != 0 && dtype == 1 && shade_kind == 1;
-  hipError_t e = nsplit > 0 ? hipMemsetAsync(aux->d_ticks, 0, (size_t)nt * 20, s) : hipSuccess;
-  if (e != hipSuccess) return e;
+  hipError_t e = hipSuccess;
+  if (nsplit > 0 && aux->ticks_clean[aux->ticks_half] < nt * 5) {
+    if ((e = hipMemsetAsync(aux->d_ticks, 0, (size_t)nt * 20, s)) != hipSuccess) return e;
+    ++aux->frame_ops;
+  }
+  aux->ticks_clean[aux->ticks_half] = 0;
+  const bool read_back = slab_ticks_wanted(aux, tsig);
   if (!aux->merge_warm && nblocks >= 1) {
     aux->merge_warm = true;
     static const int2 one = make_int2(0 | (1 << 20), 0);
     int2 *d_one = nullptr;
     if (hipMalloc((void **)&d_one, sizeof one) == hipSuccess) {
       if (hipMemcpyAsync(d_one, &one, sizeof one, hipMemcpyHostToDevice, s) == hipSuccess)
-        (void)smk_slab_merge(d_one, 1, sh.tw, sh.th, P.ntx, P.W, P.H, (const float4 *)P.out, P.out, 0, s);
+        (void)smk_slab_merge(d_one, 1, sh.tw, sh.th, P.ntx, P.W, P.H, (const float4 *)P.out, P.out, 0, nullptr, 0, s);
       (void)hipStreamSynchronize(s);
       (void)hipFree(d_one);
     }
@@ -842,15 +860,20 @@
       : P.sh.on    ? smk_slab_dispatch_shadow(P, Q, dtype, tf_mode, shade_kind, nw, sh.nl, lds, nblocks, why, s)
       : dtype == 0 ? smk_slab_dispatch_u8(P, Q, tf_mode, shade_kind, nw, sh.nl, diag, lds, nblocks, why, s)
                    : smk_slab_dispatch_f32(P, Q, tf_mode, shade_kind, nw, sh.nl, diag, lds, nblocks, why, s);
-  if (e == hipSuccess && nsplit > 0)
+  if (e == hipSuccess && nsplit > 0) {
+    const int other = aux->ticks_half ^ 1;
     e = smk_slab_merge(aux->d_order + nblocks, nsplit, sh.tw, sh.th, P.ntx, P.W, P.H, (const float4 *)aux->d_seg, P.out,
-                       P.blend == SMK_BLEND_MAX ? 1 : 0, s);
-  if (e != hipSuccess || aux->ticks_pending) return e;
+                       P.blend == SMK_BLEND_MAX ? 1 : 0, aux->d_ticks_buf + (size_t)other * aux->ticks_cap * 5, nt * 5, s);
+    if (e == hipSuccess) aux->ticks_clean[other] = nt * 5;
+  }
+  if (e != hipSuccess || !read_back) return e;
   e = hipMemcpyAsync(aux->h_ticks, aux->d_ticks, (size_t)nt * 4, hipMemcpyDeviceToHost, s);
   if (e == hipSuccess && nsplit > 0) e = hipMemcpyAsync(aux->h_pticks, aux->d_pticks, (size_t)nt * 32, hipMemcpyDeviceToHost, s);
   if (nsplit > 0) aux->cuts_pending = aux->cuts; else aux->cuts_pending.clear();
   if (e == hipSuccess) e = hipEventRecord(aux->ticks_ev, s);
   if (e != hipSuccess) return e;
+  aux->frame_ops += nsplit > 0 ? 3 : 2;
+  ++aux->tick_readbacks;
   aux->ticks_pending = true;
   aux->ticks_pending_sig = tsig;
   aux->ticks_pending_n = nt;
diff --git a/simian-spacemonkey_amd/csrc/smk_timesteps.hip b/simian-spacemonkey_amd/csrc/smk_timesteps.hip
--- a/simian-spacemonkey_amd/csrc/smk_timesteps.hip
+++ b/simian-spacemonkey_amd/csrc/smk_timesteps.hip
@@ -17,6 +17,11 @@
   return 0;
 }
 
+void smk_step_mark_frame(smk_ctx *c, long long frame) {
+  if (!c->ts_series || c->ts_cur < 0) return;
+  c->ts[c->ts_cur].used_frame = frame;
+}
+
 int smk_step_mark_used(smk_ctx *c, hipStream_t s) {
   if (!c->ts_series || c->ts_cur < 0) return 0;
   TimeStep &T = c->ts[c->ts_cur];
@@ -26,7 +31,8 @@
   return 0;
 }
 
-static void free_step(TimeStep &T) {
+static void free_step(smk_ctx *c, TimeStep &T) {
+  (void)smk_frame_ref_wait(c, T.used_frame, nullptr);
   if (T.used_valid) (void)hipEventSynchronize(T.used);
   if (T.ready_pending) (void)hipEventSynchronize(T.ready);
   if (T.vox) (void)hipFree(T.vox);
@@ -39,7 +45,7 @@
 }
 
 void smk_free_steps(smk_ctx *c) {
-  for (TimeStep &T : c->ts) free_step(T);
+  for (TimeStep &T : c->ts) free_step(c, T);
   c->ts.clear();
   c->ts_cur = -1;
 }
@@ -111,7 +117,7 @@
     ring[i] = c->ts[(size_t)keep[i]];
     c->ts[(size_t)keep[i]] = TimeStep();
   }
-  for (TimeStep &T : c->ts) free_step(T);
+  for (TimeStep &T : c->ts) free_step(c, T);
   c->ts.swap(ring);
   c->ts_cap = nsteps;
   c->ts_cur = cur;
@@ -163,6 +169,7 @@
   }
   TimeStep &T = c->ts[(size_t)k];
   const hipStream_t s = on_device ? (stream ? (hipStream_t)stream : c->stream) : nullptr;
+  if (smk_frame_ref_wait(c, T.used_frame, s)) return 1;
   if (T.used_valid) {
     if (s) HIPCHK(c, hipStreamWaitEvent(s, T.used, 0));
     else HIPCHK(c, hipEventSynchronize(T.used));
```

After: 960,000, median of 4. 2.3% higher.
